# microsoft/UniVL

Hardware: NVIDIA H100
Metric: video-text samples/sec (higher is better)
Workload: dtype bf16

## Files before the change

### include/univl_b200.h

```cpp
#ifndef UNIVL_B200_H_
#define UNIVL_B200_H_

#ifdef __cplusplus
extern "C" {
#endif

const char* univl_last_error_string(void);
int univl_abi_version(void);
int univl_set_reserved_sms(int n);
int univl_partials_reduce(const float* part, int nparts, long long rows, long long cols, float* dst, long long ld,
                          void* stream);

int univl_gemm_bf16(const void* A, long long lda, int a_mn_major, const void* B, long long ldb, int b_mn_major,
                    int M, int N, int Kc, void* out, long long ldo, int epilogue, const float* bias,
                    const void* aux_in, long long ld_aux_in, void* aux_out, long long ld_aux_out, float alpha,
                    int block_n, int split_k, void* stream);
int univl_gemm_plan(int M, int N, int Kc, int epilogue, int block_n, int split_k);

int univl_quantize_e4m3_rows(const void* x, long long ldx, void* q, long long ldq, float* scale, int M, int K,
                             void* stream);
int univl_quantize_e4m3_blocks(const float* w, long long ldw, void* q, long long ldq, float* scale, int N, int K,
                               void* stream);
int univl_gemm_fp8(const void* A, long long lda, const float* a_scale, const void* B, long long ldb,
                   const float* b_scale, int M, int N, int Kc, int epilogue, const float* bias, void* out,
                   long long ldo, float* out_scale, void* stream);

int univl_layernorm_fwd(const void* x, const void* res, const float* gamma, const float* beta, void* y, float* mean,
                        float* rstd, int rows, int cols, float eps, float p_drop, int drop_mode,
                        const unsigned long long* rng_state, unsigned long long stream_id, void* stream);
int univl_layernorm_bwd(const void* dy, const void* dy2, const void* x, const void* res, const float* gamma,
                        const float* mean, const float* rstd, void* dx_res, void* dx_dense, float* dgamma,
                        float* dbeta, float* dbias, int rows, int cols, float p_drop, int drop_mode,
                        const unsigned long long* rng_state, unsigned long long stream_id, void* stream);
int univl_layernorm_f32_fwd(const float* x, const float* gamma, const float* beta, void* y, float* mean, float* rstd,
                            int rows, int cols, float eps, void* stream);
int univl_layernorm_f32_bwd(const void* dy, const float* x, const float* gamma, const float* mean, const float* rstd,
                            float* dgamma, float* dbeta, int rows, int cols, void* stream);

int univl_embed_text_fwd(const long long* ids, const long long* type_ids, const float* word, const float* pos,
                         const float* type, const float* gamma, const float* beta, void* y, float* mean, float* rstd,
                         int n_seq, int S, int H, int vocab, float eps, float p_drop, const unsigned long long* rng_state,
                         unsigned long long stream_id, void* stream);
int univl_embed_text_bwd(const void* dy, const long long* ids, const long long* type_ids, const float* word,
                         const float* pos, const float* type, const float* gamma, const float* mean,
                         const float* rstd, float* dword, float* dpos, float* dtype, float* dgamma, float* dbeta,
                         int n_seq, int S, int H, int vocab, float p_drop, const unsigned long long* rng_state,
                         unsigned long long stream_id, void* stream);
int univl_embed_src_fwd(const void* a, const void* b, const float* pos, const float* type, const float* gamma,
                        const float* beta, void* y, float* mean, float* rstd, int Na, int Wa, int Nb, int Fb,
                        int all_pairs, int H, float eps, float p_drop, const unsigned long long* rng_state,
                        unsigned long long stream_id, void* stream);
int univl_embed_src_bwd(const void* dy, const void* a, const void* b, const float* pos, const float* type,
                        const float* gamma, const float* mean, const float* rstd, void* da, void* db, float* dpos,
                        float* dtype, float* dgamma, float* dbeta, int Na, int Wa, int Nb, int Fb, int all_pairs,
                        int H, float p_drop, const unsigned long long* rng_state, unsigned long long stream_id, void* stream);

int univl_attention_fwd(const void* q, long long ldq, const void* k, long long ldk, const void* v, long long ldv,
                        void* o, long long ldo, float* lse, const long long* mask_a, const long long* mask_b, int Wa,
                        int Fb, int Nb, int all_pairs, int n_seq, int heads, int Sq, int Sk, int causal, float scale,
                        float p_drop, const unsigned long long* rng_state, unsigned long long stream_id, void* stream);
int univl_attention_bwd(const void* q, long long ldq, const void* k, long long ldk, const void* v, long long ldv,
                        const void* o, long long ldo, const float* lse, const void* d_o, long long lddo, void* dq,
                        long long lddq, void* dk, long long lddk, void* dv, long long lddv, const long long* mask_a,
                        const long long* mask_b, int Wa, int Fb, int Nb, int all_pairs, int n_seq, int heads, int Sq,
                        int Sk, int causal, float scale, float p_drop, const unsigned long long* rng_state,
                        unsigned long long stream_id, int rng_layout, float* dbq, float* dbk, float* dbv, void* stream);
int univl_attention_long_fwd(const void* q, long long ldq, const void* k, long long ldk, const void* v, long long ldv,
                             void* o, long long ldo, float* lse, const long long* mask_a, const long long* mask_b,
                             int Wa, int Fb, int Nb, int all_pairs, int n_seq, int heads, int Sq, int Sk, int causal,
                             float scale, float p_drop, const unsigned long long* rng_state,
                             unsigned long long stream_id, void* stream);
int univl_attention_long_bwd(const void* q, long long ldq, const void* k, long long ldk, const void* v, long long ldv,
                             const void* o, long long ldo, const float* lse, const void* d_o, long long lddo, void* dq,
                             long long lddq, void* dk, long long lddk, void* dv, long long lddv,
                             const long long* mask_a, const long long* mask_b, int Wa, int Fb, int Nb, int all_pairs,
                             int n_seq, int heads, int Sq, int Sk, int causal, float scale, float p_drop,
                             const unsigned long long* rng_state, unsigned long long stream_id, int rng_layout,
                             float* dbq, float* dbk, float* dbv, void* stream);
int univl_attention_pair_fwd(const void* qa, long long ldqa, const void* ka, long long ldka, const void* va,
                             long long ldva, const void* qb, long long ldqb, const void* kb, long long ldkb,
                             const void* vb, long long ldvb, void* o, long long ldo, float* lse,
                             const long long* mask_a, const long long* mask_b, int Na, int Wa, int Nb, int Fb,
                             int heads, int Sq, float scale, void* stream);
int univl_attention_varlen_fwd(const void* qa, long long ldqa, const void* ka, long long ldka, const void* va,
                               long long ldva, const void* qb, long long ldqb, const void* kb, long long ldkb,
                               const void* vb, long long ldvb, const int* idx_a, const int* idx_b, const int* start_a,
                               const int* start_b, const int* len_a, const int* cu_seqlens, int n_seq, int max_sk,
                               int heads, int q_first, void* o, long long ldo, float* lse, float scale, void* stream);
int univl_gather_rows_varlen(const void* a, long long lda, const void* b, long long ldb, const int* idx_a,
                             const int* idx_b, const int* start_a, const int* start_b, const int* len_a,
                             const int* cu_seqlens, int n_seq, int q_first, int cols, void* out, long long ldo,
                             void* stream);
int univl_fused_qkv_attention_supported(int n_seq, int heads, int S, int H);
int univl_fused_qkv_attention_fwd(const void* x, long long ldx, const void* wqkv, long long ldw, const float* bias,
                                  void* qkv_out, long long ld_qkv, void* o, long long ldo, float* lse,
                                  const long long* mask_a, const long long* mask_b, int Wa, int Fb, int Nb,
                                  int all_pairs, int n_seq, int heads, int S, int causal, float scale, float p_drop,
                                  const unsigned long long* rng_state, unsigned long long stream_id, void* stream);
int univl_fused_attention_bwd(const void* qkv, long long ld_qkv, const void* o, long long ldo, const float* lse,
                              const void* d_o, long long lddo, void* dqkv, long long ld_dqkv, float* dbias,
                              const long long* mask_a, const long long* mask_b, int Wa, int Fb, int Nb, int all_pairs,
                              int n_seq, int heads, int S, int causal, float scale, float p_drop,
                              const unsigned long long* rng_state, unsigned long long stream_id, void* stream);

int univl_colsum_bf16(const void* x, long long ld, float* out, int rows, int cols, void* stream);
int univl_cast_f32_to_bf16(const float* src, void* dst, long long n, void* stream);
int univl_cast_bf16_to_f32(const void* src, float* dst, long long n, void* stream);
int univl_multi_cast_f32_to_bf16(const unsigned long long* device_table, int n_tensors, int blocks_per_tensor,
                                 void* stream);
int univl_fill_f32(float* p, float value, long long n, void* stream);
int univl_rng_advance(unsigned long long* rng_state, void* stream);
int univl_gelu_fwd_bf16(const void* x, void* out, long long n, void* stream);
int univl_gelu_bwd_bf16(const void* dy, const void* pre, void* out, long long n, void* stream);
int univl_tanh_fwd_bf16(const void* x, void* out, long long n, void* stream);
int univl_tanh_bwd_bf16(const void* dy, const void* y, void* out, long long n, void* stream);
int univl_scale_f32(float* dst, const float* src, long long n, const float* gscale, void* stream);

int univl_meanpool_fwd(const void* x, const long long* mask, float* out, float* norm_out, int N, int S, int H,
                       int skip_first, int guard_zero, int l2norm, void* stream);
int univl_meanpool_bwd(const float* dy, const float* y, const float* norm, const long long* mask, void* dx, int N,
                       int S, int H, int skip_first, int guard_zero, int l2norm, void* stream);
int univl_sim_matmul_fwd(const float* t, const float* v, float* sim, int Bt, int Bv, int H, int groups, void* stream);
int univl_sim_matmul_bwd(const float* dsim, const float* t, const float* v, float* dt, float* dv, int Bt, int Bv,
                         int H, int groups, void* stream);
int univl_maxmargin_loss(const float* sim, float* loss, float* dsim, int B, float margin, int n_pair, float w_same,
                         float w_diff, int groups, void* stream);
int univl_crossen_loss(const float* sim, float* loss, float* dsim, int B, int groups, void* stream);
int univl_milnce_loss(const float* sim, float* loss, float* dsim, int batch_size, int n_pair, int groups,
                      void* stream);
int univl_softmax_xent_fwd(const float* logits, long long ld, const long long* labels, const long long* pair_mask,
                           float* lse, float* sum_count, float* loss, int T, int V, int target_mode,
                           long long ignore_index, int groups, void* stream);
int univl_softmax_xent_bwd(const float* logits, long long ld, const long long* labels, const long long* pair_mask,
                           const float* lse, const float* sum_count, const float* gscale, void* dlogits,
                           long long ld_d, int T, int V, int target_mode, long long ignore_index, int groups,
                           void* stream);
int univl_vocab_xent_workspace(int T, int V);
int univl_vocab_xent_fwd(const void* x, long long ldx, const void* w, long long ldw, const float* bias,
                         const long long* labels, float* lse, float* sum_count, float* loss, void* workspace,
                         long long workspace_bytes, int T, int V, int Kc, int groups, void* stream);
int univl_vocab_xent_bwd(const void* x, long long ldx, const void* w, long long ldw, const float* bias,
                         const long long* labels, const float* lse, const float* sum_count, const float* gscale,
                         void* dlogits, long long ld_d, int T, int V, int Kc, int groups, void* stream);
int univl_pooler_sim_fwd(const void* u, const float* w, const float* b, float* out, int N, int H, void* stream);
int univl_pooler_sim_bwd(const void* u, const float* w, const float* dout, void* du, float* dw, float* db, int N,
                         int H, void* stream);

int univl_bert_adam_step(float* p, const float* g, float* m, float* v, void* p_bf16, const void* segs, int n_chunks,
                         int n_tensors, float* scratch, long long* step, float b1, float b2, float eps,
                         float max_grad_norm, float global_clip_norm, float warmup, long long t_total,
                         float grad_scale, void* stream);
int univl_bert_adam_step_bf16grad(float* p, const void* g_bf16, float* m, float* v, void* p_bf16, const void* segs,
                                  int n_chunks, int n_tensors, float* scratch, long long* step, float b1, float b2,
                                  float eps, float max_grad_norm, float global_clip_norm, float warmup,
                                  long long t_total, float grad_scale, void* stream);

#ifdef __cplusplus
}
#endif
#endif
```

### univl_b200/csrc/gemm_wgmma.cu

```cuda
#include "common.cuh"
#include "fp8.cuh"
#include "pipeline.cuh"
#include "tmap.cuh"

#include <stdio.h>
#include <type_traits>

namespace univl {

enum GemmEpilogue : int {
  EPI_BIAS_BF16 = 0,
  EPI_BIAS_GELU_BF16 = 1,
  EPI_GELU_BWD_BF16 = 2,
  EPI_ADD_BF16 = 3,
  EPI_BIAS_F32 = 4,
  EPI_ATOMIC_F32 = 5,
};

struct GemmParams {
  int M, N, Kc;
  int k_blocks_per_split;
  int epilogue;
  float alpha;
  void* out;
// ... 102 lines not shown
  if (epi == EPI_BIAS_GELU_BF16) {
    bf16* ao = p.aux_out + (long long)row * p.ld_aux_out + col;
    if (vec) *reinterpret_cast<uint32_t*>(ao) = pack_bf16x2(v0, v1);
    else {
      ao[0] = __float2bfloat16(v0);
      if (two) ao[1] = __float2bfloat16(v1);
    }
    v0 = gelu_erf(v0);
    v1 = gelu_erf(v1);
  }
  bf16* o = reinterpret_cast<bf16*>(p.out) + (long long)row * p.ldo + col;
  if (vec) *reinterpret_cast<uint32_t*>(o) = pack_bf16x2(v0, v1);
  else {
    o[0] = __float2bfloat16(v0);
    if (two) o[1] = __float2bfloat16(v1);
  }
}

constexpr int EPI_CHUNK = 8;

__device__ __forceinline__ uint4 quad_transpose(uint32_t w0, uint32_t w1, uint32_t w2, uint32_t w3, int q) {
  const bool odd = q & 1;
  uint32_t r0 = __shfl_xor_sync(0xffffffffu, odd ? w0 : w1, 1);
  uint32_t r1 = __shfl_xor_sync(0xffffffffu, odd ? w2 : w3, 1);
  if (odd) {
    w0 = r0;
    w2 = r1;
  } else {
    w1 = r0;
    w3 = r1;
  }
  const bool hi = q & 2;
  r0 = __shfl_xor_sync(0xffffffffu, hi ? w0 : w2, 2);
  r1 = __shfl_xor_sync(0xffffffffu, hi ? w1 : w3, 2);
  if (hi) {
    w0 = r0;
    w1 = r1;
  } else {
    w2 = r0;
    w3 = r1;
  }
  return make_uint4(w0, w1, w2, w3);
}

template <int EPI, bool BIAS, int BLOCK_N, bool WIDE = false>
__device__ __forceinline__ void epi_tile(const GemmParams& p, float alpha, int row, int col0,
                                         const float (&acc)[BLOCK_N / 2]) {
  constexpr int GROUPS = BLOCK_N / 8;
  constexpr int CHUNK = WIDE ? 4 : (GROUPS < EPI_CHUNK ? GROUPS : EPI_CHUNK);
  static_assert(CHUNK % 4 == 0, "a chunk holds whole quads of 8-column groups");
  constexpr bool AUX = EPI == EPI_GELU_BWD_BF16 || EPI == EPI_ADD_BF16;
  constexpr bool OUT_F32 = EPI == EPI_BIAS_F32 || EPI == EPI_ATOMIC_F32;
  static_assert(!(WIDE && OUT_F32), "16-byte stores are for the bf16 outputs");
  constexpr bool ACCUM = EPI == EPI_ATOMIC_F32;
  const int q = threadIdx.x & 3;
  const float* bias = p.bias + col0;
  const bf16* ax = p.aux_in + (long long)row * p.ld_aux_in + col0;
  const long long ax8 = 8 * p.ld_aux_in;
  bf16* ao = p.aux_out + (long long)row * p.ld_aux_out + col0;
  const long long ao8 = 8 * p.ld_aux_out;
  const long long o8 = 8 * p.ldo;
  float* of = reinterpret_cast<float*>(p.out) + (long long)row * p.ldo + col0;
  bf16* ob = reinterpret_cast<bf16*>(p.out) + (long long)row * p.ldo + col0;
  float b[2][CHUNK][2];
  uint32_t x[2][CHUNK][2];
  float2 a[2][CHUNK][2];
  auto load = [&](int j0, int s) {
#pragma unroll
    for (int j = 0; j < CHUNK; ++j) {
      const int c = (j0 + j) * 8;
      if constexpr (BIAS) {
        b[s][j][0] = __ldg(bias + c);
        b[s][j][1] = __ldg(bias + c + 1);
      }
#pragma unroll
      for (int h = 0; h < 2; ++h) {
        if constexpr (AUX) x[s][j][h] = *reinterpret_cast<const uint32_t*>(ax + h * ax8 + c);
        if constexpr (ACCUM) a[s][j][h] = *reinterpret_cast<const float2*>(of + h * o8 + c);
      }
    }
  };
  load(0, 0);
#pragma unroll
  for (int j0 = 0; j0 < GROUPS; j0 += CHUNK) {
    const int s = (j0 / CHUNK) & 1;
    if (j0 + CHUNK < GROUPS) load(j0 + CHUNK, s ^ 1);
#pragma unroll
    for (int jq = 0; jq < CHUNK; jq += 4) {
#pragma unroll
      for (int h = 0; h < 2; ++h) {
        uint32_t wo[4], wa[4];
#pragma unroll
        for (int jj = 0; jj < 4; ++jj) {
          const int j = jq + jj;
          const int c = (j0 + j) * 8;
          float v0 = __fmul_rn(acc[4 * (j0 + j) + 2 * h], alpha);
          float v1 = __fmul_rn(acc[4 * (j0 + j) + 2 * h + 1], alpha);
          if constexpr (BIAS) {
            v0 = __fadd_rn(v0, b[s][j][0]);
            v1 = __fadd_rn(v1, b[s][j][1]);
          }
          if constexpr (AUX) {
            const float2 f = unpack_bf16x2(x[s][j][h]);
            if constexpr (EPI == EPI_GELU_BWD_BF16) {
              v0 = __fmul_rn(v0, gelu_erf_grad(f.x));
              v1 = __fmul_rn(v1, gelu_erf_grad(f.y));
            } else {
              v0 = __fadd_rn(v0, f.x);
              v1 = __fadd_rn(v1, f.y);
            }
          }
          if constexpr (OUT_F32) {
            if constexpr (ACCUM) {
              v0 = __fadd_rn(a[s][j][h].x, v0);
              v1 = __fadd_rn(a[s][j][h].y, v1);
            }
            *reinterpret_cast<float2*>(of + h * o8 + c) = make_float2(v0, v1);
          } else {
            if constexpr (EPI == EPI_BIAS_GELU_BF16) {
              const uint32_t w = pack_bf16x2(v0, v1);
              if constexpr (WIDE) wa[jj] = w;
              else *reinterpret_cast<uint32_t*>(ao + h * ao8 + c) = w;
              v0 = gelu_erf(v0);
              v1 = gelu_erf(v1);
            }
            const uint32_t w = pack_bf16x2(v0, v1);
            if constexpr (WIDE) wo[jj] = w;
            else *reinterpret_cast<uint32_t*>(ob + h * o8 + c) = w;
          }
        }
        if constexpr (WIDE) {
          const int c = (j0 + jq) * 8 + 6 * q;
          if constexpr (EPI == EPI_BIAS_GELU_BF16)
            *reinterpret_cast<uint4*>(ao + h * ao8 + c) = quad_transpose(wa[0], wa[1], wa[2], wa[3], q);
          *reinterpret_cast<uint4*>(ob + h * o8 + c) = quad_transpose(wo[0], wo[1], wo[2], wo[3], q);
        }
      }
    }
  }
}

template <int BLOCK_N>
__device__ __forceinline__ void epilogue_block(const GemmParams& p, bool inside, float alpha, int n0, int row,
                                               int col0, const float (&acc)[BLOCK_N / 2]) {
  if (inside) {
    const bool bias = p.bias != nullptr;
    const bool wide = p.vec8;
    switch (p.epilogue) {
      case EPI_BIAS_BF16:
        if (wide) {
          if (bias) epi_tile<EPI_BIAS_BF16, true, BLOCK_N, true>(p, alpha, row, col0, acc);
          else epi_tile<EPI_BIAS_BF16, false, BLOCK_N, true>(p, alpha, row, col0, acc);
        } else {
          if (bias) epi_tile<EPI_BIAS_BF16, true, BLOCK_N>(p, alpha, row, col0, acc);
          else epi_tile<EPI_BIAS_BF16, false, BLOCK_N>(p, alpha, row, col0, acc);
        }
        break;
      case EPI_BIAS_GELU_BF16:
        if (wide) {
          if (bias) epi_tile<EPI_BIAS_GELU_BF16, true, BLOCK_N, true>(p, alpha, row, col0, acc);
          else epi_tile<EPI_BIAS_GELU_BF16, false, BLOCK_N, true>(p, alpha, row, col0, acc);
        } else {
          if (bias) epi_tile<EPI_BIAS_GELU_BF16, true, BLOCK_N>(p, alpha, row, col0, acc);
          else epi_tile<EPI_BIAS_GELU_BF16, false, BLOCK_N>(p, alpha, row, col0, acc);
        }
        break;
      case EPI_GELU_BWD_BF16:
        if (wide) epi_tile<EPI_GELU_BWD_BF16, false, BLOCK_N, true>(p, alpha, row, col0, acc);
        else epi_tile<EPI_GELU_BWD_BF16, false, BLOCK_N>(p, alpha, row, col0, acc);
        break;
      case EPI_ADD_BF16:
        if (wide) epi_tile<EPI_ADD_BF16, false, BLOCK_N, true>(p, alpha, row, col0, acc);
        else epi_tile<EPI_ADD_BF16, false, BLOCK_N>(p, alpha, row, col0, acc);
        break;
      case EPI_BIAS_F32:
        if (bias) epi_tile<EPI_BIAS_F32, true, BLOCK_N>(p, alpha, row, col0, acc);
        else epi_tile<EPI_BIAS_F32, false, BLOCK_N>(p, alpha, row, col0, acc);
        break;
      default:
        epi_tile<EPI_ATOMIC_F32, false, BLOCK_N>(p, alpha, row, col0, acc);
    }
  } else {
#pragma unroll
    for (int j = 0; j < BLOCK_N / 8; ++j) {
      if (n0 + j * 8 >= p.N) break;
      epi_pair(p, alpha, row, col0 + j * 8, acc[4 * j], acc[4 * j + 1]);
      epi_pair(p, alpha, row + 8, col0 + j * 8, acc[4 * j + 2], acc[4 * j + 3]);
    }
  }
}

__device__ __forceinline__ bool tile_inside(const GemmParams& p, const WorkItem& wi, int bn) {
  return p.vec2 && wi.m0 + BLOCK_M <= p.M && wi.n0 + bn <= p.N;
}

template <int BLOCK_N>
__device__ __forceinline__ bool splitk_fixup(const GemmParams& p, int tile, int half, int split, float alpha,
                                             float (&acc)[BLOCK_N / 2]) {
  constexpr int V = BLOCK_N / 8;
  constexpr int CHUNK = BLOCK_N == 256 ? 4 : 8;
  const int t = threadIdx.x & 127;
  const int lane = t & 31;
  const long long slot = 64LL * BLOCK_N;
  float4* base = reinterpret_cast<float4*>(p.slots + ((long long)tile * p.splits * 2 + half) * slot) + t;
  float4* mine = base + split * (2 * slot / 4);
#pragma unroll
  for (int j = 0; j < V; ++j) {
#pragma unroll
    for (int e = 0; e < 4; ++e) acc[4 * j + e] = __fmul_rn(acc[4 * j + e], alpha);
    __stcg(mine + j * 128, make_float4(acc[4 * j], acc[4 * j + 1], acc[4 * j + 2], acc[4 * j + 3]));
  }
  fence_acq_rel_gpu();
  __syncwarp();
  unsigned before = 0;
  if (lane == 0) before = atom_add_acq_rel_gpu(p.arrived + (tile * 2 + half) * 4 + (t >> 5), 1u);
  before = __shfl_sync(0xffffffffu, before, 0);
  if (before != (unsigned)p.splits - 1) return false;
  fence_acq_rel_gpu();
#pragma unroll
  for (int j0 = 0; j0 < V; j0 += CHUNK) {
    float4 s4[CHUNK];
#pragma unroll
    for (int j = 0; j < CHUNK; ++j) s4[j] = make_float4(0.f, 0.f, 0.f, 0.f);
    for (int s = 0; s < p.splits; ++s) {
      float4 v[CHUNK];
      if (s == split) {
#pragma unroll
        for (int j = 0; j < CHUNK; ++j) {
          const int a = 4 * (j0 + j);
          v[j] = make_float4(acc[a], acc[a + 1], acc[a + 2], acc[a + 3]);
        }
      } else {
        const float4* src = base + s * (2 * slot / 4);
#pragma unroll
        for (int j = 0; j < CHUNK; ++j) v[j] = __ldcg(src + (j0 + j) * 128);
      }
#pragma unroll
      for (int j = 0; j < CHUNK; ++j) {
        s4[j].x = __fadd_rn(s4[j].x, v[j].x);
        s4[j].y = __fadd_rn(s4[j].y, v[j].y);
        s4[j].z = __fadd_rn(s4[j].z, v[j].z);
        s4[j].w = __fadd_rn(s4[j].w, v[j].w);
      }
    }
#pragma unroll
    for (int j = 0; j < CHUNK; ++j) {
      const int a = 4 * (j0 + j);
      acc[a] = s4[j].x;
      acc[a + 1] = s4[j].y;
      acc[a + 2] = s4[j].z;
      acc[a + 3] = s4[j].w;
    }
  }
  return true;
}

template <int BLOCK_N>
__device__ __forceinline__ void finish_block(const GemmParams& p, const WorkItem& wi, int n_tiles, int kb_per,
                                             bool inside, float alpha, int half, int row, int col0,
                                             float (&acc)[BLOCK_N / 2]) {
  if (p.slots != nullptr) {
    const int tile = (wi.m0 / BLOCK_M) * n_tiles + wi.n0 / BLOCK_N;
    if (!splitk_fixup<BLOCK_N>(p, tile, half, wi.kb_begin / kb_per, alpha, acc)) return;
    alpha = 1.f;
  }
  epilogue_block<BLOCK_N>(p, inside, alpha, wi.n0, row, col0, acc);
}

constexpr int TURN_BAR = 1;

template <int BLOCK_N, int STAGES, bool A_MN, bool B_MN, int ELEM = 2>
__device__ __forceinline__ void produce_ring(const CUtensorMap* tmap_a, const CUtensorMap* tmap_b, uint8_t* smem,
                                             const Ring<STAGES>& ring, int num_work, int m_tiles, int n_tiles,
                                             int total_kb, int kb_per) {
  using L = GemmSmem<BLOCK_N, STAGES>;
  uint32_t it = 0;
  for (int w = blockIdx.x; w < num_work; w += gridDim.x) {
    const WorkItem wi = decode_work(w, m_tiles, n_tiles, total_kb, kb_per, BLOCK_N);
    for (int i = 0; i < wi.num_kb; ++i, ++it) {
      const int s = ring.acquire(it, L::STAGE_BYTES);
      uint64_t* bar = &ring.full[s];
      uint8_t* sa = smem + s * L::STAGE_BYTES;
      uint8_t* sb = sa + L::A_BYTES;
      const int k_elem = (wi.kb_begin + i) * (128 / ELEM);
      if (!A_MN) {
        tma_load_2d(sa, tmap_a, bar, k_elem, wi.m0);
      } else {
#pragma unroll
        for (int c = 0; c < BLOCK_M / 64; ++c)
          tma_load_2d(sa + c * (BLOCK_K * 128), tmap_a, bar, wi.m0 + c * 64, k_elem);
      }
      if (!B_MN) {
        tma_load_2d(sb, tmap_b, bar, k_elem, wi.n0);
      } else {
#pragma unroll
        for (int c = 0; c < BLOCK_N / 64; ++c)
          tma_load_2d(sb + c * (BLOCK_K * 128), tmap_b, bar, wi.n0 + c * 64, k_elem);
      }
    }
  }
}

template <int BLOCK_N, int STAGES, bool A_MN, bool B_MN>
__global__ void __launch_bounds__(PIPELINE_THREADS, 1)
gemm_wgmma_kernel(const __grid_constant__ CUtensorMap tmap_a, const __grid_constant__ CUtensorMap tmap_b,
                  const GemmParams p, const int num_work) {
  using L = GemmSmem<BLOCK_N, STAGES>;
  constexpr bool PING = BLOCK_N <= 128;
  constexpr bool FOLD = BLOCK_N == 64;
  Ring<STAGES> ring;
  uint8_t* smem = kernel_prologue(ring, L::BAR_OFFSET, PING ? 1 : 2, &tmap_a, &tmap_b);

  const int wg = threadIdx.x >> 7;
  const int m_tiles = (p.M + BLOCK_M - 1) / BLOCK_M;
  const int n_tiles = (p.N + BLOCK_N - 1) / BLOCK_N;
  const int total_kb = (p.Kc + BLOCK_K - 1) / BLOCK_K;
  const int kb_per = p.k_blocks_per_split;

  if (wg == 0) {
    if (producer_regs())
      produce_ring<BLOCK_N, STAGES, A_MN, B_MN>(&tmap_a, &tmap_b, smem, ring, num_work, m_tiles, n_tiles, total_kb,
                                                kb_per);
  } else if constexpr (!PING) {
    consumer_regs();
    const int c = wg - 1;
    const int t = threadIdx.x & 127;
    const int warp = t >> 5, lane = t & 31;
    uint32_t it = 0;
    for (int w = blockIdx.x; w < num_work; w += gridDim.x) {
      const WorkItem wi = decode_work(w, m_tiles, n_tiles, total_kb, kb_per, BLOCK_N);
      float acc[BLOCK_N / 2];
#pragma unroll
      for (int e = 0; e < BLOCK_N / 2; ++e) acc[e] = 0.f;
      const int last = mma_kblocks<BLOCK_N, A_MN, B_MN, L::STAGE_BYTES, L::A_BYTES>(ring, smem, c * (64 * 128), acc,
                                                                                     0, wi.num_kb, it, t == 0);
      mma_drain(ring, last, acc, t == 0);
      const int row = wi.m0 + c * 64 + warp * 16 + (lane >> 2);
      const int col0 = wi.n0 + 2 * (lane & 3);
      finish_block<BLOCK_N>(p, wi, n_tiles, kb_per, tile_inside(p, wi, BLOCK_N), p.alpha, c, row, col0, acc);
    }
  } else {
    consumer_regs();
    const int c = wg - 1;
    const int t = threadIdx.x & 127;
    const int warp = t >> 5, lane = t & 31;
    uint32_t it = 0;
    int j = 0;
    for (int w = blockIdx.x; w < num_work; w += gridDim.x, ++j) {
      const WorkItem wi = decode_work(w, m_tiles, n_tiles, total_kb, kb_per, BLOCK_N);
      if ((j & 1) != c) {
        it += wi.num_kb;
        continue;
      }
      float acc[2][BLOCK_N / 2];
#pragma unroll
      for (int e = 0; e < BLOCK_N / 2; ++e) acc[0][e] = acc[1][e] = 0.f;
      const bool fold = FOLD && p.kb_seg < wi.num_kb;
      const int seg = fold ? p.kb_seg : wi.num_kb;
      float sum[2][FOLD ? BLOCK_N / 2 : 1];
      if constexpr (FOLD) {
#pragma unroll
        for (int e = 0; e < BLOCK_N / 2; ++e) sum[0][e] = sum[1][e] = 0.f;
      }
      if (j > 0) named_bar(TURN_BAR + c, 256);
      for (int i0 = 0; i0 < wi.num_kb; i0 += seg) {
        const int i1 = min(wi.num_kb, i0 + seg);
        const int last =
            mma_kblocks<BLOCK_N, 2, A_MN, B_MN, L::STAGE_BYTES, L::A_BYTES>(ring, smem, 0, acc, i0, i1, it, t == 0);
        if (i1 == wi.num_kb && w + (int)gridDim.x < num_work)
          named_bar_arrive(TURN_BAR + (c ^ 1), 256);
        mma_drain(ring, last, acc, t == 0);
        if constexpr (FOLD) {
          if (fold) {
#pragma unroll
            for (int e = 0; e < BLOCK_N / 2; ++e) {
              sum[0][e] = __fadd_rn(sum[0][e], __fmul_rn(acc[0][e], p.alpha));
              sum[1][e] = __fadd_rn(sum[1][e], __fmul_rn(acc[1][e], p.alpha));
            }
          }
        }
      }
      float alpha = p.alpha;
      if constexpr (FOLD) {
        if (fold) {
#pragma unroll
          for (int e = 0; e < BLOCK_N / 2; ++e) {
            acc[0][e] = sum[0][e];
            acc[1][e] = sum[1][e];
          }
          alpha = 1.f;
        }
      }
      const bool inside = tile_inside(p, wi, BLOCK_N);
      const int row = wi.m0 + warp * 16 + (lane >> 2);
      const int col0 = wi.n0 + 2 * (lane & 3);
      finish_block<BLOCK_N>(p, wi, n_tiles, kb_per, inside, alpha, 0, row, col0, acc[0]);
      finish_block<BLOCK_N>(p, wi, n_tiles, kb_per, inside, alpha, 1, row + 64, col0, acc[1]);
    }
  }
}

template <int BLOCK_N, int STAGES, bool A_MN, bool B_MN>
static int launch_gemm(const CUtensorMap& ta, const CUtensorMap& tb, const GemmParams& p, int splits,
                       cudaStream_t stream) {
  using L = GemmSmem<BLOCK_N, STAGES>;
  auto kern = gemm_wgmma_kernel<BLOCK_N, STAGES, A_MN, B_MN>;
  const char* name = "univl_gemm_bf16";
  if (int rc = persistent_prepare(kern, L::DYN_BYTES, name)) return rc;
  const long long work =
      (long long)((p.M + BLOCK_M - 1) / BLOCK_M) * ((p.N + BLOCK_N - 1) / BLOCK_N) * (long long)splits;
  return persistent_launch(kern, name, work, L::DYN_BYTES, stream, ta, tb, p, (int)work);
}

template <int BLOCK_N, int STAGES>
static int dispatch_major(bool a_mn, bool b_mn, const CUtensorMap& ta, const CUtensorMap& tb, const GemmParams& p,
                          int splits, cudaStream_t stream) {
  if (!a_mn && !b_mn) return launch_gemm<BLOCK_N, STAGES, false, false>(ta, tb, p, splits, stream);
  if (!a_mn && b_mn) return launch_gemm<BLOCK_N, STAGES, false, true>(ta, tb, p, splits, stream);
  if (a_mn && b_mn) return launch_gemm<BLOCK_N, STAGES, true, true>(ta, tb, p, splits, stream);
  return launch_gemm<BLOCK_N, STAGES, true, false>(ta, tb, p, splits, stream);
}

enum Fp8Epilogue : int { FP8_EPI_BIAS_BF16 = 0, FP8_EPI_GELU_E4M3 = 1 };

struct Fp8Params {
  const float* a_scale;
  const float* b_scale;
  uint8_t* out_q;
  float* out_scale;
};

constexpr int FP8_BLOCK_N = 128;
constexpr int FP8_STAGES = 6;

template <int EPI, bool PAIRS>
__global__ void __launch_bounds__(PIPELINE_THREADS, 1)
gemm_fp8_kernel(const __grid_constant__ CUtensorMap tmap_a, const __grid_constant__ CUtensorMap tmap_b,
                const GemmParams p, const Fp8Params f, const int num_work) {
  using L = GemmSmem<FP8_BLOCK_N, FP8_STAGES>;
  Ring<FP8_STAGES> ring;
  uint8_t* smem = kernel_prologue(ring, L::BAR_OFFSET, 2, &tmap_a, &tmap_b);

  const int wg = threadIdx.x >> 7;
  const int m_tiles = (p.M + BLOCK_M - 1) / BLOCK_M;
  const int n_tiles = p.N / FP8_BLOCK_N;
  const int total_kb = p.Kc / 128;

  if (wg == 0) {
    if (producer_regs())
      produce_ring<FP8_BLOCK_N, FP8_STAGES, false, false, 1>(&tmap_a, &tmap_b, smem, ring, num_work, m_tiles, n_tiles,
                                                              total_kb, total_kb);
    return;
  }
  consumer_regs();
  const int c = wg - 1;
  const int t = threadIdx.x & 127;
  const int warp = t >> 5, lane = t & 31;
  const int M = p.M;
  uint32_t it = 0;
  for (int w = blockIdx.x; w < num_work; w += gridDim.x) {
    const WorkItem wi = decode_work(w, m_tiles, n_tiles, total_kb, total_kb, FP8_BLOCK_N);
    const int row = wi.m0 + c * 64 + warp * 16 + (lane >> 2);
    const bool in0 = row < M, in1 = row + 8 < M;
    const float* sa = f.a_scale + row;
    const float* sb = f.b_scale + (long long)(wi.n0 / FP8_BLOCK_N) * total_kb;
    float acc[FP8_BLOCK_N / 2];
#pragma unroll
    for (int e = 0; e < FP8_BLOCK_N / 2; ++e) acc[e] = 0.f;
    auto issue = [&](float (&tmp)[FP8_BLOCK_N / 2], int kb) {
      const int s = ring.wait(it + kb);
      const uint32_t a_s = smem_u32(smem + s * L::STAGE_BYTES) + c * (64 * 128);
      const uint32_t b_s = smem_u32(smem + s * L::STAGE_BYTES) + L::A_BYTES;
      wgmma_fence();
      fence_regs(tmp);
#pragma unroll
      for (int k = 0; k < 4; ++k)
        WgmmaSSE4M3N128::mma(tmp, make_smem_desc_sw128(a_s + k * 32, 16, 1024),
                             make_smem_desc_sw128(b_s + k * 32, 16, 1024), k > 0 ? 1 : 0);
      wgmma_commit();
      fence_regs(tmp);
    };
    auto promote = [&](auto newer, float (&tmp)[FP8_BLOCK_N / 2], int kb) {
      const float bs = __ldg(sb + kb);
      const float s0 = in0 ? __ldg(sa + (long long)kb * M) : 0.f;
      const float s1 = in1 ? __ldg(sa + (long long)kb * M + 8) : 0.f;
      wgmma_wait<decltype(newer)::value>();
      fence_regs(tmp);
      if (t == 0) ring.release(ring.stage(it + kb));
      const float f0 = s0 * bs, f1 = s1 * bs;
#pragma unroll
      for (int j = 0; j < FP8_BLOCK_N / 8; ++j) {
        acc[4 * j] = __fmaf_rn(tmp[4 * j], f0, acc[4 * j]);
        acc[4 * j + 1] = __fmaf_rn(tmp[4 * j + 1], f0, acc[4 * j + 1]);
        acc[4 * j + 2] = __fmaf_rn(tmp[4 * j + 2], f1, acc[4 * j + 2]);
        acc[4 * j + 3] = __fmaf_rn(tmp[4 * j + 3], f1, acc[4 * j + 3]);
      }
    };
    using One = std::integral_constant<int, 1>;
    using None = std::integral_constant<int, 0>;
    float ta[FP8_BLOCK_N / 2];
    if constexpr (PAIRS) {
      float tb[FP8_BLOCK_N / 2];
      issue(ta, 0);
      issue(tb, 1);
      int kb = 0;
      for (; kb + 2 < total_kb; kb += 2) {
        promote(One(), ta, kb);
        issue(ta, kb + 2);
        promote(One(), tb, kb + 1);
        issue(tb, kb + 3);
      }
      promote(One(), ta, kb);
      promote(None(), tb, kb + 1);
    } else {
      for (int kb = 0; kb < total_kb; ++kb) {
        issue(ta, kb);
        promote(None(), ta, kb);
      }
    }
    it += total_kb;
    const int col0 = wi.n0 + 2 * (lane & 3);
    if constexpr (EPI == FP8_EPI_BIAS_BF16) {
      if (tile_inside(p, wi, FP8_BLOCK_N)) {
        if (p.vec8) epi_tile<EPI_BIAS_BF16, true, FP8_BLOCK_N, true>(p, p.alpha, row, col0, acc);
        else epi_tile<EPI_BIAS_BF16, true, FP8_BLOCK_N>(p, p.alpha, row, col0, acc);
      } else {
#pragma unroll
        for (int j = 0; j < FP8_BLOCK_N / 8; ++j) {
          epi_pair(p, p.alpha, row, col0 + j * 8, acc[4 * j], acc[4 * j + 1]);
          epi_pair(p, p.alpha, row + 8, col0 + j * 8, acc[4 * j + 2], acc[4 * j + 3]);
        }
      }
    } else {
      const float* bias = p.bias + col0;
#pragma unroll
      for (int h = 0; h < 2; ++h) {
        float amax = 0.f;
#pragma unroll
        for (int j = 0; j < FP8_BLOCK_N / 8; ++j) {
          const float v0 = gelu_erf(__fadd_rn(acc[4 * j + 2 * h], __ldg(bias + 8 * j)));
          const float v1 = gelu_erf(__fadd_rn(acc[4 * j + 2 * h + 1], __ldg(bias + 8 * j + 1)));
          acc[4 * j + 2 * h] = v0;
          acc[4 * j + 2 * h + 1] = v1;
          amax = fmaxf(amax, fmaxf(fabsf(v0), fabsf(v1)));
        }
        amax = fmaxf(amax, __shfl_xor_sync(0xffffffffu, amax, 1));
        amax = fmaxf(amax, __shfl_xor_sync(0xffffffffu, amax, 2));
        const float sc = e4m3_scale(amax);
        const float inv = e4m3_inv_scale(sc);
        const int r = row + 8 * h;
        if (r < M) {
          uint8_t* q = f.out_q + (long long)r * p.ldo + col0;
#pragma unroll
          for (int j = 0; j < FP8_BLOCK_N / 8; ++j)
            *reinterpret_cast<uint16_t*>(q + 8 * j) =
                e4m3x2(__fmul_rn(acc[4 * j + 2 * h], inv), __fmul_rn(acc[4 * j + 2 * h + 1], inv));
          if ((lane & 3) == 0) f.out_scale[(long long)(wi.n0 / FP8_BLOCK_N) * M + r] = sc;
        }
      }
    }
  }
}

template <int EPI, bool PAIRS>
static int launch_gemm_fp8(const CUtensorMap& ta, const CUtensorMap& tb, const GemmParams& p, const Fp8Params& f,
                           cudaStream_t stream) {
  using L = GemmSmem<FP8_BLOCK_N, FP8_STAGES>;
  auto kern = gemm_fp8_kernel<EPI, PAIRS>;
  const char* name = "univl_gemm_fp8";
  if (int rc = persistent_prepare(kern, L::DYN_BYTES, name)) return rc;
  const long long work = (long long)((p.M + BLOCK_M - 1) / BLOCK_M) * (p.N / FP8_BLOCK_N);
  return persistent_launch(kern, name, work, L::DYN_BYTES, stream, ta, tb, p, f, (int)work);
}

constexpr int VX_BLOCK_N = 128;
constexpr int VX_STAGES = 6;

struct VocabXentParams {
  int T, V, Kc;
  int m_tiles, n_tiles, chunks, chunk_tiles;
  const float* bias;
  const long long* labels;
  float4* part;
  const float* lse;
  const float* count;
  const float* gscale;
  int rows_per_group, groups;
  bf16* dl;
  long long ld_d;
};

template <bool BWD>
__global__ void __launch_bounds__(PIPELINE_THREADS, 1)
vocab_xent_kernel(const __grid_constant__ CUtensorMap tmap_a, const __grid_constant__ CUtensorMap tmap_b,
                  const VocabXentParams p, const int num_work) {
  using L = GemmSmem<VX_BLOCK_N, VX_STAGES>;
  Ring<VX_STAGES> ring;
  uint8_t* smem = kernel_prologue(ring, L::BAR_OFFSET, 2, &tmap_a, &tmap_b);
  const int wg = threadIdx.x >> 7;
  const int total_kb = (p.Kc + BLOCK_K - 1) / BLOCK_K;

  if (wg == 0) {
    if (!producer_regs()) return;
    uint32_t it = 0;
    for (int w = blockIdx.x; w < num_work; w += gridDim.x) {
      const int chunk = w / p.m_tiles;
      const int m0 = (w - chunk * p.m_tiles) * BLOCK_M;
      const int nt1 = min(p.n_tiles, (chunk + 1) * p.chunk_tiles);
      for (int nt = chunk * p.chunk_tiles; nt < nt1; ++nt) {
        for (int kb = 0; kb < total_kb; ++kb, ++it) {
          const int s = ring.acquire(it, L::STAGE_BYTES);
          uint8_t* sa = smem + s * L::STAGE_BYTES;
          tma_load_2d(sa, &tmap_a, &ring.full[s], kb * BLOCK_K, m0);
          tma_load_2d(sa + L::A_BYTES, &tmap_b, &ring.full[s], kb * BLOCK_K, nt * VX_BLOCK_N);
        }
      }
    }
    return;
  }
  consumer_regs();
  const int c = wg - 1;
  const int t = threadIdx.x & 127;
  const int warp = t >> 5, lane = t & 31, q = lane & 3;
  uint32_t it = 0;
  for (int w = blockIdx.x; w < num_work; w += gridDim.x) {
    const int chunk = w / p.m_tiles;
    const int row = (w - chunk * p.m_tiles) * BLOCK_M + c * 64 + warp * 16 + (lane >> 2);
    long long lab[2];
    float m[2], s[2], xt[2], lse[2], g[2];
#pragma unroll
    for (int h = 0; h < 2; ++h) {
      const int r = row + 8 * h;
      lab[h] = r < p.T ? __ldg(p.labels + r) : -1;
      m[h] = -INFINITY;
      s[h] = 0.f;
      xt[h] = 0.f;
      if constexpr (BWD) {
        lse[h] = 0.f;
        g[h] = 0.f;
        if (lab[h] != -1) {
          lse[h] = __ldg(p.lse + r);
          g[h] = ((p.gscale ? __ldg(p.gscale) : 1.f) / (float)p.groups) / __ldg(p.count + r / p.rows_per_group);
        }
      }
    }
    const int nt1 = min(p.n_tiles, (chunk + 1) * p.chunk_tiles);
    for (int nt = chunk * p.chunk_tiles; nt < nt1; ++nt) {
      float acc[VX_BLOCK_N / 2];
#pragma unroll
      for (int e = 0; e < VX_BLOCK_N / 2; ++e) acc[e] = 0.f;
      const int last = mma_kblocks<VX_BLOCK_N, false, false, L::STAGE_BYTES, L::A_BYTES>(ring, smem, c * (64 * 128),
                                                                                          acc, 0, total_kb, it, t == 0);
      mma_drain(ring, last, acc, t == 0);

      const int col0 = nt * VX_BLOCK_N + 2 * q;
#pragma unroll
      for (int j = 0; j < VX_BLOCK_N / 8; ++j) {
#pragma unroll
        for (int e = 0; e < 2; ++e) {
          const int col = col0 + 8 * j + e;
          const float b = (p.bias != nullptr && col < p.V) ? __ldg(p.bias + col) : 0.f;
          acc[4 * j + e] = __fadd_rn(acc[4 * j + e], b);
          acc[4 * j + 2 + e] = __fadd_rn(acc[4 * j + 2 + e], b);
        }
      }
      if constexpr (!BWD) {
#pragma unroll
        for (int h = 0; h < 2; ++h) {
          float tm = -INFINITY;
#pragma unroll
          for (int j = 0; j < VX_BLOCK_N / 8; ++j)
#pragma unroll
            for (int e = 0; e < 2; ++e)
              if (col0 + 8 * j + e < p.V) tm = fmaxf(tm, acc[4 * j + 2 * h + e]);
          if (tm > m[h]) {
            s[h] = s[h] * __expf(m[h] - tm);
            m[h] = tm;
          }
#pragma unroll
          for (int j = 0; j < VX_BLOCK_N / 8; ++j)
#pragma unroll
            for (int e = 0; e < 2; ++e) {
              const int col = col0 + 8 * j + e;
              const float v = acc[4 * j + 2 * h + e];
              if (col < p.V) s[h] += __expf(v - m[h]);
              if (col == lab[h]) xt[h] = v;
            }
        }
      } else {
        const int ncol = min(p.ld_d - (long long)nt * VX_BLOCK_N, (long long)VX_BLOCK_N);
#pragma unroll
        for (int h = 0; h < 2; ++h) {
          const int r = row + 8 * h;
          if (r >= p.T) continue;
          bf16* drow = p.dl + (long long)r * p.ld_d + col0;
          const bool scored = lab[h] != -1;
#pragma unroll
          for (int j = 0; j < VX_BLOCK_N / 8; ++j) {
            if (8 * j + 2 * q >= ncol) break;
            float d[2];
#pragma unroll
            for (int e = 0; e < 2; ++e) {
              const int col = col0 + 8 * j + e;
              d[e] = 0.f;
              if (scored && col < p.V)
                d[e] = (__expf(acc[4 * j + 2 * h + e] - lse[h]) - (col == lab[h] ? 1.f : 0.f)) * g[h];
            }
            *reinterpret_cast<uint32_t*>(drow + 8 * j) = pack_bf16x2(d[0], d[1]);
          }
        }
      }
    }
    if constexpr (!BWD) {
#pragma unroll
      for (int h = 0; h < 2; ++h) {
#pragma unroll
        for (int o = 1; o <= 2; o <<= 1) {
          const float mo = __shfl_xor_sync(0xffffffffu, m[h], o);
          const float so = __shfl_xor_sync(0xffffffffu, s[h], o);
          const float xo = __shfl_xor_sync(0xffffffffu, xt[h], o);
          const float mx = fmaxf(m[h], mo);
          const float a = m[h] == -INFINITY ? 0.f : s[h] * __expf(m[h] - mx);
          const float b = mo == -INFINITY ? 0.f : so * __expf(mo - mx);
          m[h] = mx;
          s[h] = a + b;
          xt[h] += xo;
        }
        const int r = row + 8 * h;
        if (q == 0 && r < p.T) p.part[(long long)r * p.chunks + chunk] = make_float4(m[h], s[h], xt[h], 0.f);
      }
    }
  }
}

__global__ void __launch_bounds__(256)
vocab_xent_rows_kernel(const float4* __restrict__ part, const long long* __restrict__ labels, int T, int V, int chunks,
                       int chunk_cols, float* __restrict__ lse_out, float* __restrict__ nll) {
  const int r = blockIdx.x * blockDim.x + threadIdx.x;
  if (r >= T) return;
  const long long lab = labels[r];
  if (lab == -1) {
    lse_out[r] = 0.f;
    return;
  }
  const float4* pr = part + (long long)r * chunks;
  float4 f = pr[0];
  float m = f.x, s = f.y;
  for (int k = 1; k < chunks; ++k) {
    f = pr[k];
    const float mx = fmaxf(m, f.x);
    s = s * __expf(m - mx) + f.y * __expf(f.x - mx);
    m = mx;
  }
  const float lse = m + __logf(s);
  lse_out[r] = lse;
  nll[r] = (lab >= 0 && lab < V) ? lse - pr[lab / chunk_cols].z : __int_as_float(0x7fc00000);
}

constexpr int VX_GROUP_THREADS = 512;
__global__ void __launch_bounds__(VX_GROUP_THREADS)
vocab_xent_group_kernel(const float* __restrict__ nll, const long long* __restrict__ labels, int rows_per_group,
                        float* __restrict__ sum_count, int groups) {
  __shared__ float red[2][VX_GROUP_THREADS];
  const int grp = blockIdx.x;
  float sum = 0.f, cnt = 0.f;
  for (int i = threadIdx.x; i < rows_per_group; i += VX_GROUP_THREADS) {
    const long long r = (long long)grp * rows_per_group + i;
    if (labels[r] == -1) continue;
    sum += nll[r];
    cnt += 1.f;
  }
  red[0][threadIdx.x] = sum;
  red[1][threadIdx.x] = cnt;
  __syncthreads();
  for (int o = VX_GROUP_THREADS / 2; o > 0; o >>= 1) {
    if (threadIdx.x < o) {
      red[0][threadIdx.x] += red[0][threadIdx.x + o];
      red[1][threadIdx.x] += red[1][threadIdx.x + o];
    }
    __syncthreads();
  }
  if (threadIdx.x == 0) {
    sum_count[grp] = red[0][0];
    sum_count[groups + grp] = red[1][0];
  }
}

__global__ void vocab_xent_mean_kernel(const float* __restrict__ sum_count, int groups, float* __restrict__ out) {
  float acc = sum_count[0] / sum_count[groups];
  for (int g = 1; g < groups; ++g) acc += sum_count[g] / sum_count[groups + g];
  *out = groups > 1 ? acc / (float)groups : acc;
}

template <bool BWD>
static int launch_vocab_xent(const CUtensorMap& ta, const CUtensorMap& tb, const VocabXentParams& p,
                             cudaStream_t stream) {
  const long long work = (long long)p.m_tiles * p.chunks;
  return persistent_launch(vocab_xent_kernel<BWD>, BWD ? "univl_vocab_xent_bwd" : "univl_vocab_xent_fwd", work,
                           GemmSmem<VX_BLOCK_N, VX_STAGES>::DYN_BYTES, stream, ta, tb, p, (int)work);
}

}

using namespace univl;

namespace {
struct GemmPlan {
  int bn, splits, kb_per, kb_seg;
};
int plan_gemm(int M, int N, int Kc, int epilogue, int block_n, int split_k, GemmPlan* plan) {
  const int total_kb = (Kc + BLOCK_K - 1) / BLOCK_K;
  const int m_tiles = (M + BLOCK_M - 1) / BLOCK_M;
  int bn = block_n;
  if (bn == 0) {
    bn = 256;
    if (epilogue != EPI_ATOMIC_F32) {
      const auto tiles = [&](int w) { return (long long)m_tiles * ((N + w - 1) / w); };
      if (tiles(256) < 2 * PLAN_SMS) bn = 128;
      if (tiles(128) < PLAN_SMS) bn = 64;
    }
    if (N <= 64) bn = 64;
    else if (N <= 128 && bn > 128) bn = 128;
  }
  UNIVL_CHECK_ARG(bn == 64 || bn == 128 || bn == 256, "gemm: block_n must be 64/128/256");
  const int n_tiles = (N + bn - 1) / bn;
  int splits = 1;
  if (epilogue == EPI_ATOMIC_F32) {
    splits = split_k;
    if (splits == 0) {
      const long long tiles = (long long)m_tiles * n_tiles;
      splits = (int)((2 * PLAN_SMS + tiles - 1) / tiles);
      if (splits > total_kb / 2) splits = total_kb / 2;
      if (splits < 1) splits = 1;
    }
    if (splits > total_kb) splits = total_kb;
  }
  int kb_per = (total_kb + splits - 1) / splits;
  splits = (total_kb + kb_per - 1) / kb_per;
  int kb_seg = kb_per;
  if (epilogue == EPI_ATOMIC_F32 && block_n == 0 && split_k == 0 && Kc < SPLIT_MIN_K && splits > 1) {
    bn = 64;
    splits = 1;
    kb_per = total_kb;
  }
  plan->bn = bn; plan->splits = splits; plan->kb_per = kb_per; plan->kb_seg = kb_seg;
  return UNIVL_OK;
}

GemmParams gemm_params(int M, int N, int Kc, int kb_per, int epilogue, float alpha, void* out, long long ldo,
                       const float* bias, const void* aux_in, long long ld_aux_in, void* aux_out,
                       long long ld_aux_out) {
  GemmParams p;
  p.M = M; p.N = N; p.Kc = Kc;
  p.k_blocks_per_split = kb_per;
  p.epilogue = epilogue;
  p.alpha = alpha;
  p.out = out; p.ldo = ldo;
  p.bias = bias;
  p.aux_in = reinterpret_cast<const bf16*>(aux_in); p.ld_aux_in = ld_aux_in;
  p.aux_out = reinterpret_cast<bf16*>(aux_out); p.ld_aux_out = ld_aux_out;
  const bool out_f32 = epilogue == EPI_BIAS_F32 || epilogue == EPI_ATOMIC_F32;
  bool vec2 = ((uintptr_t)out % (out_f32 ? 8 : 4)) == 0 && (ldo % 2) == 0;
  if (aux_in != nullptr) vec2 = vec2 && ((uintptr_t)aux_in % 4) == 0 && (ld_aux_in % 2) == 0;
  if (aux_out != nullptr) vec2 = vec2 && ((uintptr_t)aux_out % 4) == 0 && (ld_aux_out % 2) == 0;
  p.vec2 = vec2 ? 1 : 0;
  bool vec8 = !out_f32 && ((uintptr_t)out % 16) == 0 && (ldo % 8) == 0;
  if (aux_out != nullptr) vec8 = vec8 && ((uintptr_t)aux_out % 16) == 0 && (ld_aux_out % 8) == 0;
  p.vec8 = vec8 ? 1 : 0;
  p.slots = nullptr;
  p.arrived = nullptr;
  p.splits = 1;
  p.kb_seg = kb_per;
  return p;
}
}

extern "C" int univl_gemm_plan(int M, int N, int Kc, int epilogue, int block_n, int split_k) {
  GemmPlan plan;
  if (int rc = plan_gemm(M, N, Kc, epilogue, block_n, split_k, &plan)) return rc;
  return 1;
}

extern "C" int univl_gemm_bf16(const void* A, long long lda, int a_mn_major, const void* B, long long ldb,
                               int b_mn_major, int M, int N, int Kc, void* out, long long ldo, int epilogue,
                               const float* bias, const void* aux_in, long long ld_aux_in, void* aux_out,
                               long long ld_aux_out, float alpha, int block_n, int split_k, void* stream_) {
  cudaStream_t stream = reinterpret_cast<cudaStream_t>(stream_);
  UNIVL_CHECK_ARG(M > 0 && N > 0 && Kc > 0, "gemm: empty problem M=%d N=%d K=%d", M, N, Kc);
  UNIVL_CHECK_ARG(A && B && out, "gemm: null operand");
  UNIVL_CHECK_ARG((lda % 8) == 0 && (ldb % 8) == 0, "gemm: lda/ldb must be multiples of 8 elements (got %lld, %lld)",
                  lda, ldb);
  UNIVL_CHECK_ARG(((uintptr_t)A & 15) == 0 && ((uintptr_t)B & 15) == 0, "gemm: operands must be 16-byte aligned");
  UNIVL_CHECK_ARG(epilogue >= 0 && epilogue <= 5, "gemm: unknown epilogue %d", epilogue);
  if (epilogue == EPI_GELU_BWD_BF16 || epilogue == EPI_ADD_BF16)
    UNIVL_CHECK_ARG(aux_in != nullptr, "gemm: epilogue %d needs aux_in", epilogue);
  if (epilogue == EPI_BIAS_GELU_BF16) UNIVL_CHECK_ARG(aux_out != nullptr, "gemm: gelu epilogue needs aux_out");
  UNIVL_CHECK_ARG(split_k >= 0, "gemm: bad split_k");
  if (epilogue != EPI_ATOMIC_F32) UNIVL_CHECK_ARG(split_k <= 1, "gemm: split_k>1 needs the atomic epilogue");

  GemmPlan plan;
  if (int prc = plan_gemm(M, N, Kc, epilogue, block_n, split_k, &plan)) return prc;
  const int bn = plan.bn;

  CUtensorMap ta, tb;
  int rc;
  if (!a_mn_major) rc = make_tmap(&ta, A, M, Kc, lda, BLOCK_M);
  else             rc = make_tmap(&ta, A, Kc, M, lda, BLOCK_K);
  if (rc) return rc;
  if (!b_mn_major) rc = make_tmap(&tb, B, N, Kc, ldb, bn);
  else             rc = make_tmap(&tb, B, Kc, N, ldb, BLOCK_K);
  if (rc) return rc;

  GemmParams p = gemm_params(M, N, Kc, plan.kb_per, epilogue, alpha, out, ldo, bias, aux_in, ld_aux_in, aux_out,
                             ld_aux_out);
  p.splits = plan.splits;
  p.kb_seg = plan.kb_seg;
  if (plan.splits > 1) {
    const long long tiles = (long long)((M + BLOCK_M - 1) / BLOCK_M) * ((N + bn - 1) / bn);
    const size_t slot_bytes = (size_t)tiles * plan.splits * BLOCK_M * bn * sizeof(float);
    const size_t counter_bytes = (size_t)tiles * 8 * sizeof(unsigned);
    if ((rc = scratch_alloc((void**)&p.slots, slot_bytes + counter_bytes, stream))) return rc;
    p.arrived = reinterpret_cast<unsigned*>(p.slots + slot_bytes / sizeof(float));
    const cudaError_t e = cudaMemsetAsync(p.arrived, 0, counter_bytes, stream);
    if (e != cudaSuccess) {
      cudaFreeAsync(p.slots, stream);
      return set_error(UNIVL_ERR_CUDA, "gemm split-K counters: %s", cudaGetErrorString(e));
    }
  }

  const bool amn = a_mn_major != 0, bmn = b_mn_major != 0;
  if (bn == 256) rc = dispatch_major<256, 4>(amn, bmn, ta, tb, p, plan.splits, stream);
  else if (bn == 128) rc = dispatch_major<128, 6>(amn, bmn, ta, tb, p, plan.splits, stream);
  else rc = dispatch_major<64, 8>(amn, bmn, ta, tb, p, plan.splits, stream);
  if (p.slots != nullptr) cudaFreeAsync(p.slots, stream);
  return rc;
}

extern "C" int univl_gemm_fp8(const void* A, long long lda, const float* a_scale, const void* B, long long ldb,
                              const float* b_scale, int M, int N, int Kc, int epilogue, const float* bias, void* out,
                              long long ldo, float* out_scale, void* stream_) {
  cudaStream_t stream = reinterpret_cast<cudaStream_t>(stream_);
  UNIVL_CHECK_ARG(M > 0 && N > 0 && Kc > 0, "univl_gemm_fp8: empty problem M=%d N=%d K=%d", M, N, Kc);
  UNIVL_CHECK_ARG(Kc % 128 == 0, "univl_gemm_fp8: K=%d must be a multiple of 128 (one scale per 128 columns)", Kc);
  UNIVL_CHECK_ARG(N % 128 == 0, "univl_gemm_fp8: N=%d must be a multiple of 128 (one scale per 128 x 128 block)", N);
  UNIVL_CHECK_ARG(epilogue == FP8_EPI_BIAS_BF16 || epilogue == FP8_EPI_GELU_E4M3,
                  "univl_gemm_fp8: unknown epilogue %d", epilogue);
  UNIVL_CHECK_ARG(A && B && a_scale && b_scale && bias && out, "univl_gemm_fp8: null operand, scale, bias or output");
  UNIVL_CHECK_ARG(lda >= Kc && ldb >= Kc && (lda % 16) == 0 && (ldb % 16) == 0,
                  "univl_gemm_fp8: lda/ldb must be >= K and multiples of 16 (got %lld, %lld, K=%d)", lda, ldb, Kc);
  UNIVL_CHECK_ARG(((uintptr_t)A & 15) == 0 && ((uintptr_t)B & 15) == 0,
                  "univl_gemm_fp8: A and B must be 16-byte aligned");
  UNIVL_CHECK_ARG(ldo >= N, "univl_gemm_fp8: ldo=%lld must be >= N=%d", ldo, N);
  if (epilogue == FP8_EPI_GELU_E4M3) {
    UNIVL_CHECK_ARG(out_scale != nullptr, "univl_gemm_fp8: the GELU epilogue needs out_scale");
    UNIVL_CHECK_ARG(((uintptr_t)out & 15) == 0 && (ldo % 16) == 0,
                    "univl_gemm_fp8: the e4m3 output must be 16-byte aligned with ldo a multiple of 16 (got %lld)",
                    ldo);
  }

  CUtensorMap ta, tb;
  int rc;
  if ((rc = make_tmap(&ta, A, M, Kc, lda, BLOCK_M, true))) return rc;
  if ((rc = make_tmap(&tb, B, N, Kc, ldb, FP8_BLOCK_N, true))) return rc;

  const GemmParams p = gemm_params(M, N, Kc, Kc / 128, EPI_BIAS_BF16, 1.f, out, ldo, bias, nullptr, 0, nullptr, 0);
  Fp8Params f;
  f.a_scale = a_scale;
  f.b_scale = b_scale;
  f.out_q = reinterpret_cast<uint8_t*>(out);
  f.out_scale = out_scale;
  const bool pairs = (Kc / 128) % 2 == 0;
  if (epilogue == FP8_EPI_BIAS_BF16)
    return pairs ? launch_gemm_fp8<FP8_EPI_BIAS_BF16, true>(ta, tb, p, f, stream)
                 : launch_gemm_fp8<FP8_EPI_BIAS_BF16, false>(ta, tb, p, f, stream);
  return pairs ? launch_gemm_fp8<FP8_EPI_GELU_E4M3, true>(ta, tb, p, f, stream)
               : launch_gemm_fp8<FP8_EPI_GELU_E4M3, false>(ta, tb, p, f, stream);
}

namespace {
constexpr int VX_MIN_CHUNK_TILES = 8;
struct VxPlan {
  int m_tiles, n_tiles, chunks, chunk_tiles;
};
VxPlan vx_plan(int T, int V) {
  VxPlan pl;
  pl.m_tiles = (T + BLOCK_M - 1) / BLOCK_M;
  pl.n_tiles = (V + VX_BLOCK_N - 1) / VX_BLOCK_N;
  long long best = -1;
  for (int c = 1; c <= pl.n_tiles; ++c) {
    const int ct = (pl.n_tiles + c - 1) / c;
    if (ct < VX_MIN_CHUNK_TILES && c > 1) break;
    if (c > 1 && ct == (pl.n_tiles + c - 2) / (c - 1)) continue;
    const int chunks = (pl.n_tiles + ct - 1) / ct;
    const long long rounds = ((long long)pl.m_tiles * chunks + PLAN_SMS - 1) / PLAN_SMS;
    if (best < 0 || rounds * ct < best) {
      best = rounds * ct;
      pl.chunks = chunks;
      pl.chunk_tiles = ct;
    }
  }
  return pl;
}

int vx_check(const char* name, const void* x, long long ldx, const void* w, long long ldw, const long long* labels,
             int T, int V, int Kc, int groups) {
  UNIVL_CHECK_ARG(T > 0 && V > 0 && Kc > 0, "%s: empty problem T=%d V=%d K=%d", name, T, V, Kc);
  UNIVL_CHECK_ARG(x && w && labels, "%s: null x, W or labels", name);
  UNIVL_CHECK_ARG(ldx >= Kc && ldw >= Kc && (ldx % 8) == 0 && (ldw % 8) == 0,
                  "%s: ldx/ldw must be >= K and multiples of 8 (got %lld, %lld, K=%d)", name, ldx, ldw, Kc);
  UNIVL_CHECK_ARG(((uintptr_t)x & 15) == 0 && ((uintptr_t)w & 15) == 0, "%s: x and W must be 16-byte aligned", name);
  UNIVL_CHECK_ARG(groups > 0 && T % groups == 0, "%s: %d groups must divide T=%d", name, groups, T);
  return UNIVL_OK;
}

template <bool BWD>
int vx_params(const void* x, long long ldx, const void* w, long long ldw, int T, int V, int Kc, CUtensorMap* ta,
              CUtensorMap* tb, VocabXentParams* p) {
  if (int rc = persistent_prepare(vocab_xent_kernel<BWD>, GemmSmem<VX_BLOCK_N, VX_STAGES>::DYN_BYTES,
                                  BWD ? "univl_vocab_xent_bwd" : "univl_vocab_xent_fwd"))
    return rc;
  const VxPlan pl = vx_plan(T, V);
  int rc;
  if ((rc = make_tmap(ta, x, T, Kc, ldx, BLOCK_M))) return rc;
  if ((rc = make_tmap(tb, w, V, Kc, ldw, VX_BLOCK_N))) return rc;
  *p = VocabXentParams{};
  p->T = T; p->V = V; p->Kc = Kc;
  p->m_tiles = pl.m_tiles; p->n_tiles = pl.n_tiles; p->chunks = pl.chunks; p->chunk_tiles = pl.chunk_tiles;
  return UNIVL_OK;
}


long long vx_workspace_bytes(int T, int V) {
  return (long long)T * vx_plan(T, V).chunks * (long long)sizeof(float4) + ((long long)T * 4 + 15) / 16 * 16;
}
}

extern "C" int univl_vocab_xent_workspace(int T, int V) {
  UNIVL_CHECK_ARG(T > 0 && V > 0, "univl_vocab_xent_workspace: empty problem T=%d V=%d", T, V);
  const long long bytes = vx_workspace_bytes(T, V);
  UNIVL_CHECK_ARG(bytes <= 0x7fffffffLL, "univl_vocab_xent_workspace: T=%d V=%d needs over 2 GiB", T, V);
  return (int)bytes;
}

extern "C" int univl_vocab_xent_fwd(const void* x, long long ldx, const void* w, long long ldw, const float* bias,
                                    const long long* labels, float* lse, float* sum_count, float* loss,
                                    void* workspace, long long workspace_bytes, int T, int V, int Kc, int groups,
                                    void* stream_) {
  const char* name = "univl_vocab_xent_fwd";
  if (int rc = vx_check(name, x, ldx, w, ldw, labels, T, V, Kc, groups)) return rc;
  UNIVL_CHECK_ARG(lse && sum_count && loss && workspace, "%s: null lse, sum_count, loss or workspace", name);
  UNIVL_CHECK_ARG(((uintptr_t)workspace & 15) == 0, "%s: the workspace must be 16-byte aligned", name);
  const long long need = vx_workspace_bytes(T, V);
  UNIVL_CHECK_ARG(workspace_bytes >= need, "%s: workspace of %lld bytes, needs %lld (univl_vocab_xent_workspace)",
                  name, workspace_bytes, need);
  cudaStream_t stream = reinterpret_cast<cudaStream_t>(stream_);
  CUtensorMap ta, tb;
  VocabXentParams p;
  if (int rc = vx_params<false>(x, ldx, w, ldw, T, V, Kc, &ta, &tb, &p)) return rc;
  p.bias = bias;
  p.labels = labels;
  p.part = reinterpret_cast<float4*>(workspace);
  if (int rc = launch_vocab_xent<false>(ta, tb, p, stream)) return rc;
  float* nll = reinterpret_cast<float*>(p.part + (long long)T * p.chunks);
  vocab_xent_rows_kernel<<<(T + 255) / 256, 256, 0, stream>>>(p.part, labels, T, V, p.chunks,
                                                               p.chunk_tiles * VX_BLOCK_N, lse, nll);
  vocab_xent_group_kernel<<<groups, VX_GROUP_THREADS, 0, stream>>>(nll, labels, T / groups, sum_count, groups);
  vocab_xent_mean_kernel<<<1, 1, 0, stream>>>(sum_count, groups, loss);
  UNIVL_CHECK_LAUNCH(name);
  return UNIVL_OK;
}

extern "C" int univl_vocab_xent_bwd(const void* x, long long ldx, const void* w, long long ldw, const float* bias,
                                    const long long* labels, const float* lse, const float* sum_count,
                                    const float* gscale, void* dlogits, long long ld_d, int T, int V, int Kc,
                                    int groups, void* stream_) {
  const char* name = "univl_vocab_xent_bwd";
  if (int rc = vx_check(name, x, ldx, w, ldw, labels, T, V, Kc, groups)) return rc;
  UNIVL_CHECK_ARG(lse && sum_count && dlogits, "%s: null lse, sum_count or dlogits", name);
  const long long cols = (long long)vx_plan(T, V).n_tiles * VX_BLOCK_N;
  UNIVL_CHECK_ARG(ld_d >= V && ld_d <= cols && (ld_d % 2) == 0 && ((uintptr_t)dlogits & 3) == 0,
                  "%s: ld_d=%lld must be even, >= V=%d and <= V rounded up to 128, with dlogits 4-byte aligned", name,
                  ld_d, V);
  cudaStream_t stream = reinterpret_cast<cudaStream_t>(stream_);
  CUtensorMap ta, tb;
  VocabXentParams p;
  if (int rc = vx_params<true>(x, ldx, w, ldw, T, V, Kc, &ta, &tb, &p)) return rc;
  p.bias = bias;
  p.labels = labels;
  p.lse = lse;
  p.count = sum_count + groups;
  p.gscale = gscale;
  p.rows_per_group = T / groups;
  p.groups = groups;
  p.dl = reinterpret_cast<bf16*>(dlogits);
  p.ld_d = ld_d;
  return launch_vocab_xent<true>(ta, tb, p, stream);
}
```

### univl_b200/csrc/layernorm.cu

```cuda
#include "common.cuh"

namespace univl {

constexpr int LN_WARPS = 8;
constexpr int LN_MAX_VEC = 4;

__device__ __forceinline__ void load8(const bf16* p, float (&v)[8]) {
  const uint4 u = *reinterpret_cast<const uint4*>(p);
  const uint32_t w[4] = {u.x, u.y, u.z, u.w};
#pragma unroll
  for (int j = 0; j < 4; ++j) {
    const float2 f = unpack_bf16x2(w[j]);
    v[2 * j] = f.x;
    v[2 * j + 1] = f.y;
  }
}
__device__ __forceinline__ void load8(const float* p, float (&v)[8]) {
  const float4 a = *reinterpret_cast<const float4*>(p);
  const float4 b = *reinterpret_cast<const float4*>(p + 4);
  v[0] = a.x; v[1] = a.y; v[2] = a.z; v[3] = a.w;
  v[4] = b.x; v[5] = b.y; v[6] = b.z; v[7] = b.w;
}
template <typename T> struct Raw8;
template <> struct Raw8<bf16> { uint4 u; };
template <> struct Raw8<float> { float4 a, b; };
__device__ __forceinline__ void raw_load(const bf16* p, Raw8<bf16>& r) {
  asm volatile("ld.global.nc.L1::no_allocate.v4.u32 {%0, %1, %2, %3}, [%4];"
               : "=r"(r.u.x), "=r"(r.u.y), "=r"(r.u.z), "=r"(r.u.w) : "l"(p));
}
__device__ __forceinline__ void raw_load(const float* p, Raw8<float>& r) {
  r.a = __ldg(reinterpret_cast<const float4*>(p));
  r.b = __ldg(reinterpret_cast<const float4*>(p + 4));
}
__device__ __forceinline__ void raw_unpack(const Raw8<bf16>& r, float (&v)[8]) {
  const uint32_t w[4] = {r.u.x, r.u.y, r.u.z, r.u.w};
#pragma unroll
  for (int j = 0; j < 4; ++j) {
    const float2 f = unpack_bf16x2(w[j]);
    v[2 * j] = f.x;
    v[2 * j + 1] = f.y;
  }
}
__device__ __forceinline__ void raw_unpack(const Raw8<float>& r, float (&v)[8]) {
  v[0] = r.a.x; v[1] = r.a.y; v[2] = r.a.z; v[3] = r.a.w;
  v[4] = r.b.x; v[5] = r.b.y; v[6] = r.b.z; v[7] = r.b.w;
}
__device__ __forceinline__ void store8(bf16* p, const float (&v)[8]) {
  uint4 u;
  u.x = pack_bf16x2(v[0], v[1]);
  u.y = pack_bf16x2(v[2], v[3]);
  u.z = pack_bf16x2(v[4], v[5]);
  u.w = pack_bf16x2(v[6], v[7]);
  *reinterpret_cast<uint4*>(p) = u;
}

struct DropCfg {
  int mode;
  uint32_t threshold;
  float scale;
  uint64_t seed, stream;
  const unsigned long long* rng;
};
__device__ __forceinline__ DropCfg resolve_drop(DropCfg d) {
  if (d.mode != 0 && d.rng != nullptr) {
    d.seed = d.rng[0];
    d.stream += d.rng[1] << 20;
  }
  return d;
}

__device__ __forceinline__ uint32_t keep8_mask(const DropCfg& d, uint64_t idx0) {
  return dropout_keep8(d.seed, d.stream, idx0, d.threshold);
}

template <typename TIn, int NVEC>
__global__ void __launch_bounds__(LN_WARPS * 32, NVEC <= 3 ? 3 : 2)
layernorm_fwd_kernel(const TIn* __restrict__ x, const bf16* __restrict__ res, const float* __restrict__ gamma,
                     const float* __restrict__ beta, bf16* __restrict__ y, float* __restrict__ mean_out,
                     float* __restrict__ rstd_out, int rows, float eps, DropCfg drop_in) {
  pdl_trigger();
  pdl_wait();
  const DropCfg drop = resolve_drop(drop_in);
  constexpr int cols = NVEC * 256;
  const int warp = threadIdx.x >> 5, lane = threadIdx.x & 31;
  const float inv_cols = 1.0f / (float)cols;
  const long long stride = (long long)gridDim.x * LN_WARPS;
  long long row = (long long)blockIdx.x * LN_WARPS + warp;
  Raw8<TIn> nx[NVEC];
  Raw8<bf16> nr[NVEC];
  if (row < rows) {
#pragma unroll
    for (int i = 0; i < NVEC; ++i) {
      const long long off = row * cols + (i * 32 + lane) * 8;
      raw_load(x + off, nx[i]);
      if (res != nullptr) raw_load(res + off, nr[i]);
    }
  }
  for (; row < rows; row += stride) {
    float z[NVEC][8];
    float s = 0.f;
#pragma unroll
    for (int i = 0; i < NVEC; ++i) {
      const int c = (i * 32 + lane) * 8;
      raw_unpack(nx[i], z[i]);
      if (drop.mode == 1) {
        const uint32_t keep = keep8_mask(drop, (uint64_t)row * cols + c);
#pragma unroll
        for (int j = 0; j < 8; ++j) z[i][j] = ((keep >> j) & 1u) ? z[i][j] * drop.scale : 0.f;
      }
      if (res != nullptr) {
        float r[8];
        raw_unpack(nr[i], r);
#pragma unroll
        for (int j = 0; j < 8; ++j) z[i][j] += r[j];
      }
#pragma unroll
      for (int j = 0; j < 8; ++j) s += z[i][j];
    }
    const long long next = row + stride;
    if (next < rows) {
#pragma unroll
      for (int i = 0; i < NVEC; ++i) {
        const long long off = next * cols + (i * 32 + lane) * 8;
        raw_load(x + off, nx[i]);
        if (res != nullptr) raw_load(res + off, nr[i]);
      }
    }
    const float mean = warp_sum(s) * inv_cols;
    float q = 0.f;
#pragma unroll
    for (int i = 0; i < NVEC; ++i)
#pragma unroll
      for (int j = 0; j < 8; ++j) {
        const float d = z[i][j] - mean;
        q += d * d;
      }
    const float var = warp_sum(q) * inv_cols;
    const float rstd = 1.0f / sqrtf(var + eps);
    if (lane == 0) {
      if (mean_out) mean_out[row] = mean;
      if (rstd_out) rstd_out[row] = rstd;
    }
#pragma unroll
    for (int i = 0; i < NVEC; ++i) {
      const int c = (i * 32 + lane) * 8;
      float g[8], b[8], o[8];
      load8(gamma + c, g);
      load8(beta + c, b);
#pragma unroll
      for (int j = 0; j < 8; ++j) o[j] = g[j] * ((z[i][j] - mean) * rstd) + b[j];
      if (drop.mode == 2) {
        const uint32_t keep = keep8_mask(drop, (uint64_t)row * cols + c);
#pragma unroll
        for (int j = 0; j < 8; ++j) o[j] = ((keep >> j) & 1u) ? o[j] * drop.scale : 0.f;
      }
      store8(y + row * cols + c, o);
    }
  }
}

template <typename TIn>
static void launch_ln_fwd(int grid, cudaStream_t st, const TIn* x, const bf16* res, const float* gamma,
                          const float* beta, bf16* y, float* mean, float* rstd, int rows, int cols, float eps,
                          DropCfg drop) {
  const dim3 g(grid), b(LN_WARPS * 32);
  switch (cols >> 8) {
    case 1: launch_kernel(layernorm_fwd_kernel<TIn, 1>, g, b, 0, st, x, res, gamma, beta, y, mean, rstd, rows, eps, drop); break;
    case 2: launch_kernel(layernorm_fwd_kernel<TIn, 2>, g, b, 0, st, x, res, gamma, beta, y, mean, rstd, rows, eps, drop); break;
    case 3: launch_kernel(layernorm_fwd_kernel<TIn, 3>, g, b, 0, st, x, res, gamma, beta, y, mean, rstd, rows, eps, drop); break;
    default: launch_kernel(layernorm_fwd_kernel<TIn, 4>, g, b, 0, st, x, res, gamma, beta, y, mean, rstd, rows, eps, drop); break;
  }
}


template <typename TIn>
__device__ __forceinline__ void ln_bwd_load(const bf16* dy, const bf16* dy2, const TIn* x, const bf16* res,
                                            long long off, const DropCfg& drop, float (&z)[8], float (&d)[8],
                                            uint32_t& keep) {
  load8(x + off, z);
  keep = 0xffu;
  if (drop.mode != 0) keep = keep8_mask(drop, (uint64_t)off);
  if (drop.mode == 1) {
#pragma unroll
    for (int j = 0; j < 8; ++j) z[j] = ((keep >> j) & 1u) ? z[j] * drop.scale : 0.f;
  }
  if (res != nullptr) {
    float r[8];
    load8(res + off, r);
#pragma unroll
    for (int j = 0; j < 8; ++j) z[j] += r[j];
  }
  load8(dy + off, d);
  if (dy2 != nullptr) {
    float d2[8];
    load8(dy2 + off, d2);
#pragma unroll
    for (int j = 0; j < 8; ++j) d[j] += d2[j];
  }
  if (drop.mode == 2) {
#pragma unroll
    for (int j = 0; j < 8; ++j) d[j] = ((keep >> j) & 1u) ? d[j] * drop.scale : 0.f;
  }
}

constexpr int LNB_WARPS = 4;
__device__ __forceinline__ void acc8_add(float* p, const float (&v)[8]) {
  float4 a = *reinterpret_cast<float4*>(p), b = *reinterpret_cast<float4*>(p + 4);
  a.x += v[0]; a.y += v[1]; a.z += v[2]; a.w += v[3];
  b.x += v[4]; b.y += v[5]; b.z += v[6]; b.w += v[7];
  *reinterpret_cast<float4*>(p) = a;
  *reinterpret_cast<float4*>(p + 4) = b;
}
template <typename TIn, int NVEC>
__global__ void __launch_bounds__(LNB_WARPS * 32, NVEC <= 3 ? 5 : 3)
layernorm_bwd_kernel(const bf16* __restrict__ dy, const bf16* __restrict__ dy2, const TIn* __restrict__ x,
                     const bf16* __restrict__ res, const float* __restrict__ gamma, const float* __restrict__ mean_in,
                     const float* __restrict__ rstd_in, bf16* __restrict__ dx_res, bf16* __restrict__ dx_dense,
                     float* __restrict__ dgamma, float* __restrict__ dbeta, float* __restrict__ dbias, int rows,
                     DropCfg drop_in) {
  pdl_trigger();
  pdl_wait();
  const DropCfg drop = resolve_drop(drop_in);
  extern __shared__ __align__(16) float lnb_acc[];
  constexpr int cols = NVEC * 256;
  const int warp = threadIdx.x >> 5, lane = threadIdx.x & 31;
  const float inv_cols = 1.0f / (float)cols;
  const bool emit = dx_res != nullptr || dx_dense != nullptr || dbias != nullptr;
  float* my = lnb_acc + warp * 3 * cols;
  for (int k = lane * 4; k < 3 * cols; k += 128) *reinterpret_cast<float4*>(my + k) = make_float4(0.f, 0.f, 0.f, 0.f);
  __syncwarp();

  for (long long row = (long long)blockIdx.x * LNB_WARPS + warp; row < rows; row += (long long)gridDim.x * LNB_WARPS) {
    const float mean = mean_in[row], rstd = rstd_in[row];
    const float nm = -mean * rstd;
    float xh[NVEC][8], g[NVEC][8];
    uint32_t keep[NVEC];
    float s1 = 0.f, s2 = 0.f;
#pragma unroll
    for (int i = 0; i < NVEC; ++i) {
      const int c = (i * 32 + lane) * 8;
      float d[8], gm[8], dh[8];
      ln_bwd_load(dy, dy2, x, res, row * cols + c, drop, xh[i], d, keep[i]);
      load8(gamma + c, gm);
#pragma unroll
      for (int j = 0; j < 8; ++j) {
        const float h = fmaf(xh[i][j], rstd, nm);
        const float gg = d[j] * gm[j];
        s1 += gg;
        s2 = fmaf(gg, h, s2);
        dh[j] = d[j] * h;
        xh[i][j] = h;
        g[i][j] = gg;
      }
      acc8_add(my + c, dh);
      acc8_add(my + cols + c, d);
    }
    if (!emit) continue;
    s1 = warp_sum(s1);
    s2 = warp_sum(s2);
    const float a = -s1 * inv_cols * rstd, b = -s2 * inv_cols * rstd;
#pragma unroll
    for (int i = 0; i < NVEC; ++i) {
      const int c = (i * 32 + lane) * 8;
      float dz[8], dd[8];
#pragma unroll
      for (int j = 0; j < 8; ++j) {
        dz[j] = fmaf(xh[i][j], b, fmaf(g[i][j], rstd, a));
        dd[j] = (drop.mode == 1) ? (((keep[i] >> j) & 1u) ? dz[j] * drop.scale : 0.f) : dz[j];
      }
      if (dbias != nullptr) acc8_add(my + 2 * cols + c, dd);
      if (dx_res != nullptr) store8(dx_res + row * cols + c, dz);
      if (dx_dense != nullptr && dx_dense != dx_res) store8(dx_dense + row * cols + c, dd);
    }
  }
  __syncthreads();
  for (int which = 0; which < 3; ++which) {
    float* dst = which == 0 ? dgamma : which == 1 ? dbeta : dbias;
    if (dst == nullptr) continue;
    for (int e = threadIdx.x; e < cols; e += LNB_WARPS * 32) {
      float t = 0.f;
#pragma unroll
      for (int w = 0; w < LNB_WARPS; ++w) t += lnb_acc[(w * 3 + which) * cols + e];
      dst[(long long)blockIdx.x * cols + e] = t;
    }
  }
}

template <typename TIn>
static int launch_ln_bwd(int grid, cudaStream_t st, const bf16* dy, const bf16* dy2, const TIn* x, const bf16* res,
                         const float* gamma, const float* mean, const float* rstd, bf16* dx_res, bf16* dx_dense,
                         float* dgamma_out, float* dbeta_out, float* dbias_out, int rows, int cols, DropCfg drop) {
  const size_t smem = (size_t)LNB_WARPS * 3 * cols * sizeof(float);
  float* outs[3] = {dgamma_out, dbeta_out, dbias_out};
  float* parts[3] = {nullptr, nullptr, nullptr};
  for (int w = 0; w < 3; ++w)
    if (outs[w] != nullptr)
      if (int rc = scratch_alloc((void**)&parts[w], (size_t)grid * cols * sizeof(float), st)) return rc;
  float *dgamma = parts[0], *dbeta = parts[1], *dbias = parts[2];
  switch (cols >> 8) {
    case 1: launch_kernel(layernorm_bwd_kernel<TIn, 1>, dim3(grid), dim3(LNB_WARPS * 32), smem, st, dy, dy2, x, res, gamma, mean, rstd, dx_res, dx_dense, dgamma, dbeta, dbias, rows, drop); break;
    case 2: launch_kernel(layernorm_bwd_kernel<TIn, 2>, dim3(grid), dim3(LNB_WARPS * 32), smem, st, dy, dy2, x, res, gamma, mean, rstd, dx_res, dx_dense, dgamma, dbeta, dbias, rows, drop); break;
    case 3: launch_kernel(layernorm_bwd_kernel<TIn, 3>, dim3(grid), dim3(LNB_WARPS * 32), smem, st, dy, dy2, x, res, gamma, mean, rstd, dx_res, dx_dense, dgamma, dbeta, dbias, rows, drop); break;
    default: launch_kernel(layernorm_bwd_kernel<TIn, 4>, dim3(grid), dim3(LNB_WARPS * 32), smem, st, dy, dy2, x, res, gamma, mean, rstd, dx_res, dx_dense, dgamma, dbeta, dbias, rows, drop); break;
  }
  UNIVL_CHECK_LAUNCH("layernorm_bwd");
  for (int w = 0; w < 3; ++w)
    if (parts[w] != nullptr)
      if (int rc = partials_reduce(parts[w], grid, 1, cols, outs[w], cols, st)) return rc;
  return UNIVL_OK;
}

static int check_ln_shape(const char* what, int rows, int cols) {
  UNIVL_CHECK_ARG(rows >= 0 && cols > 0 && (cols % 256) == 0 && cols <= 256 * LN_MAX_VEC,
                  "%s: cols must be a multiple of 256 and <= %d (got rows=%d cols=%d)", what, 256 * LN_MAX_VEC, rows,
                  cols);
  return UNIVL_OK;
}

static DropCfg make_drop(int mode, float p, const unsigned long long* rng, unsigned long long stream) {
  DropCfg d;
  d.mode = (p > 0.f) ? mode : 0;
  d.threshold = dropout_threshold16(p);
  d.scale = (p > 0.f) ? 1.0f / (1.0f - p) : 1.0f;
  d.seed = 0;
  d.stream = stream;
  d.rng = rng;
  return d;
}

static int lnb_grid(int rows) {
  long long blocks = ((long long)rows + LNB_WARPS - 1) / LNB_WARPS;
  const long long cap = (long long)device_sms() * 5;
  return (int)(blocks < 1 ? 1 : (blocks > cap ? cap : blocks));
}
static int ln_grid(int rows) {
  long long blocks = ((long long)rows + LN_WARPS - 1) / LN_WARPS;
  const long long cap = (long long)device_sms() * 8;
  return (int)(blocks < 1 ? 1 : (blocks > cap ? cap : blocks));
}

}

using namespace univl;

extern "C" int univl_layernorm_fwd(const void* x, const void* res, const float* gamma, const float* beta, void* y,
                                   float* mean, float* rstd, int rows, int cols, float eps, float p_drop,
                                   int drop_mode, const unsigned long long* rng_state,
                                   unsigned long long stream_id, void* stream) {
  if (int rc = check_ln_shape("layernorm_fwd", rows, cols)) return rc;
  UNIVL_CHECK_ARG(x && gamma && beta && y, "layernorm_fwd: null pointer");
  UNIVL_CHECK_ARG(p_drop == 0.f || rng_state != nullptr, "layernorm_fwd: dropout needs rng_state");
  UNIVL_CHECK_ARG(p_drop >= 0.f && p_drop < 1.f && drop_mode >= 0 && drop_mode <= 2, "layernorm_fwd: bad dropout");
  if (rows == 0) return UNIVL_OK;
  launch_ln_fwd<bf16>(ln_grid(rows), (cudaStream_t)stream, (const bf16*)x, (const bf16*)res, gamma, beta, (bf16*)y, mean,
                      rstd, rows, cols, eps, make_drop(drop_mode, p_drop, rng_state, stream_id));
  UNIVL_CHECK_LAUNCH("layernorm_fwd");
  return UNIVL_OK;
}

extern "C" int univl_layernorm_bwd(const void* dy, const void* dy2, const void* x, const void* res,
                                   const float* gamma, const float* mean, const float* rstd, void* dx_res,
                                   void* dx_dense, float* dgamma, float* dbeta, float* dbias, int rows, int cols,
                                   float p_drop, int drop_mode, const unsigned long long* rng_state,
                                   unsigned long long stream_id, void* stream) {
  if (int rc = check_ln_shape("layernorm_bwd", rows, cols)) return rc;
  UNIVL_CHECK_ARG(dy && x && gamma && mean && rstd, "layernorm_bwd: null pointer");
  UNIVL_CHECK_ARG(p_drop == 0.f || rng_state != nullptr, "layernorm_bwd: dropout needs rng_state");
  UNIVL_CHECK_ARG(p_drop >= 0.f && p_drop < 1.f && drop_mode >= 0 && drop_mode <= 2, "layernorm_bwd: bad dropout");
  if (rows == 0) return UNIVL_OK;
  return launch_ln_bwd<bf16>(lnb_grid(rows), (cudaStream_t)stream, (const bf16*)dy, (const bf16*)dy2, (const bf16*)x,
                             (const bf16*)res, gamma, mean, rstd, (bf16*)dx_res, (bf16*)dx_dense, dgamma, dbeta, dbias,
                             rows, cols, make_drop(drop_mode, p_drop, rng_state, stream_id));
}

extern "C" int univl_layernorm_f32_fwd(const float* x, const float* gamma, const float* beta, void* y, float* mean,
                                       float* rstd, int rows, int cols, float eps, void* stream) {
  if (int rc = check_ln_shape("layernorm_f32_fwd", rows, cols)) return rc;
  UNIVL_CHECK_ARG(x && gamma && beta && y, "layernorm_f32_fwd: null pointer");
  if (rows == 0) return UNIVL_OK;
  launch_ln_fwd<float>(ln_grid(rows), (cudaStream_t)stream, x, (const bf16*)nullptr, gamma, beta, (bf16*)y, mean, rstd,
                       rows, cols, eps, make_drop(0, 0.f, nullptr, 0));
  UNIVL_CHECK_LAUNCH("layernorm_f32_fwd");
  return UNIVL_OK;
}

extern "C" int univl_layernorm_f32_bwd(const void* dy, const float* x, const float* gamma, const float* mean,
                                       const float* rstd, float* dgamma, float* dbeta, int rows, int cols,
                                       void* stream) {
  if (int rc = check_ln_shape("layernorm_f32_bwd", rows, cols)) return rc;
  UNIVL_CHECK_ARG(dy && x && gamma && mean && rstd && dgamma && dbeta, "layernorm_f32_bwd: null pointer");
  if (rows == 0) return UNIVL_OK;
  return launch_ln_bwd<float>(lnb_grid(rows), (cudaStream_t)stream, (const bf16*)dy, nullptr, x, nullptr, gamma, mean,
                              rstd, nullptr, nullptr, dgamma, dbeta, nullptr, rows, cols, make_drop(0, 0.f, nullptr, 0));
}
```

### univl_b200/csrc/misc.cu

```cuda
#include "common.cuh"

namespace univl {

__device__ __forceinline__ uint4 ld_nc_v4(const bf16* p) {
  uint4 u;
  asm volatile("ld.global.nc.L1::no_allocate.v4.u32 {%0, %1, %2, %3}, [%4];"
               : "=r"(u.x), "=r"(u.y), "=r"(u.z), "=r"(u.w) : "l"(p));
  return u;
}

__global__ void __launch_bounds__(256)
colsum_bf16_kernel(const bf16* __restrict__ x, long long ld, float* __restrict__ out, int rows, int cols,
                   int rows_per_block) {
  pdl_trigger();
  pdl_wait();
  __shared__ float red[8][257];
  const int cv = threadIdx.x & 31, rl = threadIdx.x >> 5;
  const int c0 = blockIdx.x * 256 + cv * 8;
  const int r_begin = blockIdx.y * rows_per_block;
  const int r_end = min(rows, r_begin + rows_per_block);
  float acc[8];
#pragma unroll
  for (int j = 0; j < 8; ++j) acc[j] = 0.f;
  auto add8 = [&](const uint4& u) {
    const uint32_t w[4] = {u.x, u.y, u.z, u.w};
#pragma unroll
    for (int j = 0; j < 4; ++j) {
      const float2 f = unpack_bf16x2(w[j]);
      acc[2 * j] += f.x;
      acc[2 * j + 1] += f.y;
    }
  };
  if (c0 < cols) {
    const bf16* base = x + c0;
    if (c0 + 8 <= cols && (ld & 7) == 0 && (reinterpret_cast<uintptr_t>(base) & 15) == 0) {
      int r = r_begin + rl;
      for (; r + 24 < r_end; r += 32) {
        uint4 u[4];
#pragma unroll
        for (int k = 0; k < 4; ++k) u[k] = ld_nc_v4(base + (long long)(r + 8 * k) * ld);
#pragma unroll
        for (int k = 0; k < 4; ++k) add8(u[k]);
      }
      for (; r < r_end; r += 8) add8(ld_nc_v4(base + (long long)r * ld));
    } else {
      for (int r = r_begin + rl; r < r_end; r += 8) {
        const bf16* p = base + (long long)r * ld;
#pragma unroll
        for (int j = 0; j < 8; ++j)
          if (c0 + j < cols) acc[j] += __bfloat162float(p[j]);
      }
    }
  }
#pragma unroll
  for (int j = 0; j < 8; ++j) red[rl][cv * 8 + j] = acc[j];
  __syncthreads();
  const int e = threadIdx.x;
  const int c = blockIdx.x * 256 + e;
  if (c < cols) {
    float t = 0.f;
#pragma unroll
    for (int w = 0; w < 8; ++w) t += red[w][e];
    out[(long long)blockIdx.y * cols + c] = t;
  }
}

__global__ void __launch_bounds__(256)
cast_f32_bf16_kernel(const float* __restrict__ src, bf16* __restrict__ dst, long long n) {
  const long long stride = (long long)gridDim.x * blockDim.x * 8;
  for (long long i = ((long long)blockIdx.x * blockDim.x + threadIdx.x) * 8; i < n; i += stride) {
    if (i + 8 <= n && (reinterpret_cast<uintptr_t>(src + i) & 15) == 0 && (reinterpret_cast<uintptr_t>(dst + i) & 15) == 0) {
      const float4 a = *reinterpret_cast<const float4*>(src + i);
      const float4 b = *reinterpret_cast<const float4*>(src + i + 4);
      uint4 u;
      u.x = pack_bf16x2(a.x, a.y); u.y = pack_bf16x2(a.z, a.w);
      u.z = pack_bf16x2(b.x, b.y); u.w = pack_bf16x2(b.z, b.w);
      *reinterpret_cast<uint4*>(dst + i) = u;
    } else {
      for (long long j = i; j < n && j < i + 8; ++j) dst[j] = __float2bfloat16(src[j]);
    }
  }
}

__global__ void __launch_bounds__(256)
multi_cast_kernel(const unsigned long long* __restrict__ table) {
  const float* src = reinterpret_cast<const float*>(table[3 * blockIdx.y]);
  bf16* dst = reinterpret_cast<bf16*>(table[3 * blockIdx.y + 1]);
  const long long n = (long long)table[3 * blockIdx.y + 2];
  const long long stride = (long long)gridDim.x * blockDim.x * 8;
  for (long long i = ((long long)blockIdx.x * blockDim.x + threadIdx.x) * 8; i < n; i += stride) {
    if (i + 8 <= n && (reinterpret_cast<uintptr_t>(src + i) & 15) == 0 && (reinterpret_cast<uintptr_t>(dst + i) & 15) == 0) {
      const float4 a = *reinterpret_cast<const float4*>(src + i);
      const float4 b = *reinterpret_cast<const float4*>(src + i + 4);
      uint4 u;
      u.x = pack_bf16x2(a.x, a.y); u.y = pack_bf16x2(a.z, a.w);
      u.z = pack_bf16x2(b.x, b.y); u.w = pack_bf16x2(b.z, b.w);
      *reinterpret_cast<uint4*>(dst + i) = u;
    } else {
      for (long long j = i; j < n && j < i + 8; ++j) dst[j] = __float2bfloat16(src[j]);
    }
  }
}

__global__ void __launch_bounds__(256)
eltwise_bf16_kernel(const bf16* __restrict__ dy, const bf16* __restrict__ x, bf16* __restrict__ out, long long n,
                    int mode) {
  const long long stride = (long long)gridDim.x * blockDim.x * 2;
  for (long long i = ((long long)blockIdx.x * blockDim.x + threadIdx.x) * 2; i < n; i += stride) {
    const bool pair = i + 1 < n;
    const float x0 = __bfloat162float(x[i]), x1 = pair ? __bfloat162float(x[i + 1]) : 0.f;
    const float d0 = dy ? __bfloat162float(dy[i]) : 0.f, d1 = (dy && pair) ? __bfloat162float(dy[i + 1]) : 0.f;
    float o0, o1;
    if (mode == 0) { o0 = d0 * gelu_erf_grad(x0); o1 = d1 * gelu_erf_grad(x1); }
    else if (mode == 1) { o0 = tanhf(x0); o1 = tanhf(x1); }
    else if (mode == 3) { o0 = gelu_erf(x0); o1 = gelu_erf(x1); }
    else { o0 = d0 * (1.f - x0 * x0); o1 = d1 * (1.f - x1 * x1); }
    out[i] = __float2bfloat16(o0);
    if (pair) out[i + 1] = __float2bfloat16(o1);
  }
}

__global__ void __launch_bounds__(256) fill_f32_kernel(float* __restrict__ p, float v, long long n) {
  const long long stride = (long long)gridDim.x * blockDim.x;
  for (long long i = (long long)blockIdx.x * blockDim.x + threadIdx.x; i < n; i += stride) p[i] = v;
}

__global__ void rng_advance_kernel(unsigned long long* state) { state[1] += 1; }

}

using namespace univl;

extern "C" int univl_rng_advance(unsigned long long* rng_state, void* stream) {
  UNIVL_CHECK_ARG(rng_state != nullptr, "rng_advance: null state");
  rng_advance_kernel<<<1, 1, 0, (cudaStream_t)stream>>>(rng_state);
  UNIVL_CHECK_LAUNCH("rng_advance");
  return UNIVL_OK;
}

extern "C" int univl_colsum_bf16(const void* x, long long ld, float* out, int rows, int cols, void* stream) {
  UNIVL_CHECK_ARG(x && out && rows >= 0 && cols > 0, "colsum: bad arguments");
  if (rows == 0) return UNIVL_OK;
  const int col_blocks = (cols + 255) / 256;
  int row_blocks = (device_sms() * 4 + col_blocks - 1) / col_blocks;
  if (row_blocks > (rows + 63) / 64) row_blocks = (rows + 63) / 64;
  if (row_blocks < 1) row_blocks = 1;
  const int rpb = (rows + row_blocks - 1) / row_blocks;
  row_blocks = (rows + rpb - 1) / rpb;
  float* part;
  if (int rc = scratch_alloc((void**)&part, (size_t)row_blocks * cols * sizeof(float), (cudaStream_t)stream)) return rc;
  launch_kernel(colsum_bf16_kernel, dim3(col_blocks, row_blocks), dim3(256), 0, (cudaStream_t)stream, (const bf16*)x, ld,
                part, rows, cols, rpb);
  UNIVL_CHECK_LAUNCH("colsum_bf16");
  return partials_reduce(part, row_blocks, 1, cols, out, cols, (cudaStream_t)stream);
}

extern "C" int univl_cast_f32_to_bf16(const float* src, void* dst, long long n, void* stream) {
  UNIVL_CHECK_ARG(src && dst && n >= 0, "cast: bad arguments");
  if (n == 0) return UNIVL_OK;
  long long blocks = (n + 2047) / 2048;
  if (blocks > device_sms() * 8) blocks = device_sms() * 8;
  cast_f32_bf16_kernel<<<(int)blocks, 256, 0, (cudaStream_t)stream>>>(src, (bf16*)dst, n);
  UNIVL_CHECK_LAUNCH("cast_f32_to_bf16");
  return UNIVL_OK;
}

namespace univl {
__global__ void __launch_bounds__(256) cast_bf16_f32_kernel(const bf16* __restrict__ src, float* __restrict__ dst, long long n) {
  const long long n8 = n >> 3;
  for (long long i = (long long)blockIdx.x * blockDim.x + threadIdx.x; i < n8; i += (long long)gridDim.x * blockDim.x) {
    const uint4 u = *reinterpret_cast<const uint4*>(src + i * 8);
    const float2 a = unpack_bf16x2(u.x), b = unpack_bf16x2(u.y), c = unpack_bf16x2(u.z), d = unpack_bf16x2(u.w);
    *reinterpret_cast<float4*>(dst + i * 8) = make_float4(a.x, a.y, b.x, b.y);
    *reinterpret_cast<float4*>(dst + i * 8 + 4) = make_float4(c.x, c.y, d.x, d.y);
  }
  if (blockIdx.x == 0)
    for (long long i = n8 * 8 + threadIdx.x; i < n; i += blockDim.x) dst[i] = __bfloat162float(src[i]);
}
}

extern "C" int univl_cast_bf16_to_f32(const void* src, float* dst, long long n, void* stream) {
  UNIVL_CHECK_ARG(src && dst && n >= 0, "cast: bad arguments");
  UNIVL_CHECK_ARG(((uintptr_t)src & 15) == 0 && ((uintptr_t)dst & 15) == 0, "cast_bf16_to_f32: 16-byte alignment");
  if (n == 0) return UNIVL_OK;
  long long blocks = (n + 2047) / 2048;
  if (blocks > device_sms() * 8) blocks = device_sms() * 8;
  cast_bf16_f32_kernel<<<(int)blocks, 256, 0, (cudaStream_t)stream>>>((const bf16*)src, dst, n);
  UNIVL_CHECK_LAUNCH("cast_bf16_to_f32");
  return UNIVL_OK;
}

extern "C" int univl_multi_cast_f32_to_bf16(const unsigned long long* device_table, int n_tensors, int blocks_per_tensor,
                                            void* stream) {
  UNIVL_CHECK_ARG(device_table && n_tensors >= 0 && blocks_per_tensor > 0, "multi_cast: bad arguments");
  if (n_tensors == 0) return UNIVL_OK;
  UNIVL_CHECK_ARG(n_tensors <= 65535, "multi_cast: too many tensors");
  multi_cast_kernel<<<dim3(blocks_per_tensor, n_tensors), 256, 0, (cudaStream_t)stream>>>(device_table);
  UNIVL_CHECK_LAUNCH("multi_cast_f32_to_bf16");
  return UNIVL_OK;
}

static int launch_eltwise(const void* dy, const void* x, void* out, long long n, int mode, void* stream) {
  if (n == 0) return UNIVL_OK;
  long long blocks = (n + 511) / 512;
  if (blocks > device_sms() * 8) blocks = device_sms() * 8;
  eltwise_bf16_kernel<<<(int)blocks, 256, 0, (cudaStream_t)stream>>>((const bf16*)dy, (const bf16*)x, (bf16*)out, n,
                                                                     mode);
  UNIVL_CHECK_LAUNCH("eltwise_bf16");
  return UNIVL_OK;
}
extern "C" int univl_gelu_bwd_bf16(const void* dy, const void* pre, void* out, long long n, void* stream) {
  UNIVL_CHECK_ARG(dy && pre && out && n >= 0, "gelu_bwd: bad arguments");
  return launch_eltwise(dy, pre, out, n, 0, stream);
}
extern "C" int univl_gelu_fwd_bf16(const void* x, void* out, long long n, void* stream) {
  UNIVL_CHECK_ARG(x && out && n >= 0, "gelu_fwd: bad arguments");
  return launch_eltwise(nullptr, x, out, n, 3, stream);
}
extern "C" int univl_tanh_fwd_bf16(const void* x, void* out, long long n, void* stream) {
  UNIVL_CHECK_ARG(x && out && n >= 0, "tanh_fwd: bad arguments");
  return launch_eltwise(nullptr, x, out, n, 1, stream);
}
extern "C" int univl_tanh_bwd_bf16(const void* dy, const void* y, void* out, long long n, void* stream) {
  UNIVL_CHECK_ARG(dy && y && out && n >= 0, "tanh_bwd: bad arguments");
  return launch_eltwise(dy, y, out, n, 2, stream);
}

extern "C" int univl_fill_f32(float* p, float value, long long n, void* stream) {
  UNIVL_CHECK_ARG(p && n >= 0, "fill: bad arguments");
  if (n == 0) return UNIVL_OK;
  if (value == 0.0f) {
    cudaError_t e = cudaMemsetAsync(p, 0, (size_t)n * sizeof(float), (cudaStream_t)stream);
    if (e != cudaSuccess) return set_error(UNIVL_ERR_CUDA, "fill memset: %s", cudaGetErrorString(e));
    return UNIVL_OK;
  }
  long long blocks = (n + 255) / 256;
  if (blocks > device_sms() * 16) blocks = device_sms() * 16;
  fill_f32_kernel<<<(int)blocks, 256, 0, (cudaStream_t)stream>>>(p, value, n);
  UNIVL_CHECK_LAUNCH("fill_f32");
  return UNIVL_OK;
}
```

### univl_b200/modules/module_cross.py

```python
import logging

import torch
from torch import nn

from .. import ops
from .. import runtime as rt
from .transformer import EncoderStack, Pooler, _layer_params, check_config, hidden_list
from .until_config import PretrainedConfig
from .until_module import LayerNorm, PreTrainedModel

logger = logging.getLogger(__name__)

PRETRAINED_MODEL_ARCHIVE_MAP = {}
CONFIG_NAME = "cross_config.json"
WEIGHTS_NAME = "cross_pytorch_model.bin"


class CrossConfig(PretrainedConfig):
    pretrained_model_archive_map = PRETRAINED_MODEL_ARCHIVE_MAP
    config_name = CONFIG_NAME
    weights_name = WEIGHTS_NAME

    def __init__(self, vocab_size_or_config_json_file, hidden_size=768, num_hidden_layers=12,
                 num_attention_heads=12, intermediate_size=3072, hidden_act="gelu", hidden_dropout_prob=0.1,
                 attention_probs_dropout_prob=0.1, max_position_embeddings=512, type_vocab_size=2,
                 initializer_range=0.02):
        self._init_from(vocab_size_or_config_json_file, dict(
            hidden_size=hidden_size, num_hidden_layers=num_hidden_layers, num_attention_heads=num_attention_heads,
            hidden_act=hidden_act, intermediate_size=intermediate_size, hidden_dropout_prob=hidden_dropout_prob,
            attention_probs_dropout_prob=attention_probs_dropout_prob,
            max_position_embeddings=max_position_embeddings, type_vocab_size=type_vocab_size,
            initializer_range=initializer_range))


class CrossEmbeddings(nn.Module):

    def __init__(self, config):
        super(CrossEmbeddings, self).__init__()
        self.position_embeddings = nn.Embedding(config.max_position_embeddings, config.hidden_size)
        self.token_type_embeddings = nn.Embedding(config.type_vocab_size, config.hidden_size)
        self.LayerNorm = LayerNorm(config.hidden_size, eps=1e-12)
        self.dropout = nn.Dropout(config.hidden_dropout_prob)

    def run(self, text2d, video2d, Nt, W, Nv, F, all_pairs):
        return ops.EmbedSrcFn.apply(text2d, video2d, Nt, W, Nv, F, all_pairs, self.position_embeddings.weight,
                                    self.token_type_embeddings.weight, self.LayerNorm.weight, self.LayerNorm.bias,
                                    self.dropout.p, self.training)


def _n_seq(Nt, Nv, groups):
    groups = int(groups)
    if groups and (Nt % groups or Nv % groups):
        raise ValueError("cross pairing: %d groups must divide %d text and %d video rows" % (groups, Nt, Nv))
    return Nt * Nv // groups if groups else Nt


class CrossModel(PreTrainedModel):

    def __init__(self, config):
        super(CrossModel, self).__init__(config)
        check_config(config)
        self.embeddings = CrossEmbeddings(config)
        self.encoder = EncoderStack(config)
        self.pooler = Pooler(config)
        self.apply(self.init_weights)

    def encode_pairs(self, text2d, video2d, text_mask, video_mask, all_pairs, keep_all=False):
        Nt, W = text_mask.shape
        Nv, F = video_mask.shape
        n_seq = _n_seq(Nt, Nv, all_pairs)
        x = self.embeddings.run(text2d, video2d, Nt, W, Nv, F, all_pairs)
        mask = ops.MaskSpec(text_mask, video_mask, all_pairs=all_pairs)
        return self.encoder.run(x, n_seq, W + F, mask, keep_all=keep_all), n_seq, W + F

    def encode_pairs_first_token(self, text2d, video2d, text_mask, video_mask, all_pairs):
        Nt, W = text_mask.shape
        Nv, F = video_mask.shape
        n_seq = _n_seq(Nt, Nv, all_pairs)
        x = self.embeddings.run(text2d, video2d, Nt, W, Nv, F, all_pairs)
        mask = ops.MaskSpec(text_mask, video_mask, all_pairs=all_pairs)
        return self.encoder.run_first_token(x, n_seq, W + F, mask), n_seq

    def first_layer_source_qkv(self, text2d, video2d, Nt, W, Nv, F):
        return self.first_layer_source_rows(text2d, video2d, Nt, W, Nv, F)[1]

    def first_layer_source_rows(self, text2d, video2d, Nt, W, Nv, F):
        emb = self.embeddings
        pos, typ = emb.position_embeddings.weight, emb.token_type_embeddings.weight
        gamma, beta = emb.LayerNorm.weight, emb.LayerNorm.bias
        rows_t = Nt * W
        x = torch.empty((rows_t + Nv * F, text2d.shape[1]), dtype=torch.bfloat16, device=text2d.device)
        ops.embed_src_rows_eval(text2d, Nt, W, pos, typ, gamma, beta, x[:rows_t])
        ops.embed_src_rows_eval(video2d, Nv, F, pos[W:], typ[1:], gamma, beta, x[rows_t:])
        a = self.encoder.layer[0].attention.self
        wqkv = rt.current().bf16_qkv(a.query.weight, a.key.weight, a.value.weight)
        return x, ops.linear_fwd(x, wqkv, rt.packed_bias(a.query.bias, a.key.bias, a.value.bias))

    def encode_pairs_first_token_eval(self, text2d, video2d, text_mask, video_mask, qkv_t, qkv_v):
        Nt, W = text_mask.shape
        Nv, F = video_mask.shape
        S = W + F
        x = self.embeddings.run(text2d, video2d, Nt, W, Nv, F, 1)
        mask = ops.MaskSpec(text_mask, video_mask, all_pairs=1)
        layers = self.encoder.layer
        x = ops.pair_layer_eval(x, qkv_t, qkv_v, Nt, Nv, S, mask, _layer_params(layers[0]), len(layers) == 1)
        if len(layers) == 1:
            return x
        return self.encoder.run_first_token(x, Nt * Nv, S, mask, start=1)

    def fp8_eval_weights(self):
        layers = self.encoder.layer
        out = []
        for i, layer in enumerate(layers):
            names = ("kv",) if i == len(layers) - 1 else ("o", "w1", "w2") if i == 0 else ("qkv", "o", "w1", "w2")
            out.append(ops.fp8_layer_weights(_layer_params(layer), names))
        return out

    def encode_pairs_first_token_eval_fp8(self, text2d, video2d, text_mask, video_mask, qkv_t, qkv_v, qw):
        Nt, W = text_mask.shape
        Nv, F = video_mask.shape
        S = W + F
        n_seq = Nt * Nv
        x = self.embeddings.run(text2d, video2d, Nt, W, Nv, F, 1)
        mask = ops.MaskSpec(text_mask, video_mask, all_pairs=1)
        layers = self.encoder.layer
        x = ops.pair_layer_eval_fp8(x, qkv_t, qkv_v, Nt, Nv, S, mask, _layer_params(layers[0]), qw[0])
        for i in range(1, len(layers) - 1):
            x = ops.encoder_layer_eval_fp8(x, n_seq, S, mask, _layer_params(layers[i]), qw[i])
        return ops.cls_layer_eval_fp8(x, n_seq, S, mask, _layer_params(layers[-1]), qw[-1])

    def encode_pairs_first_token_eval_packed(self, x, qkv, rows_t, seqs, qw=None):
        layers = self.encoder.layer
        h = ops.pair_layer_eval_packed(x[:rows_t], x[rows_t:], qkv[:rows_t], qkv[rows_t:], seqs,
                                       _layer_params(layers[0]), len(layers) == 1, qw[0] if qw else None)
        if len(layers) == 1:
            return h
        for i in range(1, len(layers) - 1):
            h = ops.encoder_layer_eval_packed(h, seqs, _layer_params(layers[i]), qw[i] if qw else None)
        return ops.cls_layer_eval_packed(h, seqs, _layer_params(layers[-1]), qw[-1] if qw else None)

    def forward(self, concat_input, concat_type=None, attention_mask=None, output_all_encoded_layers=True):
        N, S, _ = concat_input.shape
        if attention_mask is None:
            attention_mask = torch.ones(N, S, dtype=torch.long, device=concat_input.device)
        if concat_type is None:
            concat_type = torch.zeros_like(attention_mask)
        W = int((concat_type[0] == 0).sum().item())
        if not bool((concat_type[:, :W] == 0).all()) or not bool((concat_type[:, W:] == 1).all()):
            raise ValueError("CrossModel.forward: concat_type must be [0]*W + [1]*F for every row")
        with rt.use_model(self, concat_input.device):
            x = concat_input.to(torch.bfloat16)
            text = x[:, :W].contiguous().view(N * W, -1)
            video = x[:, W:].contiguous().view(N * (S - W), -1) if S > W else None
            am = attention_mask.long()
            outs, n_seq, S2 = self.encode_pairs(text, video, am[:, :W].contiguous(),
                                                am[:, W:].contiguous() if S > W else am[:, :0], False, keep_all=True)
            pooled = self.pooler.run(outs[-1], n_seq, S2)
            layers = hidden_list(outs, n_seq, S2)
            return (layers if output_all_encoded_layers else layers[-1]), pooled
```

### univl_b200/ops.py

```python
import math
import os

import torch

from . import lib
from . import runtime as rt
from .runtime import call, ptr

BF16 = torch.bfloat16
F32 = torch.float32
LN_EPS = 1e-12
HEADS = 12
LD_VOCAB_ALIGN = 64

EPI_BIAS, EPI_GELU, EPI_GELU_BWD, EPI_ADD, EPI_F32, EPI_ATOMIC = 0, 1, 2, 3, 4, 5


def _empty(shape, dtype, like):
    return torch.empty(shape, dtype=dtype, device=like.device)


def _zeros(shape, dtype, like):
    return torch.zeros(shape, dtype=dtype, device=like.device)


def _check2d(t, name):
    if t.dim() != 2 or t.stride(1) != 1:
        raise RuntimeError("univl_b200: %s must be a row-major 2-D tensor (got shape %s strides %s)"
                           % (name, tuple(t.shape), t.stride()))


class GradSink:

    def __init__(self):
        self.flat = rt.current_sink()

    def one(self, param):
        if param is None:
            return None, None
        if self.flat is not None and self.flat.has(param):
            return self.flat.grad_view(param), None
        t = torch.zeros(param.shape, dtype=F32, device=param.device)
        return t, t

    def packed(self, params):
        if self.flat is not None and all(self.flat.has(p) for p in params):
            v = self.flat.grad_view_packed(params)
            if v is not None:
                return v, [None] * len(params)
        rows = sum(p.shape[0] for p in params)
        t = torch.zeros((rows,) + tuple(params[0].shape[1:]), dtype=F32, device=params[0].device)
        outs, r = [], 0
        for p in params:
            outs.append(t[r:r + p.shape[0]])
            r += p.shape[0]
        return t, outs


def gemm(a, b, M, N, K, out, epi=EPI_BIAS, bias=None, aux_in=None, aux_out=None, a_mn=False, b_mn=False, alpha=1.0,
         block_n=0, split_k=0):
    _check2d(a, "gemm A"); _check2d(b, "gemm B"); _check2d(out, "gemm out")
    call("univl_gemm_bf16", a.data_ptr(), a.stride(0), int(a_mn), b.data_ptr(), b.stride(0), int(b_mn), M, N, K,
         out.data_ptr(), out.stride(0), epi, ptr(bias), ptr(aux_in), aux_in.stride(0) if aux_in is not None else 0,
         ptr(aux_out), aux_out.stride(0) if aux_out is not None else 0, float(alpha), block_n, split_k)
    return out


def linear_fwd(x, w16, bias, epi=EPI_BIAS, aux_out=None, out_dtype=BF16, ld_out=None):
    T, K = x.shape
    N = w16.shape[0]
    if ld_out is None:
        out = _empty((T, N), out_dtype, x)
    else:
        out = _empty((T, ld_out), out_dtype, x)[:, :N]
    return gemm(x, w16, T, N, K, out, epi=epi, bias=bias, aux_out=aux_out)


def linear_dgrad(dy, w16, epi=EPI_BIAS, aux_in=None):
    T, N = dy.shape
    K = w16.shape[1]
    out = _empty((T, K), BF16, dy)
    return gemm(dy, w16, T, K, N, out, epi=epi, aux_in=aux_in, b_mn=True)


def linear_wgrad(dy, x, dw=None):
    T, N = dy.shape
    K = x.shape[1]
    if dw is None:
        dw = _zeros((N, K), F32, dy)
    return gemm(dy, x, N, K, T, dw, epi=EPI_ATOMIC, a_mn=True, b_mn=True)


def colsum(x, out=None):
    rows, cols = x.shape
    if out is None:
        out = _zeros((cols,), F32, x)
    call("univl_colsum_bf16", x.data_ptr(), x.stride(0), out.data_ptr(), rows, cols)
    return out


def layernorm_fwd(x, res, gamma, beta, p=0.0, mode=0, seed=0, stream=0):
    rows, cols = x.shape
    y = _empty((rows, cols), BF16, x)
    mean = _empty((rows,), F32, x)
    rstd = _empty((rows,), F32, x)
    call("univl_layernorm_fwd", x.data_ptr(), ptr(res), gamma.data_ptr(), beta.data_ptr(), y.data_ptr(),
         mean.data_ptr(), rstd.data_ptr(), rows, cols, LN_EPS, float(p), mode, seed, stream)
    return y, mean, rstd


def layernorm_bwd(dy, dy2, x, res, gamma, mean, rstd, p=0.0, mode=0, seed=0, stream=0, want_dbias=True,
                  want_dx=True, dgamma=None, dbeta=None, dbias=None):
    rows, cols = x.shape
    dx_res = _empty((rows, cols), BF16, x) if want_dx else None
    dx_dense = _empty((rows, cols), BF16, x) if (want_dx and p > 0.0 and mode == 1) else dx_res
    dgamma = _zeros((cols,), F32, x) if dgamma is None else dgamma
    dbeta = _zeros((cols,), F32, x) if dbeta is None else dbeta
    if dbias is None and want_dbias:
        dbias = _zeros((cols,), F32, x)
    call("univl_layernorm_bwd", dy.data_ptr(), ptr(dy2), x.data_ptr(), ptr(res), gamma.data_ptr(), mean.data_ptr(),
         rstd.data_ptr(), ptr(dx_res), ptr(dx_dense), dgamma.data_ptr(), dbeta.data_ptr(), ptr(dbias), rows, cols,
         float(p), mode, seed, stream)
    return dx_res, dx_dense, dgamma, dbeta, dbias


class MaskSpec:

    def __init__(self, mask_a=None, mask_b=None, all_pairs=False, causal=False):
        self.a = mask_a.contiguous() if mask_a is not None else None
        self.b = mask_b.contiguous() if mask_b is not None else None
        self.all_pairs = int(all_pairs)
        self.causal = bool(causal)
        for m in (self.a, self.b):
            if m is not None and m.dtype != torch.int64:
                raise RuntimeError("univl_b200: masks must be int64 (as the reference dataloaders emit them)")

    @property
    def Wa(self):
        return self.a.shape[1] if self.a is not None else 0

    @property
    def Fb(self):
        return self.b.shape[1] if self.b is not None else 0

    @property
    def Nb(self):
        return self.b.shape[0] if self.b is not None else 0


SHORT_ATTN_MAX_S = 256


def _attention_entry(kind, Sq, Sk):
    if Sq > SHORT_ATTN_MAX_S or Sk > SHORT_ATTN_MAX_S:
        return "univl_attention_long_" + kind
    return "univl_attention_" + kind


def attention_fwd(q, k, v, n_seq, Sq, Sk, mask, p=0.0, seed=0, stream=0):
    o = _empty((n_seq * Sq, HEADS * 64), BF16, q)
    lse = _empty((n_seq * HEADS * Sq,), F32, q)
    call(_attention_entry("fwd", Sq, Sk), q.data_ptr(), q.stride(0), k.data_ptr(), k.stride(0), v.data_ptr(),
         v.stride(0), o.data_ptr(), o.stride(0), lse.data_ptr(), ptr(mask.a), ptr(mask.b), mask.Wa, mask.Fb, mask.Nb,
         int(mask.all_pairs), n_seq, HEADS, Sq, Sk, int(mask.causal), 1.0 / math.sqrt(64.0), float(p), seed, stream)
    return o, lse


def fused_attention_supported(n_seq, S, H):
    if os.environ.get("UNIVL_FUSED_ATTN", "1") == "0":
        return False
    from . import lib
    return bool(lib.load().univl_fused_qkv_attention_supported(int(n_seq), HEADS, int(S), int(H)))


def fused_qkv_attention_fwd(x, wqkv, bqkv, n_seq, S, mask, p=0.0, seed=0, stream=0, save_qkv=True):
    T, H = x.shape
    _check2d(x, "fused attention x"); _check2d(wqkv, "fused attention wqkv")
    o = _empty((T, H), BF16, x)
    lse = _empty((n_seq * HEADS * S,), F32, x)
    qkv = _empty((T, 3 * H), BF16, x) if save_qkv else None
    call("univl_fused_qkv_attention_fwd", x.data_ptr(), x.stride(0), wqkv.data_ptr(), wqkv.stride(0), bqkv.data_ptr(),
         ptr(qkv), 3 * H, o.data_ptr(), o.stride(0), lse.data_ptr(), ptr(mask.a), ptr(mask.b), mask.Wa, mask.Fb,
         mask.Nb, int(mask.all_pairs), n_seq, HEADS, S, int(mask.causal), 1.0 / math.sqrt(64.0), float(p), seed, stream)
    return o, lse, qkv


def fused_attention_bwd(qkv, o, lse, d_o, dqkv, n_seq, S, mask, p=0.0, seed=0, stream=0, dbias=None):
    call("univl_fused_attention_bwd", qkv.data_ptr(), qkv.stride(0), o.data_ptr(), o.stride(0), lse.data_ptr(),
         d_o.data_ptr(), d_o.stride(0), dqkv.data_ptr(), dqkv.stride(0), ptr(dbias), ptr(mask.a), ptr(mask.b), mask.Wa,
         mask.Fb, mask.Nb, int(mask.all_pairs), n_seq, HEADS, S, int(mask.causal), 1.0 / math.sqrt(64.0), float(p), seed,
         stream)


def attention_bwd(q, k, v, o, lse, d_o, dq, dk, dv, n_seq, Sq, Sk, mask, p=0.0, seed=0, stream=0, dbias=None,
                  rng_layout=0):
    dbq, dbk, dbv = dbias if dbias is not None else (None, None, None)
    entry = _attention_entry("bwd", Sq, Sk)
    assert rng_layout == 0 or entry == "univl_attention_bwd", (rng_layout, Sq, Sk)
    call(entry, q.data_ptr(), q.stride(0), k.data_ptr(), k.stride(0), v.data_ptr(), v.stride(0),
         o.data_ptr(), o.stride(0), lse.data_ptr(), d_o.data_ptr(), d_o.stride(0), dq.data_ptr(), dq.stride(0),
         dk.data_ptr(), dk.stride(0), dv.data_ptr(), dv.stride(0), ptr(mask.a), ptr(mask.b), mask.Wa, mask.Fb,
         mask.Nb, int(mask.all_pairs), n_seq, HEADS, Sq, Sk, int(mask.causal), 1.0 / math.sqrt(64.0), float(p), seed,
         stream, int(rng_layout), ptr(dbq), ptr(dbk), ptr(dbv))


def attention_pair_fwd(qkv_a, qkv_b, Na, Nb, Sq, mask):
    H = HEADS * 64
    o = _empty((Na * Nb * Sq, H), BF16, qkv_a)
    call("univl_attention_pair_fwd", qkv_a.data_ptr(), qkv_a.stride(0), qkv_a[:, H:].data_ptr(), qkv_a.stride(0),
         qkv_a[:, 2 * H:].data_ptr(), qkv_a.stride(0), qkv_b.data_ptr(), qkv_b.stride(0), qkv_b[:, H:].data_ptr(),
         qkv_b.stride(0), qkv_b[:, 2 * H:].data_ptr(), qkv_b.stride(0), o.data_ptr(), o.stride(0), None, ptr(mask.a),
         ptr(mask.b), Na, mask.Wa, Nb, mask.Fb, HEADS, Sq, 1.0 / math.sqrt(64.0))
    return o


def embed_src_rows_eval(a, N, W, pos, type_w, gamma, beta, out):
    mean = _empty((N * W,), F32, a)
    rstd = _empty((N * W,), F32, a)
    call("univl_embed_src_fwd", a.data_ptr(), None, pos.data_ptr(), type_w.data_ptr(), gamma.data_ptr(),
         beta.data_ptr(), out.data_ptr(), mean.data_ptr(), rstd.data_ptr(), N, W, 0, 0, 0, a.shape[1], LN_EPS, 0.0,
         None, 0)
    return out


def pair_layer_eval(x, qkv_a, qkv_b, Na, Nb, S, mask, params, first_token):
    arena = rt.current()
    wa = dict(zip(ATT_KEYS, params[:10]))
    wf = dict(zip(FFN_KEYS, params[10:16]))
    drop = _Drop(0.0, 0.0, False)
    n_seq = Na * Nb
    ctx = attention_pair_fwd(qkv_a, qkv_b, Na, Nb, 1 if first_token else S, mask)
    xq = x.view(n_seq, S, -1)[:, 0].contiguous() if first_token else x
    ao = linear_fwd(ctx, arena.bf16(wa["o"]), wa["bo"])
    y, _, _ = layernorm_fwd(ao, xq, wa["gamma"], wa["beta"], 0.0, 1, drop.seed, drop.stream())
    return ffn_block_fwd(y, wf, drop)[0]


E4M3 = torch.float8_e4m3fn
FP8_EPI_BIAS, FP8_EPI_GELU = 0, 1


def quantize_e4m3_rows(x):
    _check2d(x, "quantize_e4m3_rows x")
    M, K = x.shape
    q = _empty((M, K), E4M3, x)
    s = _empty((K // 128, M), F32, x)
    call("univl_quantize_e4m3_rows", x.data_ptr(), x.stride(0), q.data_ptr(), q.stride(0), s.data_ptr(), M, K)
    return q, s


def quantize_e4m3_blocks(w, q=None, s=None):
    _check2d(w, "quantize_e4m3_blocks w")
    N, K = w.shape
    q = _empty((N, K), E4M3, w) if q is None else q
    s = _empty((N // 128, K // 128), F32, w) if s is None else s
    call("univl_quantize_e4m3_blocks", w.data_ptr(), w.stride(0), q.data_ptr(), q.stride(0), s.data_ptr(), N, K)
    return q, s


def gemm_fp8(a, a_scale, b, b_scale, bias, gelu=False):
    _check2d(a, "gemm_fp8 A"); _check2d(b, "gemm_fp8 B")
    M, K = a.shape
    N = b.shape[0]
    if gelu:
        out = _empty((M, N), E4M3, a)
        out_s = _empty((N // 128, M), F32, a)
    else:
        out = _empty((M, N), BF16, a)
        out_s = None
    call("univl_gemm_fp8", a.data_ptr(), a.stride(0), a_scale.data_ptr(), b.data_ptr(), b.stride(0),
         b_scale.data_ptr(), M, N, K, FP8_EPI_GELU if gelu else FP8_EPI_BIAS, bias.data_ptr(), out.data_ptr(),
         out.stride(0), ptr(out_s))
    return (out, out_s) if gelu else out


def fp8_layer_weights(params, names):
    wa = dict(zip(ATT_KEYS, params[:10]))
    wf = dict(zip(FFN_KEYS, params[10:16]))
    H = wa["q"].shape[1]

    def stacked(ws):
        q = _empty((len(ws) * H, H), E4M3, ws[0])
        s = _empty((len(ws) * H // 128, H // 128), F32, ws[0])
        for i, w in enumerate(ws):
            quantize_e4m3_blocks(w, q[i * H:(i + 1) * H], s[i * H // 128:(i + 1) * H // 128])
        return q, s

    make = {"qkv": lambda: stacked((wa["q"], wa["k"], wa["v"])), "kv": lambda: stacked((wa["k"], wa["v"])),
            "o": lambda: quantize_e4m3_blocks(wa["o"]), "w1": lambda: quantize_e4m3_blocks(wf["w1"]),
            "w2": lambda: quantize_e4m3_blocks(wf["w2"])}
    return {n: make[n]() for n in names}


def _fp8_layer_tail(ctx, x, params, qw):
    wa = dict(zip(ATT_KEYS, params[:10]))
    wf = dict(zip(FFN_KEYS, params[10:16]))
    drop = _Drop(0.0, 0.0, False)
    ao = gemm_fp8(*quantize_e4m3_rows(ctx), *qw["o"], wa["bo"])
    y, _, _ = layernorm_fwd(ao, x, wa["gamma"], wa["beta"], 0.0, 1, drop.seed, drop.stream())
    h, hs = gemm_fp8(*quantize_e4m3_rows(y), *qw["w1"], wf["b1"], gelu=True)
    fo = gemm_fp8(h, hs, *qw["w2"], wf["b2"])
    out, _, _ = layernorm_fwd(fo, y, wf["gamma"], wf["beta"], 0.0, 1, drop.seed, drop.stream())
    return out


def pair_layer_eval_fp8(x, qkv_a, qkv_b, Na, Nb, S, mask, params, qw):
    ctx = attention_pair_fwd(qkv_a, qkv_b, Na, Nb, S, mask)
    return _fp8_layer_tail(ctx, x, params, qw)


def encoder_layer_eval_fp8(x, n_seq, S, mask, params, qw):
    wa = dict(zip(ATT_KEYS, params[:10]))
    H = x.shape[1]
    qkv = gemm_fp8(*quantize_e4m3_rows(x), *qw["qkv"], rt.packed_bias(wa["bq"], wa["bk"], wa["bv"]))
    drop = _Drop(0.0, 0.0, False)
    ctx, _ = attention_fwd(qkv[:, :H], qkv[:, H:2 * H], qkv[:, 2 * H:], n_seq, S, S, mask, 0.0, drop.seed,
                           drop.stream())
    return _fp8_layer_tail(ctx, x, params, qw)


def cls_layer_eval_fp8(x, n_seq, S, mask, params, qw):
    arena = rt.current()
    wa = dict(zip(ATT_KEYS, params[:10]))
    wf = dict(zip(FFN_KEYS, params[10:16]))
    drop = _Drop(0.0, 0.0, False)
    H = x.shape[1]
    x0 = x.view(n_seq, S, H)[:, 0].contiguous()
    kv = gemm_fp8(*quantize_e4m3_rows(x), *qw["kv"], rt.packed_bias(wa["bk"], wa["bv"]))
    q = linear_fwd(x0, arena.bf16_qkv(wa["q"], wa["k"], wa["v"])[:H], wa["bq"])
    ctx, _ = attention_fwd(q, kv[:, :H], kv[:, H:], n_seq, 1, S, mask, 0.0, drop.seed, drop.stream())
    ao = linear_fwd(ctx, arena.bf16(wa["o"]), wa["bo"])
    y, _, _ = layernorm_fwd(ao, x0, wa["gamma"], wa["beta"], 0.0, 1, drop.seed, drop.stream())
    return ffn_block_fwd(y, wf, drop)[0]


I32 = torch.int32


def _exclusive_cumsum(n):
    out = torch.zeros(n.numel() + 1, dtype=torch.int64, device=n.device)
    torch.cumsum(n, 0, out=out[1:])
    return out


class VarlenSeqs:

    def __init__(self, cu, total, max_sk, idx_a=None, idx_b=None, start_a=None, start_b=None, len_a=None):
        self.cu, self.total, self.max_sk = cu, int(total), int(max_sk)
        self.idx_a, self.idx_b, self.start_a, self.start_b, self.len_a = idx_a, idx_b, start_a, start_b, len_a
        self.n_seq = cu.numel() - 1

    def packed(self):
        return VarlenSeqs(self.cu, self.total, self.max_sk)

    def index_args(self):
        return (ptr(self.idx_a), ptr(self.idx_b), ptr(self.start_a), ptr(self.start_b), ptr(self.len_a),
                self.cu.data_ptr())


def _valid_rows(m, n):
    flat = m.reshape(-1)
    slot = torch.where(flat, torch.cumsum(flat, 0) - 1, n)
    out = torch.empty(n + 1, dtype=I32, device=m.device)
    out.scatter_(0, slot, torch.arange(flat.numel(), dtype=I32, device=m.device))
    return out[:n]


class PairPacking:

    def __init__(self, text_mask, video_mask):
        tm, vm = text_mask != 0, video_mask != 0
        self.text_shape, self.video_shape = tuple(tm.shape), tuple(vm.shape)
        nt, nv = tm.sum(1), vm.sum(1)
        token0 = tm[:, 0].all().view(1) if tm.shape[1] else torch.zeros(1, dtype=torch.bool, device=tm.device)
        host = torch.cat([nt, nv, token0.long()]).cpu().tolist()
        Nt = tm.shape[0]
        self.len_t, self.len_v = host[:Nt], host[Nt:-1]
        self.token0_valid = bool(host[-1])
        self.idx_t = _valid_rows(tm, sum(self.len_t))
        self.idx_v = _valid_rows(vm, sum(self.len_v))
        self.start_t = _exclusive_cumsum(nt)[:-1].to(I32)
        self.start_v = _exclusive_cumsum(nv)[:-1].to(I32)
        self.n_t, self.n_v = nt.to(I32), nv.to(I32)
        self.max_sk = max(self.len_t, default=0) + max(self.len_v, default=0)

    def tokens(self, t0, t1, v0, v1):
        return (v1 - v0) * sum(self.len_t[t0:t1]) + (t1 - t0) * sum(self.len_v[v0:v1])

    def tile(self, t0, t1, v0, v1):
        nt, nv = t1 - t0, v1 - v0
        len_a = self.n_t[t0:t1].repeat_interleave(nv)
        len_b = self.n_v[v0:v1].repeat(nt)
        cu = _exclusive_cumsum(len_a.long() + len_b.long()).to(I32)
        return VarlenSeqs(cu, self.tokens(t0, t1, v0, v1), self.max_sk, self.idx_t, self.idx_v,
                          self.start_t[t0:t1].repeat_interleave(nv), self.start_v[v0:v1].repeat(nt), len_a)


def attention_varlen_fwd(q, k, v, seqs, q_first, qb=None, kb=None, vb=None):
    o = _empty((seqs.n_seq if q_first else seqs.total, HEADS * 64), BF16, q)
    if o.shape[0] == 0:
        return o
    b = (qb, kb, vb) if seqs.idx_a is not None else (None, None, None)
    call("univl_attention_varlen_fwd", q.data_ptr(), q.stride(0), k.data_ptr(), k.stride(0), v.data_ptr(),
         v.stride(0), ptr(b[0]), b[0].stride(0) if b[0] is not None else 0, ptr(b[1]),
         b[1].stride(0) if b[1] is not None else 0, ptr(b[2]), b[2].stride(0) if b[2] is not None else 0,
         *seqs.index_args(), seqs.n_seq, seqs.max_sk, HEADS, int(q_first), o.data_ptr(), o.stride(0), None,
         1.0 / math.sqrt(64.0))
    return o


def gather_rows_varlen(a, b, seqs, q_first):
    _check2d(a, "gather_rows_varlen a")
    out = _empty((seqs.n_seq if q_first else seqs.total, a.shape[1]), BF16, a)
    if out.shape[0] == 0:
        return out
    call("univl_gather_rows_varlen", a.data_ptr(), a.stride(0), ptr(b), b.stride(0) if b is not None else 0,
         *seqs.index_args(), seqs.n_seq, int(q_first), a.shape[1], out.data_ptr(), out.stride(0))
    return out


def _split_qkv(qkv):
    H = qkv.shape[1] // 3
    return qkv[:, :H], qkv[:, H:2 * H], qkv[:, 2 * H:]


def _attn_out(ctx, x, params):
    wa = dict(zip(ATT_KEYS, params[:10]))
    drop = _Drop(0.0, 0.0, False)
    ao = linear_fwd(ctx, rt.current().bf16(wa["o"]), wa["bo"])
    return layernorm_fwd(ao, x, wa["gamma"], wa["beta"], 0.0, 1, drop.seed, drop.stream())[0]


def _ffn(y, params):
    return ffn_block_fwd(y, dict(zip(FFN_KEYS, params[10:16])), _Drop(0.0, 0.0, False))[0]


def pair_layer_eval_packed(x_a, x_b, qkv_a, qkv_b, seqs, params, first_token, qw=None):
    xq = gather_rows_varlen(x_a, x_b, seqs, first_token)
    ctx = attention_varlen_fwd(*_split_qkv(qkv_a), seqs, first_token, *_split_qkv(qkv_b))
    if qw is not None:
        return _fp8_layer_tail(ctx, xq, params, qw)
    y = _attn_out(ctx, xq, params)
    del ctx, xq
    return _ffn(y, params)


def encoder_layer_eval_packed(x, seqs, params, qw=None):
    wa = dict(zip(ATT_KEYS, params[:10]))
    bias = rt.packed_bias(wa["bq"], wa["bk"], wa["bv"])
    if qw is None:
        qkv = linear_fwd(x, rt.current().bf16_qkv(wa["q"], wa["k"], wa["v"]), bias)
    else:
        qkv = gemm_fp8(*quantize_e4m3_rows(x), *qw["qkv"], bias)
    ctx = attention_varlen_fwd(*_split_qkv(qkv), seqs.packed(), False)
    del qkv
    if qw is not None:
        return _fp8_layer_tail(ctx, x, params, qw)
    y = _attn_out(ctx, x, params)
    del ctx
    return _ffn(y, params)


def cls_layer_eval_packed(x, seqs, params, qw=None):
    arena = rt.current()
    wa = dict(zip(ATT_KEYS, params[:10]))
    H = x.shape[1]
    wqkv = arena.bf16_qkv(wa["q"], wa["k"], wa["v"])
    bias = rt.packed_bias(wa["bk"], wa["bv"])
    if qw is None:
        kv = linear_fwd(x, wqkv[H:], bias)
    else:
        kv = gemm_fp8(*quantize_e4m3_rows(x), *qw["kv"], bias)
    packed = seqs.packed()
    x0 = gather_rows_varlen(x, None, packed, True)
    q = linear_fwd(x0, wqkv[:H], wa["bq"])
    ctx = attention_varlen_fwd(q, kv[:, :H], kv[:, H:], packed, True)
    del kv
    return _ffn(_attn_out(ctx, x0, params), params)


class _Drop:

    def __init__(self, p_hidden, p_attn, training):
        arena = rt.current()
        self.ph = float(p_hidden) if training else 0.0
        self.pa = float(p_attn) if training else 0.0
        self.seed = arena.seed
        self.arena = arena
        self.epoch = arena.epoch_host

    def stream(self):
        return self.arena.next_stream()


def attn_block_fwd(xq, xkv, n_seq, Sq, Sk, mask, w, drop, need_bwd=True):
    arena = rt.current()
    H = xq.shape[1]
    self_attn = xkv is xq
    sv = {"self": self_attn, "fused": False}
    wqkv = arena.bf16_qkv(w["q"], w["k"], w["v"])
    ctx = None
    if self_attn and fused_attention_supported(n_seq, Sq, H):
        sa, sd = drop.stream(), drop.stream()
        ctx, lse, qkv = fused_qkv_attention_fwd(xq, wqkv, rt.packed_bias(w["bq"], w["bk"], w["bv"]), n_seq, Sq, mask,
                                                drop.pa, drop.seed, sa, save_qkv=need_bwd)
        sv["qkv"] = qkv
        sv["fused"] = True
    elif self_attn:
        qkv = linear_fwd(xq, wqkv, rt.packed_bias(w["bq"], w["bk"], w["bv"]))
        q, k, v = qkv[:, :H], qkv[:, H:2 * H], qkv[:, 2 * H:]
        sv["qkv"] = qkv
    else:
        q = linear_fwd(xq, wqkv[:H], w["bq"])
        kv = linear_fwd(xkv, wqkv[H:], rt.packed_bias(w["bk"], w["bv"]))
        k, v = kv[:, :H], kv[:, H:]
        sv["q"], sv["kv"] = q, kv
    if ctx is None:
        sa, sd = drop.stream(), drop.stream()
        ctx, lse = attention_fwd(q, k, v, n_seq, Sq, Sk, mask, drop.pa, drop.seed, sa)
    ao = linear_fwd(ctx, arena.bf16(w["o"]), w["bo"])
    y, mean, rstd = layernorm_fwd(ao, xq, w["gamma"], w["beta"], drop.ph, 1, drop.seed, sd)
    sv.update(xq=xq, xkv=xkv, ctx=ctx, lse=lse, ao=ao, mean=mean, rstd=rstd, sa=sa, sd=sd, n_seq=n_seq, Sq=Sq, Sk=Sk,
              mask=mask, pa=drop.pa, ph=drop.ph, seed=drop.seed, wqkv=wqkv, wo=arena.bf16(w["o"]),
              gamma=w["gamma"], w=w, sink=GradSink(), arena=arena, epoch=drop.epoch)
    return y, sv


def attn_block_bwd(dy, dy2, sv, need_dxkv=True):
    H = sv["xq"].shape[1]
    sv["arena"].check_epoch(sv["epoch"], max(sv["pa"], sv["ph"]))
    w, sink = sv["w"], sv["sink"]
    dgamma, r_gamma = sink.one(w["gamma"])
    dbeta, r_beta = sink.one(w["beta"])
    dbo, r_bo = sink.one(w["bo"])
    g, gd, _, _, _ = layernorm_bwd(dy, dy2, sv["ao"], sv["xq"], sv["gamma"], sv["mean"], sv["rstd"], sv["ph"], 1,
                                   sv["seed"], sv["sd"], dgamma=dgamma, dbeta=dbeta, dbias=dbo)
    dwo, r_o = sink.one(w["o"])
    linear_wgrad(gd, sv["ctx"], dwo)
    dctx = linear_dgrad(gd, sv["wo"])
    T, Tk = sv["xq"].shape[0], sv["xkv"].shape[0]
    dwqkv, r_w = sink.packed((w["q"], w["k"], w["v"]))
    dbqkv, r_b = sink.packed((w["bq"], w["bk"], w["bv"]))
    if sv["self"]:
        qkv = sv["qkv"]
        dqkv = _empty((T, 3 * H), BF16, dy)
        if sv["fused"] and os.environ.get("UNIVL_FUSED_ATTN_BWD", "1") != "0":
            fused_attention_bwd(qkv, sv["ctx"], sv["lse"], dctx, dqkv, sv["n_seq"], sv["Sq"], sv["mask"], sv["pa"],
                                sv["seed"], sv["sa"], dbias=dbqkv)
        else:
            attention_bwd(qkv[:, :H], qkv[:, H:2 * H], qkv[:, 2 * H:], sv["ctx"], sv["lse"], dctx, dqkv[:, :H],
                          dqkv[:, H:2 * H], dqkv[:, 2 * H:], sv["n_seq"], sv["Sq"], sv["Sk"], sv["mask"], sv["pa"],
                          sv["seed"], sv["sa"], dbias=(dbqkv[:H], dbqkv[H:2 * H], dbqkv[2 * H:]),
                          rng_layout=1 if sv["fused"] else 0)
        linear_wgrad(dqkv, sv["xq"], dwqkv)
        dxq = linear_dgrad(dqkv, sv["wqkv"], epi=EPI_ADD, aux_in=g)
        dxkv = None
    else:
        q, kv = sv["q"], sv["kv"]
        dq = _empty((T, H), BF16, dy)
        dkv = _empty((Tk, 2 * H), BF16, dy)
        attention_bwd(q, kv[:, :H], kv[:, H:], sv["ctx"], sv["lse"], dctx, dq, dkv[:, :H], dkv[:, H:], sv["n_seq"],
                      sv["Sq"], sv["Sk"], sv["mask"], sv["pa"], sv["seed"], sv["sa"],
                      dbias=(dbqkv[:H], dbqkv[H:2 * H], dbqkv[2 * H:]))
        linear_wgrad(dq, sv["xq"], dwqkv[:H])
        linear_wgrad(dkv, sv["xkv"], dwqkv[H:])
        dxq = linear_dgrad(dq, sv["wqkv"][:H], epi=EPI_ADD, aux_in=g)
        dxkv = linear_dgrad(dkv, sv["wqkv"][H:]) if need_dxkv else None
    rets = {"q": r_w[0], "k": r_w[1], "v": r_w[2], "bq": r_b[0], "bk": r_b[1], "bv": r_b[2], "o": r_o, "bo": r_bo,
            "gamma": r_gamma, "beta": r_beta}
    return dxq, dxkv, rets


def ffn_block_fwd(x, w, drop):
    arena = rt.current()
    w1, w2 = arena.bf16(w["w1"]), arena.bf16(w["w2"])
    T = x.shape[0]
    pre = _empty((T, w1.shape[0]), BF16, x)
    h = linear_fwd(x, w1, w["b1"], epi=EPI_GELU, aux_out=pre)
    fo = linear_fwd(h, w2, w["b2"])
    sd = drop.stream()
    y, mean, rstd = layernorm_fwd(fo, x, w["gamma"], w["beta"], drop.ph, 1, drop.seed, sd)
    sv = dict(x=x, pre=pre, h=h, fo=fo, mean=mean, rstd=rstd, sd=sd, ph=drop.ph, seed=drop.seed, w1=w1, w2=w2,
              gamma=w["gamma"], w=w, sink=GradSink(), arena=arena, epoch=drop.epoch)
    return y, sv


def ffn_block_bwd(dy, sv):
    w, sink = sv["w"], sv["sink"]
    sv["arena"].check_epoch(sv["epoch"], sv["ph"])
    dgamma, r_gamma = sink.one(w["gamma"])
    dbeta, r_beta = sink.one(w["beta"])
    db2, r_b2 = sink.one(w["b2"])
    g, gd, _, _, _ = layernorm_bwd(dy, None, sv["fo"], sv["x"], sv["gamma"], sv["mean"], sv["rstd"], sv["ph"], 1,
                                   sv["seed"], sv["sd"], dgamma=dgamma, dbeta=dbeta, dbias=db2)
    dw2, r_w2 = sink.one(w["w2"])
    linear_wgrad(gd, sv["h"], dw2)
    dpre = linear_dgrad(gd, sv["w2"], epi=EPI_GELU_BWD, aux_in=sv["pre"])
    db1, r_b1 = sink.one(w["b1"])
    colsum(dpre, db1)
    dw1, r_w1 = sink.one(w["w1"])
    linear_wgrad(dpre, sv["x"], dw1)
    dx = linear_dgrad(dpre, sv["w1"])
    return g, dx, {"w1": r_w1, "b1": r_b1, "w2": r_w2, "b2": r_b2, "gamma": r_gamma, "beta": r_beta}


ATT_KEYS = ("q", "bq", "k", "bk", "v", "bv", "o", "bo", "gamma", "beta")
FFN_KEYS = ("w1", "b1", "w2", "b2", "gamma", "beta")


class EncoderLayerFn(torch.autograd.Function):

    @staticmethod
    def forward(ctx, x, n_seq, S, mask, p_hidden, p_attn, training, *params):
        wa = dict(zip(ATT_KEYS, params[:10]))
        wf = dict(zip(FFN_KEYS, params[10:16]))
        drop = _Drop(p_hidden, p_attn, training)
        y1, sva = attn_block_fwd(x, x, n_seq, S, S, mask, wa, drop, need_bwd=any(ctx.needs_input_grad))
        y2, svf = ffn_block_fwd(y1, wf, drop)
        ctx.sva, ctx.svf = sva, svf
        return y2

    @staticmethod
    def backward(ctx, dy):
        dy = dy.contiguous()
        g2, dy1, gf = ffn_block_bwd(dy, ctx.svf)
        dx, _, ga = attn_block_bwd(dy1, g2, ctx.sva)
        ctx.sva = ctx.svf = None
        return (dx, None, None, None, None, None, None) + tuple(ga[k] for k in ATT_KEYS) + \
            tuple(gf[k] for k in FFN_KEYS)


class EncoderLayerClsFn(torch.autograd.Function):

    @staticmethod
    def forward(ctx, x, n_seq, S, mask, p_hidden, p_attn, training, *params):
        wa = dict(zip(ATT_KEYS, params[:10]))
        wf = dict(zip(FFN_KEYS, params[10:16]))
        drop = _Drop(p_hidden, p_attn, training)
        H = x.shape[1]
        xq = x.view(n_seq, S, H)[:, 0].contiguous()
        y1, sva = attn_block_fwd(xq, x, n_seq, 1, S, mask, wa, drop)
        y2, svf = ffn_block_fwd(y1, wf, drop)
        ctx.sva, ctx.svf = sva, svf
        ctx.shape = (n_seq, S, H)
        return y2

    @staticmethod
    def backward(ctx, dy):
        dy = dy.contiguous()
        n_seq, S, H = ctx.shape
        g2, dy1, gf = ffn_block_bwd(dy, ctx.svf)
        dxq, dxkv, ga = attn_block_bwd(dy1, g2, ctx.sva)
        dxkv.view(n_seq, S, H)[:, 0].add_(dxq)
        ctx.sva = ctx.svf = None
        return (dxkv, None, None, None, None, None, None) + tuple(ga[k] for k in ATT_KEYS) + \
            tuple(gf[k] for k in FFN_KEYS)


class DecoderLayerFn(torch.autograd.Function):

    @staticmethod
    def forward(ctx, x, enc, n_seq, L, Se, slf_mask, enc_mask, p_hidden, p_attn, training, *params):
        ws = dict(zip(ATT_KEYS, params[:10]))
        we = dict(zip(ATT_KEYS, params[10:20]))
        wf = dict(zip(FFN_KEYS, params[20:26]))
        drop = _Drop(p_hidden, p_attn, training)
        s, svs = attn_block_fwd(x, x, n_seq, L, L, slf_mask, ws, drop, need_bwd=any(ctx.needs_input_grad))
        d, sve = attn_block_fwd(s, enc, n_seq, L, Se, enc_mask, we, drop)
        y, svf = ffn_block_fwd(d, wf, drop)
        ctx.svs, ctx.sve, ctx.svf = svs, sve, svf
        ctx.need_enc = enc.requires_grad
        return y

    @staticmethod
    def backward(ctx, dy):
        dy = dy.contiguous()
        g3, dd, gf = ffn_block_bwd(dy, ctx.svf)
        ds, denc, ge = attn_block_bwd(dd, g3, ctx.sve, need_dxkv=ctx.need_enc)
        dx, _, gs = attn_block_bwd(ds, None, ctx.svs)
        ctx.svs = ctx.sve = ctx.svf = None
        return (dx, denc) + (None,) * 8 + tuple(gs[k] for k in ATT_KEYS) + tuple(ge[k] for k in ATT_KEYS) + \
            tuple(gf[k] for k in FFN_KEYS)


class VideoNormFn(torch.autograd.Function):

    @staticmethod
    def forward(ctx, video, gamma, beta):
        x = video.reshape(-1, video.shape[-1])
        rows, cols = x.shape
        y = _empty((rows, cols), BF16, x)
        mean = _empty((rows,), F32, x)
        rstd = _empty((rows,), F32, x)
        call("univl_layernorm_f32_fwd", x.data_ptr(), gamma.data_ptr(), beta.data_ptr(), y.data_ptr(),
             mean.data_ptr(), rstd.data_ptr(), rows, cols, LN_EPS)
        ctx.save_for_backward(x, gamma, beta, mean, rstd)
        ctx.sink = GradSink()
        return y.view(video.shape)

    @staticmethod
    def backward(ctx, dy):
        x, gamma, beta, mean, rstd = ctx.saved_tensors
        dy = dy.contiguous().view(x.shape)
        dgamma, r_g = ctx.sink.one(gamma)
        dbeta, r_b = ctx.sink.one(beta)
        call("univl_layernorm_f32_bwd", dy.data_ptr(), x.data_ptr(), gamma.data_ptr(), mean.data_ptr(),
             rstd.data_ptr(), dgamma.data_ptr(), dbeta.data_ptr(), x.shape[0], x.shape[1])
        return None, r_g, r_b


class EmbedTextFn(torch.autograd.Function):

    @staticmethod
    def forward(ctx, ids, type_ids, word, pos, type_w, gamma, beta, p, training):
        n_seq, S = ids.shape
        H = word.shape[1]
        arena = rt.current()
        p = float(p) if training else 0.0
        stream = arena.next_stream()
        ids = ids.contiguous()
        type_ids = type_ids.contiguous() if type_ids is not None else None
        y = _empty((n_seq * S, H), BF16, word)
        mean = _empty((n_seq * S,), F32, word)
        rstd = _empty((n_seq * S,), F32, word)
        call("univl_embed_text_fwd", ids.data_ptr(), ptr(type_ids), word.data_ptr(), pos.data_ptr(), ptr(type_w),
             gamma.data_ptr(), beta.data_ptr(), y.data_ptr(), mean.data_ptr(), rstd.data_ptr(), n_seq, S, H,
             word.shape[0], LN_EPS, p, arena.seed, stream)
        ctx.save_for_backward(ids, type_ids, word, pos, type_w, gamma, beta, mean, rstd)
        ctx.cfg = (n_seq, S, H, p, arena.seed, stream)
        ctx.sink = GradSink()
        return y

    @staticmethod
    def backward(ctx, dy):
        ids, type_ids, word, pos, type_w, gamma, beta, mean, rstd = ctx.saved_tensors
        n_seq, S, H, p, seed, stream = ctx.cfg
        dy = dy.contiguous()
        dword, r_word = ctx.sink.one(word)
        dpos, r_pos = ctx.sink.one(pos)
        dtype, r_type = ctx.sink.one(type_w)
        dgamma, r_g = ctx.sink.one(gamma)
        dbeta, r_b = ctx.sink.one(beta)
        call("univl_embed_text_bwd", dy.data_ptr(), ids.data_ptr(), ptr(type_ids), word.data_ptr(), pos.data_ptr(),
             ptr(type_w), gamma.data_ptr(), mean.data_ptr(), rstd.data_ptr(), dword.data_ptr(), dpos.data_ptr(),
             ptr(dtype), dgamma.data_ptr(), dbeta.data_ptr(), n_seq, S, H, word.shape[0], p, seed, stream)
        return None, None, r_word, r_pos, r_type, r_g, r_b, None, None


class EmbedSrcFn(torch.autograd.Function):

    @staticmethod
    def forward(ctx, a, b, Na, Wa, Nb, Fb, all_pairs, pos, type_w, gamma, beta, p, training):
        arena = rt.current()
        H = a.shape[1]
        p = float(p) if training else 0.0
        stream = arena.next_stream()
        all_pairs = int(all_pairs)
        n_seq = Na * Nb // all_pairs if (all_pairs and Fb > 0) else Na
        rows = n_seq * (Wa + Fb)
        y = _empty((rows, H), BF16, a)
        mean = _empty((rows,), F32, a)
        rstd = _empty((rows,), F32, a)
        call("univl_embed_src_fwd", a.data_ptr(), ptr(b), pos.data_ptr(), ptr(type_w), gamma.data_ptr(),
             beta.data_ptr(), y.data_ptr(), mean.data_ptr(), rstd.data_ptr(), Na, Wa, Nb, Fb, all_pairs, H,
             LN_EPS, p, arena.seed, stream)
        ctx.save_for_backward(a, b, pos, type_w, gamma, beta, mean, rstd)
        ctx.cfg = (Na, Wa, Nb, Fb, all_pairs, H, p, arena.seed, stream)
        ctx.sink = GradSink()
        return y

    @staticmethod
    def backward(ctx, dy):
        a, b, pos, type_w, gamma, beta, mean, rstd = ctx.saved_tensors
        Na, Wa, Nb, Fb, all_pairs, H, p, seed, stream = ctx.cfg
        dy = dy.contiguous()
        da = _empty(a.shape, BF16, a)
        db = _empty(b.shape, BF16, a) if b is not None else None
        dpos, r_pos = ctx.sink.one(pos)
        dtype, r_type = ctx.sink.one(type_w)
        dgamma, r_g = ctx.sink.one(gamma)
        dbeta, r_b = ctx.sink.one(beta)
        call("univl_embed_src_bwd", dy.data_ptr(), a.data_ptr(), ptr(b), pos.data_ptr(), ptr(type_w),
             gamma.data_ptr(), mean.data_ptr(), rstd.data_ptr(), da.data_ptr(), ptr(db), dpos.data_ptr(),
             ptr(dtype), dgamma.data_ptr(), dbeta.data_ptr(), Na, Wa, Nb, Fb, all_pairs, H, p, seed, stream)
        return da, db, None, None, None, None, None, r_pos, r_type, r_g, r_b, None, None


class LinearFn(torch.autograd.Function):

    @staticmethod
    def forward(ctx, x, weight, bias, gelu, needs_dx):
        arena = rt.current()
        w16 = arena.bf16(weight)
        T = x.shape[0]
        pre = None
        if gelu:
            pre = _empty((T, w16.shape[0]), BF16, x)
            y = linear_fwd(x, w16, bias, epi=EPI_GELU, aux_out=pre)
        else:
            y = linear_fwd(x, w16, bias)
        ctx.save_for_backward(x, w16, pre, weight, bias)
        ctx.needs_dx = needs_dx
        ctx.sink = GradSink()
        return y

    @staticmethod
    def backward(ctx, dy):
        x, w16, pre, weight, bias = ctx.saved_tensors
        dy = dy.contiguous()
        if pre is not None:
            dy = gelu_bwd(dy, pre)
        db, r_b = ctx.sink.one(bias)
        if db is not None:
            colsum(dy, db)
        dw, r_w = ctx.sink.one(weight)
        linear_wgrad(dy, x, dw)
        dx = linear_dgrad(dy, w16) if ctx.needs_dx else None
        return dx, r_w, r_b, None, None


class LinearTFn(torch.autograd.Function):

    @staticmethod
    def forward(ctx, x, weight, bias):
        w16 = rt.current().bf16(weight)
        T, K = x.shape
        N = w16.shape[1]
        y = _empty((T, N), BF16, x)
        gemm(x, w16, T, N, K, y, bias=bias, b_mn=True)
        ctx.save_for_backward(x, w16, weight, bias)
        ctx.sink = GradSink()
        return y

    @staticmethod
    def backward(ctx, dy):
        x, w16, weight, bias = ctx.saved_tensors
        dy = dy.contiguous()
        T, K = x.shape
        N = w16.shape[1]
        dx = _empty((T, K), BF16, x)
        gemm(dy, w16, T, K, N, dx)
        dw, r_w = ctx.sink.one(weight)
        gemm(x, dy, K, N, T, dw, epi=EPI_ATOMIC, a_mn=True, b_mn=True)
        db, r_b = ctx.sink.one(bias)
        colsum(dy, db)
        return dx, r_w, r_b


def gelu_bwd(dy, pre):
    out = _empty(dy.shape, BF16, dy)
    call("univl_gelu_bwd_bf16", dy.data_ptr(), pre.data_ptr(), out.data_ptr(), dy.numel())
    return out


class TanhFn(torch.autograd.Function):

    @staticmethod
    def forward(ctx, x):
        x = x.contiguous()
        y = _empty(x.shape, BF16, x)
        call("univl_tanh_fwd_bf16", x.data_ptr(), y.data_ptr(), x.numel())
        ctx.save_for_backward(y)
        return y

    @staticmethod
    def backward(ctx, dy):
        (y,) = ctx.saved_tensors
        out = _empty(y.shape, BF16, y)
        dy = dy.contiguous()
        call("univl_tanh_bwd_bf16", dy.data_ptr(), y.data_ptr(), out.data_ptr(), y.numel())
        return out


class LayerNormFn(torch.autograd.Function):

    @staticmethod
    def forward(ctx, x, gamma, beta):
        y, mean, rstd = layernorm_fwd(x, None, gamma, beta)
        ctx.save_for_backward(x, gamma, beta, mean, rstd)
        ctx.sink = GradSink()
        return y

    @staticmethod
    def backward(ctx, dy):
        x, gamma, beta, mean, rstd = ctx.saved_tensors
        dgamma, r_g = ctx.sink.one(gamma)
        dbeta, r_b = ctx.sink.one(beta)
        dx, _, _, _, _ = layernorm_bwd(dy.contiguous(), None, x, None, gamma, mean, rstd, want_dbias=False,
                                       dgamma=dgamma, dbeta=dbeta)
        return dx, r_g, r_b


def _ld_pad(n):
    return (n + LD_VOCAB_ALIGN - 1) // LD_VOCAB_ALIGN * LD_VOCAB_ALIGN


VOCAB_LOSS_MODES = ("logits", "fused")


def vocab_loss_mode():
    value = os.environ.get("UNIVL_VOCAB_LOSS", "logits")
    if value not in VOCAB_LOSS_MODES:
        raise ValueError("UNIVL_VOCAB_LOSS must be one of %s, got %r" % ("/".join(VOCAB_LOSS_MODES), value))
    return value


def vocab_xent_fwd(x, w16, bias, labels, groups):
    _check2d(x, "vocab_xent x"); _check2d(w16, "vocab_xent W")
    T, K = x.shape
    V = w16.shape[0]
    nbytes = lib.load().univl_vocab_xent_workspace(T, V)
    if nbytes < 0:
        raise RuntimeError("univl_vocab_xent_workspace failed: %s" % lib.load().univl_last_error_string().decode())
    ws = _empty((nbytes,), torch.uint8, x)
    lse = _empty((T,), F32, x)
    sc = _empty((2 * groups,), F32, x)
    loss = _empty((), F32, x)
    call("univl_vocab_xent_fwd", x.data_ptr(), x.stride(0), w16.data_ptr(), w16.stride(0), ptr(bias),
         labels.data_ptr(), lse.data_ptr(), sc.data_ptr(), loss.data_ptr(), ws.data_ptr(), ws.numel(), T, V, K, groups)
    return loss, lse, sc


def vocab_xent_bwd(x, w16, bias, labels, lse, sc, g, groups):
    T, K = x.shape
    V = w16.shape[0]
    ld = _ld_pad(V)
    dl = _empty((T, ld), BF16, x)
    call("univl_vocab_xent_bwd", x.data_ptr(), x.stride(0), w16.data_ptr(), w16.stride(0), ptr(bias),
         labels.data_ptr(), lse.data_ptr(), sc.data_ptr(), ptr(g), dl.data_ptr(), ld, T, V, K, groups)
    return dl


class ProjXentFn(torch.autograd.Function):

    @staticmethod
    def forward(ctx, x, W, bias, labels, pair_mask, target_mode, w_is_param, return_logits, groups):
        arena = rt.current()
        w16 = arena.bf16(W) if w_is_param else W
        T, K = x.shape
        fused = vocab_loss_mode() == "fused" and target_mode == 0 and pair_mask is None and not return_logits
        if fused:
            labels = labels.contiguous()
            loss, lse, sc = vocab_xent_fwd(x, w16, bias, labels, groups)
            ctx.save_for_backward(x, w16, None, labels, None, lse, sc, W if w_is_param else None, bias)
            ctx.cfg = (target_mode, w_is_param, bias is not None, groups, False)
            ctx.sink = GradSink()
            return loss
        windowed = target_mode == 1 and groups > 1
        if windowed and (w_is_param or w16.shape[0] != T or T % groups):
            raise ValueError("grouped NCE needs one frame row per scored row and T divisible by the %d groups" % groups)
        V = T // groups if windowed else w16.shape[0]
        ld = _ld_pad(V)
        logits = _empty((T, ld), F32, x)[:, :V]
        if windowed:
            for g in range(groups):
                rows = slice(g * V, (g + 1) * V)
                gemm(x[rows], w16[rows], V, V, K, logits[rows], epi=EPI_F32, bias=bias)
        else:
# ... 165 lines not shown
```

Measured before the change: 1445.

## Pack padded sequences and bound GEMM/layernorm work by device-side live row count

Adds a packed-row path for encoder layers in which only live (unpadded) tokens are processed. GEMM kernels read a device-side live row count and shrink M and the work count, and layernorm forward/backward and colsum take row maps so dropout indices stay consistent with the padded layout. Weight gradients expand the packed rows back to the padded layout and keep the full-size GEMMs. This cuts the FLOPs and bandwidth spent on padding tokens. In exchange it adds gather/expand kernels, extra template instantiations, and layernorm launch bounds that give fewer blocks per SM on the live variants.

```diff
diff --git a/include/univl_b200.h b/include/univl_b200.h
--- a/include/univl_b200.h
+++ b/include/univl_b200.h
@@ -16,6 +16,10 @@
                     const void* aux_in, long long ld_aux_in, void* aux_out, long long ld_aux_out, float alpha,
                     int block_n, int split_k, void* stream);
 int univl_gemm_plan(int M, int N, int Kc, int epilogue, int block_n, int split_k);
+int univl_gemm_bf16_live(const void* A, long long lda, int a_mn_major, const void* B, long long ldb, int b_mn_major,
+                         int M, int N, int Kc, void* out, long long ldo, int epilogue, const float* bias,
+                         const void* aux_in, long long ld_aux_in, void* aux_out, long long ld_aux_out, float alpha,
+                         int block_n, int split_k, const int* live, void* stream);
 
 int univl_quantize_e4m3_rows(const void* x, long long ldx, void* q, long long ldq, float* scale, int M, int K,
                              void* stream);
@@ -32,6 +36,15 @@
                         const float* mean, const float* rstd, void* dx_res, void* dx_dense, float* dgamma,
                         float* dbeta, float* dbias, int rows, int cols, float p_drop, int drop_mode,
                         const unsigned long long* rng_state, unsigned long long stream_id, void* stream);
+int univl_layernorm_fwd_rows(const void* x, const void* res, const float* gamma, const float* beta, void* y,
+                             float* mean, float* rstd, int rows, int cols, float eps, float p_drop, int drop_mode,
+                             const unsigned long long* rng_state, unsigned long long stream_id, const int* live,
+                             const int* row_map, void* stream);
+int univl_layernorm_bwd_rows(const void* dy, const void* dy2, const void* x, const void* res, const float* gamma,
+                             const float* mean, const float* rstd, void* dx_res, void* dx_dense, float* dgamma,
+                             float* dbeta, float* dbias, int rows, int cols, float p_drop, int drop_mode,
+                             const unsigned long long* rng_state, unsigned long long stream_id, const int* pos,
+                             void* stream);
 int univl_layernorm_f32_fwd(const float* x, const float* gamma, const float* beta, void* y, float* mean, float* rstd,
                             int rows, int cols, float eps, void* stream);
 int univl_layernorm_f32_bwd(const void* dy, const float* x, const float* gamma, const float* mean, const float* rstd,
@@ -104,6 +117,11 @@
                               const unsigned long long* rng_state, unsigned long long stream_id, void* stream);
 
 int univl_colsum_bf16(const void* x, long long ld, float* out, int rows, int cols, void* stream);
+int univl_colsum_bf16_rows(const void* x, long long ld, float* out, int rows, int cols, const int* pos, void* stream);
+int univl_rows_gather(const void* src, long long lds, const int* idx, const int* live, int rows, int cols, void* out,
+                      long long ldo, void* stream);
+int univl_rows_expand(const void* src, long long lds, const int* pos, int rows, int cols, void* out, long long ldo,
+                      void* stream);
 int univl_cast_f32_to_bf16(const float* src, void* dst, long long n, void* stream);
 int univl_cast_bf16_to_f32(const void* src, float* dst, long long n, void* stream);
 int univl_multi_cast_f32_to_bf16(const unsigned long long* device_table, int n_tensors, int blocks_per_tensor,
diff --git a/univl_b200/csrc/gemm_wgmma.cu b/univl_b200/csrc/gemm_wgmma.cu
--- a/univl_b200/csrc/gemm_wgmma.cu
+++ b/univl_b200/csrc/gemm_wgmma.cu
@@ -428,9 +428,8 @@
 }
 
 template <int BLOCK_N, int STAGES, bool A_MN, bool B_MN>
-__global__ void __launch_bounds__(PIPELINE_THREADS, 1)
-gemm_wgmma_kernel(const __grid_constant__ CUtensorMap tmap_a, const __grid_constant__ CUtensorMap tmap_b,
-                  const GemmParams p, const int num_work) {
+__device__ __forceinline__ void gemm_body(const CUtensorMap& tmap_a, const CUtensorMap& tmap_b, const GemmParams& p,
+                                          const int num_work) {
   using L = GemmSmem<BLOCK_N, STAGES>;
   constexpr bool PING = BLOCK_N <= 128;
   constexpr bool FOLD = BLOCK_N == 64;
@@ -526,25 +525,52 @@
   }
 }
 
-template <int BLOCK_N, int STAGES, bool A_MN, bool B_MN>
-static int launch_gemm(const CUtensorMap& ta, const CUtensorMap& tb, const GemmParams& p, int splits,
+enum GemmLive : int { LIVE_NONE = 0, LIVE_M = 1 };
+
+template <int BLOCK_N, int STAGES, bool A_MN, bool B_MN, int LIVE>
+__global__ void __launch_bounds__(PIPELINE_THREADS, 1)
+gemm_wgmma_kernel(const __grid_constant__ CUtensorMap tmap_a, const __grid_constant__ CUtensorMap tmap_b,
+                  const GemmParams p_in, const int num_work_in, const int* __restrict__ live) {
+  if constexpr (LIVE == LIVE_NONE) {
+    gemm_body<BLOCK_N, STAGES, A_MN, B_MN>(tmap_a, tmap_b, p_in, num_work_in);
+  } else {
+    GemmParams p = p_in;
+    p.M = min(max(0, *live), p_in.M);
+    const int num_work = ((p.M + BLOCK_M - 1) / BLOCK_M) * ((p.N + BLOCK_N - 1) / BLOCK_N);
+    gemm_body<BLOCK_N, STAGES, A_MN, B_MN>(tmap_a, tmap_b, p, num_work);
+  }
+}
+
+template <int BLOCK_N, int STAGES, bool A_MN, bool B_MN, int LIVE>
+static int launch_gemm(const CUtensorMap& ta, const CUtensorMap& tb, const GemmParams& p, int splits, const int* live,
                        cudaStream_t stream) {
   using L = GemmSmem<BLOCK_N, STAGES>;
-  auto kern = gemm_wgmma_kernel<BLOCK_N, STAGES, A_MN, B_MN>;
+  auto kern = gemm_wgmma_kernel<BLOCK_N, STAGES, A_MN, B_MN, LIVE>;
   const char* name = "univl_gemm_bf16";
   if (int rc = persistent_prepare(kern, L::DYN_BYTES, name)) return rc;
   const long long work =
       (long long)((p.M + BLOCK_M - 1) / BLOCK_M) * ((p.N + BLOCK_N - 1) / BLOCK_N) * (long long)splits;
-  return persistent_launch(kern, name, work, L::DYN_BYTES, stream, ta, tb, p, (int)work);
+  return persistent_launch(kern, name, work, L::DYN_BYTES, stream, ta, tb, p, (int)work, live);
+}
+
+template <int BLOCK_N, int STAGES, int LIVE>
+static int dispatch_major(bool a_mn, bool b_mn, const CUtensorMap& ta, const CUtensorMap& tb, const GemmParams& p,
+                          int splits, const int* live, cudaStream_t stream) {
+  if (!a_mn && !b_mn) return launch_gemm<BLOCK_N, STAGES, false, false, LIVE>(ta, tb, p, splits, live, stream);
+  if (!a_mn && b_mn) return launch_gemm<BLOCK_N, STAGES, false, true, LIVE>(ta, tb, p, splits, live, stream);
+  if (a_mn && b_mn) return launch_gemm<BLOCK_N, STAGES, true, true, LIVE>(ta, tb, p, splits, live, stream);
+  return launch_gemm<BLOCK_N, STAGES, true, false, LIVE>(ta, tb, p, splits, live, stream);
 }
 
 template <int BLOCK_N, int STAGES>
-static int dispatch_major(bool a_mn, bool b_mn, const CUtensorMap& ta, const CUtensorMap& tb, const GemmParams& p,
-                          int splits, cudaStream_t stream) {
-  if (!a_mn && !b_mn) return launch_gemm<BLOCK_N, STAGES, false, false>(ta, tb, p, splits, stream);
-  if (!a_mn && b_mn) return launch_gemm<BLOCK_N, STAGES, false, true>(ta, tb, p, splits, stream);
-  if (a_mn && b_mn) return launch_gemm<BLOCK_N, STAGES, true, true>(ta, tb, p, splits, stream);
-  return launch_gemm<BLOCK_N, STAGES, true, false>(ta, tb, p, splits, stream);
+static int dispatch_live(int live_mode, bool a_mn, bool b_mn, const CUtensorMap& ta, const CUtensorMap& tb,
+                         const GemmParams& p, int splits, const int* live, cudaStream_t stream) {
+  if (live_mode == LIVE_M) {
+    UNIVL_CHECK_ARG(!a_mn, "gemm_live: live M rows need a K-major A");
+    if (b_mn) return launch_gemm<BLOCK_N, STAGES, false, true, LIVE_M>(ta, tb, p, splits, live, stream);
+    return launch_gemm<BLOCK_N, STAGES, false, false, LIVE_M>(ta, tb, p, splits, live, stream);
+  }
+  return dispatch_major<BLOCK_N, STAGES, LIVE_NONE>(a_mn, b_mn, ta, tb, p, splits, nullptr, stream);
 }
 
 enum Fp8Epilogue : int { FP8_EPI_BIAS_BF16 = 0, FP8_EPI_GELU_E4M3 = 1 };
@@ -1007,10 +1033,10 @@
   return 1;
 }
 
-extern "C" int univl_gemm_bf16(const void* A, long long lda, int a_mn_major, const void* B, long long ldb,
-                               int b_mn_major, int M, int N, int Kc, void* out, long long ldo, int epilogue,
-                               const float* bias, const void* aux_in, long long ld_aux_in, void* aux_out,
-                               long long ld_aux_out, float alpha, int block_n, int split_k, void* stream_) {
+static int gemm_bf16(const void* A, long long lda, int a_mn_major, const void* B, long long ldb, int b_mn_major, int M,
+                     int N, int Kc, void* out, long long ldo, int epilogue, const float* bias, const void* aux_in,
+                     long long ld_aux_in, void* aux_out, long long ld_aux_out, float alpha, int block_n, int split_k,
+                     const int* live, int live_mode, void* stream_) {
   cudaStream_t stream = reinterpret_cast<cudaStream_t>(stream_);
   UNIVL_CHECK_ARG(M > 0 && N > 0 && Kc > 0, "gemm: empty problem M=%d N=%d K=%d", M, N, Kc);
   UNIVL_CHECK_ARG(A && B && out, "gemm: null operand");
@@ -1055,11 +1081,30 @@
   }
 
   const bool amn = a_mn_major != 0, bmn = b_mn_major != 0;
-  if (bn == 256) rc = dispatch_major<256, 4>(amn, bmn, ta, tb, p, plan.splits, stream);
-  else if (bn == 128) rc = dispatch_major<128, 6>(amn, bmn, ta, tb, p, plan.splits, stream);
-  else rc = dispatch_major<64, 8>(amn, bmn, ta, tb, p, plan.splits, stream);
+  if (bn == 256) rc = dispatch_live<256, 4>(live_mode, amn, bmn, ta, tb, p, plan.splits, live, stream);
+  else if (bn == 128) rc = dispatch_live<128, 6>(live_mode, amn, bmn, ta, tb, p, plan.splits, live, stream);
+  else rc = dispatch_live<64, 8>(live_mode, amn, bmn, ta, tb, p, plan.splits, live, stream);
   if (p.slots != nullptr) cudaFreeAsync(p.slots, stream);
   return rc;
+}
+
+extern "C" int univl_gemm_bf16(const void* A, long long lda, int a_mn_major, const void* B, long long ldb,
+                               int b_mn_major, int M, int N, int Kc, void* out, long long ldo, int epilogue,
+                               const float* bias, const void* aux_in, long long ld_aux_in, void* aux_out,
+                               long long ld_aux_out, float alpha, int block_n, int split_k, void* stream) {
+  return gemm_bf16(A, lda, a_mn_major, B, ldb, b_mn_major, M, N, Kc, out, ldo, epilogue, bias, aux_in, ld_aux_in,
+                   aux_out, ld_aux_out, alpha, block_n, split_k, nullptr, LIVE_NONE, stream);
+}
+
+extern "C" int univl_gemm_bf16_live(const void* A, long long lda, int a_mn_major, const void* B, long long ldb,
+                                    int b_mn_major, int M, int N, int Kc, void* out, long long ldo, int epilogue,
+                                    const float* bias, const void* aux_in, long long ld_aux_in, void* aux_out,
+                                    long long ld_aux_out, float alpha, int block_n, int split_k, const int* live,
+                                    void* stream) {
+  UNIVL_CHECK_ARG(live != nullptr, "gemm_live: null live row count");
+  UNIVL_CHECK_ARG(epilogue != EPI_ATOMIC_F32, "gemm_live: weight gradients are not bounded by live rows");
+  return gemm_bf16(A, lda, a_mn_major, B, ldb, b_mn_major, M, N, Kc, out, ldo, epilogue, bias, aux_in, ld_aux_in,
+                   aux_out, ld_aux_out, alpha, block_n, split_k, live, LIVE_M, stream);
 }
 
 extern "C" int univl_gemm_fp8(const void* A, long long lda, const float* a_scale, const void* B, long long ldb,
diff --git a/univl_b200/csrc/layernorm.cu b/univl_b200/csrc/layernorm.cu
--- a/univl_b200/csrc/layernorm.cu
+++ b/univl_b200/csrc/layernorm.cu
@@ -73,14 +73,16 @@
   return dropout_keep8(d.seed, d.stream, idx0, d.threshold);
 }
 
-template <typename TIn, int NVEC>
-__global__ void __launch_bounds__(LN_WARPS * 32, NVEC <= 3 ? 3 : 2)
+template <typename TIn, int NVEC, bool LIVE = false>
+__global__ void __launch_bounds__(LN_WARPS * 32, LIVE ? 2 : (NVEC <= 3 ? 3 : 2))
 layernorm_fwd_kernel(const TIn* __restrict__ x, const bf16* __restrict__ res, const float* __restrict__ gamma,
                      const float* __restrict__ beta, bf16* __restrict__ y, float* __restrict__ mean_out,
-                     float* __restrict__ rstd_out, int rows, float eps, DropCfg drop_in) {
+                     float* __restrict__ rstd_out, int rows, float eps, DropCfg drop_in,
+                     const int* __restrict__ live = nullptr, const int* __restrict__ row_map = nullptr) {
   pdl_trigger();
   pdl_wait();
   const DropCfg drop = resolve_drop(drop_in);
+  if constexpr (LIVE) rows = min(rows, *live);
   constexpr int cols = NVEC * 256;
   const int warp = threadIdx.x >> 5, lane = threadIdx.x & 31;
   const float inv_cols = 1.0f / (float)cols;
@@ -104,7 +106,8 @@
       const int c = (i * 32 + lane) * 8;
       raw_unpack(nx[i], z[i]);
       if (drop.mode == 1) {
-        const uint32_t keep = keep8_mask(drop, (uint64_t)row * cols + c);
+        const uint64_t drow = LIVE ? (uint64_t)row_map[row] : (uint64_t)row;
+        const uint32_t keep = keep8_mask(drop, drow * cols + c);
 #pragma unroll
         for (int j = 0; j < 8; ++j) z[i][j] = ((keep >> j) & 1u) ? z[i][j] * drop.scale : 0.f;
       }
@@ -150,7 +153,8 @@
 #pragma unroll
       for (int j = 0; j < 8; ++j) o[j] = g[j] * ((z[i][j] - mean) * rstd) + b[j];
       if (drop.mode == 2) {
-        const uint32_t keep = keep8_mask(drop, (uint64_t)row * cols + c);
+        const uint64_t drow = LIVE ? (uint64_t)row_map[row] : (uint64_t)row;
+        const uint32_t keep = keep8_mask(drop, drow * cols + c);
 #pragma unroll
         for (int j = 0; j < 8; ++j) o[j] = ((keep >> j) & 1u) ? o[j] * drop.scale : 0.f;
       }
@@ -165,21 +169,21 @@
                           DropCfg drop) {
   const dim3 g(grid), b(LN_WARPS * 32);
   switch (cols >> 8) {
-    case 1: launch_kernel(layernorm_fwd_kernel<TIn, 1>, g, b, 0, st, x, res, gamma, beta, y, mean, rstd, rows, eps, drop); break;
-    case 2: launch_kernel(layernorm_fwd_kernel<TIn, 2>, g, b, 0, st, x, res, gamma, beta, y, mean, rstd, rows, eps, drop); break;
-    case 3: launch_kernel(layernorm_fwd_kernel<TIn, 3>, g, b, 0, st, x, res, gamma, beta, y, mean, rstd, rows, eps, drop); break;
-    default: launch_kernel(layernorm_fwd_kernel<TIn, 4>, g, b, 0, st, x, res, gamma, beta, y, mean, rstd, rows, eps, drop); break;
+    case 1: launch_kernel(layernorm_fwd_kernel<TIn, 1>, g, b, 0, st, x, res, gamma, beta, y, mean, rstd, rows, eps, drop, nullptr, nullptr); break;
+    case 2: launch_kernel(layernorm_fwd_kernel<TIn, 2>, g, b, 0, st, x, res, gamma, beta, y, mean, rstd, rows, eps, drop, nullptr, nullptr); break;
+    case 3: launch_kernel(layernorm_fwd_kernel<TIn, 3>, g, b, 0, st, x, res, gamma, beta, y, mean, rstd, rows, eps, drop, nullptr, nullptr); break;
+    default: launch_kernel(layernorm_fwd_kernel<TIn, 4>, g, b, 0, st, x, res, gamma, beta, y, mean, rstd, rows, eps, drop, nullptr, nullptr); break;
   }
 }
 
 
 template <typename TIn>
 __device__ __forceinline__ void ln_bwd_load(const bf16* dy, const bf16* dy2, const TIn* x, const bf16* res,
-                                            long long off, const DropCfg& drop, float (&z)[8], float (&d)[8],
-                                            uint32_t& keep) {
+                                            long long off, long long drop_off, const DropCfg& drop, float (&z)[8],
+                                            float (&d)[8], uint32_t& keep) {
   load8(x + off, z);
   keep = 0xffu;
-  if (drop.mode != 0) keep = keep8_mask(drop, (uint64_t)off);
+  if (drop.mode != 0) keep = keep8_mask(drop, (uint64_t)drop_off);
   if (drop.mode == 1) {
 #pragma unroll
     for (int j = 0; j < 8; ++j) z[j] = ((keep >> j) & 1u) ? z[j] * drop.scale : 0.f;
@@ -211,13 +215,13 @@
   *reinterpret_cast<float4*>(p) = a;
   *reinterpret_cast<float4*>(p + 4) = b;
 }
-template <typename TIn, int NVEC>
-__global__ void __launch_bounds__(LNB_WARPS * 32, NVEC <= 3 ? 5 : 3)
+template <typename TIn, int NVEC, bool LIVE = false>
+__global__ void __launch_bounds__(LNB_WARPS * 32, LIVE ? 4 : (NVEC <= 3 ? 5 : 3))
 layernorm_bwd_kernel(const bf16* __restrict__ dy, const bf16* __restrict__ dy2, const TIn* __restrict__ x,
                      const bf16* __restrict__ res, const float* __restrict__ gamma, const float* __restrict__ mean_in,
                      const float* __restrict__ rstd_in, bf16* __restrict__ dx_res, bf16* __restrict__ dx_dense,
                      float* __restrict__ dgamma, float* __restrict__ dbeta, float* __restrict__ dbias, int rows,
-                     DropCfg drop_in) {
+                     DropCfg drop_in, const int* __restrict__ pos = nullptr) {
   pdl_trigger();
   pdl_wait();
   const DropCfg drop = resolve_drop(drop_in);
@@ -230,7 +234,12 @@
   for (int k = lane * 4; k < 3 * cols; k += 128) *reinterpret_cast<float4*>(my + k) = make_float4(0.f, 0.f, 0.f, 0.f);
   __syncwarp();
 
-  for (long long row = (long long)blockIdx.x * LNB_WARPS + warp; row < rows; row += (long long)gridDim.x * LNB_WARPS) {
+  for (long long q = (long long)blockIdx.x * LNB_WARPS + warp; q < rows; q += (long long)gridDim.x * LNB_WARPS) {
+    long long row = q;
+    if constexpr (LIVE) {
+      row = pos[q];
+      if (row < 0) continue;
+    }
     const float mean = mean_in[row], rstd = rstd_in[row];
     const float nm = -mean * rstd;
     float xh[NVEC][8], g[NVEC][8];
@@ -240,7 +249,7 @@
     for (int i = 0; i < NVEC; ++i) {
       const int c = (i * 32 + lane) * 8;
       float d[8], gm[8], dh[8];
-      ln_bwd_load(dy, dy2, x, res, row * cols + c, drop, xh[i], d, keep[i]);
+      ln_bwd_load(dy, dy2, x, res, row * cols + c, q * cols + c, drop, xh[i], d, keep[i]);
       load8(gamma + c, gm);
 #pragma unroll
       for (int j = 0; j < 8; ++j) {
@@ -289,7 +298,8 @@
 template <typename TIn>
 static int launch_ln_bwd(int grid, cudaStream_t st, const bf16* dy, const bf16* dy2, const TIn* x, const bf16* res,
                          const float* gamma, const float* mean, const float* rstd, bf16* dx_res, bf16* dx_dense,
-                         float* dgamma_out, float* dbeta_out, float* dbias_out, int rows, int cols, DropCfg drop) {
+                         float* dgamma_out, float* dbeta_out, float* dbias_out, int rows, int cols, DropCfg drop,
+                         const int* pos = nullptr) {
   const size_t smem = (size_t)LNB_WARPS * 3 * cols * sizeof(float);
   float* outs[3] = {dgamma_out, dbeta_out, dbias_out};
   float* parts[3] = {nullptr, nullptr, nullptr};
@@ -297,11 +307,17 @@
     if (outs[w] != nullptr)
       if (int rc = scratch_alloc((void**)&parts[w], (size_t)grid * cols * sizeof(float), st)) return rc;
   float *dgamma = parts[0], *dbeta = parts[1], *dbias = parts[2];
-  switch (cols >> 8) {
-    case 1: launch_kernel(layernorm_bwd_kernel<TIn, 1>, dim3(grid), dim3(LNB_WARPS * 32), smem, st, dy, dy2, x, res, gamma, mean, rstd, dx_res, dx_dense, dgamma, dbeta, dbias, rows, drop); break;
-    case 2: launch_kernel(layernorm_bwd_kernel<TIn, 2>, dim3(grid), dim3(LNB_WARPS * 32), smem, st, dy, dy2, x, res, gamma, mean, rstd, dx_res, dx_dense, dgamma, dbeta, dbias, rows, drop); break;
-    case 3: launch_kernel(layernorm_bwd_kernel<TIn, 3>, dim3(grid), dim3(LNB_WARPS * 32), smem, st, dy, dy2, x, res, gamma, mean, rstd, dx_res, dx_dense, dgamma, dbeta, dbias, rows, drop); break;
-    default: launch_kernel(layernorm_bwd_kernel<TIn, 4>, dim3(grid), dim3(LNB_WARPS * 32), smem, st, dy, dy2, x, res, gamma, mean, rstd, dx_res, dx_dense, dgamma, dbeta, dbias, rows, drop); break;
+  const dim3 g(grid), b(LNB_WARPS * 32);
+  if (pos != nullptr) {
+    UNIVL_CHECK_ARG(cols == 768, "layernorm_bwd_rows: cols must be 768 (got %d)", cols);
+    launch_kernel(layernorm_bwd_kernel<TIn, 3, true>, g, b, smem, st, dy, dy2, x, res, gamma, mean, rstd, dx_res, dx_dense, dgamma, dbeta, dbias, rows, drop, pos);
+  } else {
+    switch (cols >> 8) {
+      case 1: launch_kernel(layernorm_bwd_kernel<TIn, 1>, g, b, smem, st, dy, dy2, x, res, gamma, mean, rstd, dx_res, dx_dense, dgamma, dbeta, dbias, rows, drop, nullptr); break;
+      case 2: launch_kernel(layernorm_bwd_kernel<TIn, 2>, g, b, smem, st, dy, dy2, x, res, gamma, mean, rstd, dx_res, dx_dense, dgamma, dbeta, dbias, rows, drop, nullptr); break;
+      case 3: launch_kernel(layernorm_bwd_kernel<TIn, 3>, g, b, smem, st, dy, dy2, x, res, gamma, mean, rstd, dx_res, dx_dense, dgamma, dbeta, dbias, rows, drop, nullptr); break;
+      default: launch_kernel(layernorm_bwd_kernel<TIn, 4>, g, b, smem, st, dy, dy2, x, res, gamma, mean, rstd, dx_res, dx_dense, dgamma, dbeta, dbias, rows, drop, nullptr); break;
+    }
   }
   UNIVL_CHECK_LAUNCH("layernorm_bwd");
   for (int w = 0; w < 3; ++w)
@@ -373,6 +389,39 @@
                              rows, cols, make_drop(drop_mode, p_drop, rng_state, stream_id));
 }
 
+extern "C" int univl_layernorm_fwd_rows(const void* x, const void* res, const float* gamma, const float* beta, void* y,
+                                        float* mean, float* rstd, int rows, int cols, float eps, float p_drop,
+                                        int drop_mode, const unsigned long long* rng_state,
+                                        unsigned long long stream_id, const int* live, const int* row_map,
+                                        void* stream) {
+  if (int rc = check_ln_shape("layernorm_fwd_rows", rows, cols)) return rc;
+  UNIVL_CHECK_ARG(x && gamma && beta && y && live && row_map, "layernorm_fwd_rows: null pointer");
+  UNIVL_CHECK_ARG(cols == 768, "layernorm_fwd_rows: cols must be 768 (got %d)", cols);
+  UNIVL_CHECK_ARG(p_drop == 0.f || rng_state != nullptr, "layernorm_fwd_rows: dropout needs rng_state");
+  UNIVL_CHECK_ARG(p_drop >= 0.f && p_drop < 1.f && drop_mode >= 0 && drop_mode <= 2, "layernorm_fwd_rows: bad dropout");
+  if (rows == 0) return UNIVL_OK;
+  launch_kernel(layernorm_fwd_kernel<bf16, 3, true>, dim3(ln_grid(rows)), dim3(LN_WARPS * 32), 0, (cudaStream_t)stream,
+                (const bf16*)x, (const bf16*)res, gamma, beta, (bf16*)y, mean, rstd, rows, eps,
+                make_drop(drop_mode, p_drop, rng_state, stream_id), live, row_map);
+  UNIVL_CHECK_LAUNCH("layernorm_fwd_rows");
+  return UNIVL_OK;
+}
+
+extern "C" int univl_layernorm_bwd_rows(const void* dy, const void* dy2, const void* x, const void* res,
+                                        const float* gamma, const float* mean, const float* rstd, void* dx_res,
+                                        void* dx_dense, float* dgamma, float* dbeta, float* dbias, int rows, int cols,
+                                        float p_drop, int drop_mode, const unsigned long long* rng_state,
+                                        unsigned long long stream_id, const int* pos, void* stream) {
+  if (int rc = check_ln_shape("layernorm_bwd_rows", rows, cols)) return rc;
+  UNIVL_CHECK_ARG(dy && x && gamma && mean && rstd && pos, "layernorm_bwd_rows: null pointer");
+  UNIVL_CHECK_ARG(p_drop == 0.f || rng_state != nullptr, "layernorm_bwd_rows: dropout needs rng_state");
+  UNIVL_CHECK_ARG(p_drop >= 0.f && p_drop < 1.f && drop_mode >= 0 && drop_mode <= 2, "layernorm_bwd_rows: bad dropout");
+  if (rows == 0) return UNIVL_OK;
+  return launch_ln_bwd<bf16>(lnb_grid(rows), (cudaStream_t)stream, (const bf16*)dy, (const bf16*)dy2, (const bf16*)x,
+                             (const bf16*)res, gamma, mean, rstd, (bf16*)dx_res, (bf16*)dx_dense, dgamma, dbeta, dbias,
+                             rows, cols, make_drop(drop_mode, p_drop, rng_state, stream_id), pos);
+}
+
 extern "C" int univl_layernorm_f32_fwd(const float* x, const float* gamma, const float* beta, void* y, float* mean,
                                        float* rstd, int rows, int cols, float eps, void* stream) {
   if (int rc = check_ln_shape("layernorm_f32_fwd", rows, cols)) return rc;
diff --git a/univl_b200/csrc/misc.cu b/univl_b200/csrc/misc.cu
--- a/univl_b200/csrc/misc.cu
+++ b/univl_b200/csrc/misc.cu
@@ -9,9 +9,10 @@
   return u;
 }
 
+template <bool POS = false>
 __global__ void __launch_bounds__(256)
 colsum_bf16_kernel(const bf16* __restrict__ x, long long ld, float* __restrict__ out, int rows, int cols,
-                   int rows_per_block) {
+                   int rows_per_block, const int* __restrict__ pos = nullptr) {
   pdl_trigger();
   pdl_wait();
   __shared__ float red[8][257];
@@ -31,7 +32,13 @@
       acc[2 * j + 1] += f.y;
     }
   };
-  if (c0 < cols) {
+  if constexpr (POS) {
+    if (c0 + 8 <= cols)
+      for (int r = r_begin + rl; r < r_end; r += 8) {
+        const int pr = pos[r];
+        if (pr >= 0) add8(ld_nc_v4(x + (long long)pr * ld + c0));
+      }
+  } else if (c0 < cols) {
     const bf16* base = x + c0;
     if (c0 + 8 <= cols && (ld & 7) == 0 && (reinterpret_cast<uintptr_t>(base) & 15) == 0) {
       int r = r_begin + rl;
@@ -138,7 +145,7 @@
   return UNIVL_OK;
 }
 
-extern "C" int univl_colsum_bf16(const void* x, long long ld, float* out, int rows, int cols, void* stream) {
+static int colsum_bf16(const void* x, long long ld, float* out, int rows, int cols, const int* pos, void* stream) {
   UNIVL_CHECK_ARG(x && out && rows >= 0 && cols > 0, "colsum: bad arguments");
   if (rows == 0) return UNIVL_OK;
   const int col_blocks = (cols + 255) / 256;
@@ -149,10 +156,94 @@
   row_blocks = (rows + rpb - 1) / rpb;
   float* part;
   if (int rc = scratch_alloc((void**)&part, (size_t)row_blocks * cols * sizeof(float), (cudaStream_t)stream)) return rc;
-  launch_kernel(colsum_bf16_kernel, dim3(col_blocks, row_blocks), dim3(256), 0, (cudaStream_t)stream, (const bf16*)x, ld,
-                part, rows, cols, rpb);
+  if (pos != nullptr)
+    launch_kernel(colsum_bf16_kernel<true>, dim3(col_blocks, row_blocks), dim3(256), 0, (cudaStream_t)stream,
+                  (const bf16*)x, ld, part, rows, cols, rpb, pos);
+  else
+    launch_kernel(colsum_bf16_kernel<false>, dim3(col_blocks, row_blocks), dim3(256), 0, (cudaStream_t)stream,
+                  (const bf16*)x, ld, part, rows, cols, rpb, nullptr);
   UNIVL_CHECK_LAUNCH("colsum_bf16");
   return partials_reduce(part, row_blocks, 1, cols, out, cols, (cudaStream_t)stream);
+}
+
+extern "C" int univl_colsum_bf16(const void* x, long long ld, float* out, int rows, int cols, void* stream) {
+  return colsum_bf16(x, ld, out, rows, cols, nullptr, stream);
+}
+
+extern "C" int univl_colsum_bf16_rows(const void* x, long long ld, float* out, int rows, int cols, const int* pos,
+                                      void* stream) {
+  UNIVL_CHECK_ARG(pos != nullptr && (cols % 8) == 0 && (ld % 8) == 0 && ((uintptr_t)x & 15) == 0,
+                  "colsum_rows: null row map or rows not 16-byte vectors");
+  return colsum_bf16(x, ld, out, rows, cols, pos, stream);
+}
+
+__global__ void __launch_bounds__(256)
+rows_gather_kernel(const bf16* __restrict__ src, long long lds, const int* __restrict__ idx,
+                   const int* __restrict__ live, int rows, int cols, bf16* __restrict__ out, long long ldo) {
+  pdl_trigger();
+  pdl_wait();
+  const int n = min(rows, *live);
+  const int lane = threadIdx.x & 31;
+  for (int r = (blockIdx.x * blockDim.x + threadIdx.x) >> 5; r < n; r += (gridDim.x * blockDim.x) >> 5) {
+    const uint4* s = reinterpret_cast<const uint4*>(src + (long long)idx[r] * lds);
+    uint4* o = reinterpret_cast<uint4*>(out + (long long)r * ldo);
+    for (int c = lane; c < cols / 8; c += 32) o[c] = ld_nc_v4(reinterpret_cast<const bf16*>(s + c));
+  }
+}
+
+__global__ void __launch_bounds__(256)
+rows_expand_kernel(const bf16* __restrict__ src, long long lds, const int* __restrict__ pos, int rows, int cols,
+                   bf16* __restrict__ out, long long ldo) {
+  pdl_trigger();
+  pdl_wait();
+  const int lane = threadIdx.x & 31;
+  for (int q = (blockIdx.x * blockDim.x + threadIdx.x) >> 5; q < rows; q += (gridDim.x * blockDim.x) >> 5) {
+    const int r = pos[q];
+    uint4* o = reinterpret_cast<uint4*>(out + (long long)q * ldo);
+    if (r >= 0) {
+      const uint4* s = reinterpret_cast<const uint4*>(src + (long long)r * lds);
+      for (int c = lane; c < cols / 8; c += 32) o[c] = ld_nc_v4(reinterpret_cast<const bf16*>(s + c));
+    } else {
+      for (int c = lane; c < cols / 8; c += 32) o[c] = make_uint4(0, 0, 0, 0);
+    }
+  }
+}
+
+static int rows_grid(int rows) {
+  const long long blocks = ((long long)rows + 7) / 8;
+  const long long cap = (long long)device_sms() * 16;
+  return (int)(blocks < 1 ? 1 : (blocks > cap ? cap : blocks));
+}
+
+static int check_rows_copy(const char* what, const void* src, long long lds, const void* out, long long ldo, int rows,
+                           int cols) {
+  UNIVL_CHECK_ARG(src && out && rows >= 0 && cols > 0 && (cols % 8) == 0 && (lds % 8) == 0 && (ldo % 8) == 0 &&
+                      ((uintptr_t)src & 15) == 0 && ((uintptr_t)out & 15) == 0,
+                  "%s: bad arguments (rows %d, cols %d; 16-byte aligned rows of a multiple of 8 columns)", what, rows,
+                  cols);
+  return UNIVL_OK;
+}
+
+extern "C" int univl_rows_gather(const void* src, long long lds, const int* idx, const int* live, int rows, int cols,
+                                 void* out, long long ldo, void* stream) {
+  if (int rc = check_rows_copy("rows_gather", src, lds, out, ldo, rows, cols)) return rc;
+  UNIVL_CHECK_ARG(idx && live, "rows_gather: null index");
+  if (rows == 0) return UNIVL_OK;
+  launch_kernel(rows_gather_kernel, dim3(rows_grid(rows)), dim3(256), 0, (cudaStream_t)stream, (const bf16*)src, lds,
+                idx, live, rows, cols, (bf16*)out, ldo);
+  UNIVL_CHECK_LAUNCH("rows_gather");
+  return UNIVL_OK;
+}
+
+extern "C" int univl_rows_expand(const void* src, long long lds, const int* pos, int rows, int cols, void* out,
+                                 long long ldo, void* stream) {
+  if (int rc = check_rows_copy("rows_expand", src, lds, out, ldo, rows, cols)) return rc;
+  UNIVL_CHECK_ARG(pos != nullptr, "rows_expand: null index");
+  if (rows == 0) return UNIVL_OK;
+  launch_kernel(rows_expand_kernel, dim3(rows_grid(rows)), dim3(256), 0, (cudaStream_t)stream, (const bf16*)src, lds,
+                pos, rows, cols, (bf16*)out, ldo);
+  UNIVL_CHECK_LAUNCH("rows_expand");
+  return UNIVL_OK;
 }
 
 extern "C" int univl_cast_f32_to_bf16(const float* src, void* dst, long long n, void* stream) {
diff --git a/univl_b200/modules/module_cross.py b/univl_b200/modules/module_cross.py
--- a/univl_b200/modules/module_cross.py
+++ b/univl_b200/modules/module_cross.py
@@ -1,4 +1,5 @@
 import logging
+import os
 
 import torch
 from torch import nn
@@ -48,6 +49,16 @@
                                     self.dropout.p, self.training)
 
 
+CROSS_LAYOUTS = ("packed", "padded")
+
+
+def cross_layout():
+    value = os.environ.get("UNIVL_CROSS_LAYOUT", "packed")
+    if value not in CROSS_LAYOUTS:
+        raise ValueError("UNIVL_CROSS_LAYOUT must be one of %s, got %r" % ("/".join(CROSS_LAYOUTS), value))
+    return value
+
+
 def _n_seq(Nt, Nv, groups):
     groups = int(groups)
     if groups and (Nt % groups or Nv % groups):
@@ -79,7 +90,18 @@
         n_seq = _n_seq(Nt, Nv, all_pairs)
         x = self.embeddings.run(text2d, video2d, Nt, W, Nv, F, all_pairs)
         mask = ops.MaskSpec(text_mask, video_mask, all_pairs=all_pairs)
-        return self.encoder.run_first_token(x, n_seq, W + F, mask), n_seq
+        if cross_layout() == "padded" or W == 0 or F == 0:
+            return self.encoder.run_first_token(x, n_seq, W + F, mask), n_seq
+        pk = ops.CrossPacking(mask.a, mask.b, all_pairs)
+        x = ops.PackRowsFn.apply(x, pk)
+        layers = self.encoder.layer
+        for layer in layers[:-1]:
+            x = ops.EncoderLayerPackedFn.apply(x, pk, mask, layer.attention.output.dropout.p,
+                                               layer.attention.self.dropout.p, layer.training, *_layer_params(layer))
+        last = layers[-1]
+        return ops.EncoderLayerClsPackedFn.apply(x, pk, mask, last.attention.output.dropout.p,
+                                                 last.attention.self.dropout.p, last.training,
+                                                 *_layer_params(last)), n_seq
 
     def first_layer_source_qkv(self, text2d, video2d, Nt, W, Nv, F):
         return self.first_layer_source_rows(text2d, video2d, Nt, W, Nv, F)[1]
diff --git a/univl_b200/ops.py b/univl_b200/ops.py
--- a/univl_b200/ops.py
+++ b/univl_b200/ops.py
@@ -58,29 +58,37 @@
 
 
 def gemm(a, b, M, N, K, out, epi=EPI_BIAS, bias=None, aux_in=None, aux_out=None, a_mn=False, b_mn=False, alpha=1.0,
-         block_n=0, split_k=0):
+         block_n=0, split_k=0, live=None):
     _check2d(a, "gemm A"); _check2d(b, "gemm B"); _check2d(out, "gemm out")
-    call("univl_gemm_bf16", a.data_ptr(), a.stride(0), int(a_mn), b.data_ptr(), b.stride(0), int(b_mn), M, N, K,
-         out.data_ptr(), out.stride(0), epi, ptr(bias), ptr(aux_in), aux_in.stride(0) if aux_in is not None else 0,
-         ptr(aux_out), aux_out.stride(0) if aux_out is not None else 0, float(alpha), block_n, split_k)
+    args = (a.data_ptr(), a.stride(0), int(a_mn), b.data_ptr(), b.stride(0), int(b_mn), M, N, K, out.data_ptr(),
+            out.stride(0), epi, ptr(bias), ptr(aux_in), aux_in.stride(0) if aux_in is not None else 0, ptr(aux_out),
+            aux_out.stride(0) if aux_out is not None else 0, float(alpha), block_n, split_k)
+    if live is None:
+        call("univl_gemm_bf16", *args)
+    else:
+        call("univl_gemm_bf16_live", *args, live.data_ptr())
     return out
 
 
-def linear_fwd(x, w16, bias, epi=EPI_BIAS, aux_out=None, out_dtype=BF16, ld_out=None):
+def linear_fwd(x, w16, bias, epi=EPI_BIAS, aux_out=None, out_dtype=BF16, ld_out=None, live=None):
     T, K = x.shape
     N = w16.shape[0]
     if ld_out is None:
         out = _empty((T, N), out_dtype, x)
     else:
         out = _empty((T, ld_out), out_dtype, x)[:, :N]
-    return gemm(x, w16, T, N, K, out, epi=epi, bias=bias, aux_out=aux_out)
-
-
-def linear_dgrad(dy, w16, epi=EPI_BIAS, aux_in=None):
+    return gemm(x, w16, T, N, K, out, epi=epi, bias=bias, aux_out=aux_out, **_live_kw(live))
+
+
+def _live_kw(live):
+    return {} if live is None else {"live": live}
+
+
+def linear_dgrad(dy, w16, epi=EPI_BIAS, aux_in=None, live=None):
     T, N = dy.shape
     K = w16.shape[1]
     out = _empty((T, K), BF16, dy)
-    return gemm(dy, w16, T, K, N, out, epi=epi, aux_in=aux_in, b_mn=True)
+    return gemm(dy, w16, T, K, N, out, epi=epi, aux_in=aux_in, b_mn=True, **_live_kw(live))
 
 
 def linear_wgrad(dy, x, dw=None):
@@ -91,26 +99,33 @@
     return gemm(dy, x, N, K, T, dw, epi=EPI_ATOMIC, a_mn=True, b_mn=True)
 
 
-def colsum(x, out=None):
+def colsum(x, out=None, pos=None):
     rows, cols = x.shape
     if out is None:
         out = _zeros((cols,), F32, x)
-    call("univl_colsum_bf16", x.data_ptr(), x.stride(0), out.data_ptr(), rows, cols)
+    if pos is None:
+        call("univl_colsum_bf16", x.data_ptr(), x.stride(0), out.data_ptr(), rows, cols)
+    else:
+        call("univl_colsum_bf16_rows", x.data_ptr(), x.stride(0), out.data_ptr(), rows, cols, pos.data_ptr())
     return out
 
 
-def layernorm_fwd(x, res, gamma, beta, p=0.0, mode=0, seed=0, stream=0):
+def layernorm_fwd(x, res, gamma, beta, p=0.0, mode=0, seed=0, stream=0, pk=None):
     rows, cols = x.shape
     y = _empty((rows, cols), BF16, x)
     mean = _empty((rows,), F32, x)
     rstd = _empty((rows,), F32, x)
-    call("univl_layernorm_fwd", x.data_ptr(), ptr(res), gamma.data_ptr(), beta.data_ptr(), y.data_ptr(),
-         mean.data_ptr(), rstd.data_ptr(), rows, cols, LN_EPS, float(p), mode, seed, stream)
+    args = (x.data_ptr(), ptr(res), gamma.data_ptr(), beta.data_ptr(), y.data_ptr(), mean.data_ptr(), rstd.data_ptr(),
+            rows, cols, LN_EPS, float(p), mode, seed, stream)
+    if pk is None:
+        call("univl_layernorm_fwd", *args)
+    else:
+        call("univl_layernorm_fwd_rows", *args, pk.live.data_ptr(), pk.row_map.data_ptr())
     return y, mean, rstd
 
 
 def layernorm_bwd(dy, dy2, x, res, gamma, mean, rstd, p=0.0, mode=0, seed=0, stream=0, want_dbias=True,
-                  want_dx=True, dgamma=None, dbeta=None, dbias=None):
+                  want_dx=True, dgamma=None, dbeta=None, dbias=None, pk=None):
     rows, cols = x.shape
     dx_res = _empty((rows, cols), BF16, x) if want_dx else None
     dx_dense = _empty((rows, cols), BF16, x) if (want_dx and p > 0.0 and mode == 1) else dx_res
@@ -118,9 +133,13 @@
     dbeta = _zeros((cols,), F32, x) if dbeta is None else dbeta
     if dbias is None and want_dbias:
         dbias = _zeros((cols,), F32, x)
-    call("univl_layernorm_bwd", dy.data_ptr(), ptr(dy2), x.data_ptr(), ptr(res), gamma.data_ptr(), mean.data_ptr(),
-         rstd.data_ptr(), ptr(dx_res), ptr(dx_dense), dgamma.data_ptr(), dbeta.data_ptr(), ptr(dbias), rows, cols,
-         float(p), mode, seed, stream)
+    args = (dy.data_ptr(), ptr(dy2), x.data_ptr(), ptr(res), gamma.data_ptr(), mean.data_ptr(), rstd.data_ptr(),
+            ptr(dx_res), ptr(dx_dense), dgamma.data_ptr(), dbeta.data_ptr(), ptr(dbias), rows, cols, float(p), mode,
+            seed, stream)
+    if pk is None:
+        call("univl_layernorm_bwd", *args)
+    else:
+        call("univl_layernorm_bwd_rows", *args, pk.pos.data_ptr())
     return dx_res, dx_dense, dgamma, dbeta, dbias
 
 
@@ -394,6 +413,68 @@
         cu = _exclusive_cumsum(len_a.long() + len_b.long()).to(I32)
         return VarlenSeqs(cu, self.tokens(t0, t1, v0, v1), self.max_sk, self.idx_t, self.idx_v,
                           self.start_t[t0:t1].repeat_interleave(nv), self.start_v[v0:v1].repeat(nt), len_a)
+
+
+PACK_ALIGN = 128
+
+
+class CrossPacking:
+
+    def __init__(self, text_mask, video_mask, groups):
+        Nt, W = text_mask.shape
+        Nv, F = video_mask.shape
+        dev = text_mask.device
+        G = int(groups)
+        if G:
+            Bt, Bv = Nt // G, Nv // G
+            p = torch.arange(Nt * Nv // G, device=dev)
+            g, r = p // (Bt * Bv), p % (Bt * Bv)
+            i, j = g * Bt + r // Bv, g * Bv + r % Bv
+        else:
+            i = j = torch.arange(Nt, device=dev)
+        tm = text_mask.index_select(0, i) != 0
+        keep = torch.cat([tm, video_mask.index_select(0, j) != 0], 1)
+        keep |= ~tm[:, :1]
+        self.n_seq, self.S = keep.shape
+        cap = self.n_seq * self.S
+        self.capacity = cap
+        flat = keep.reshape(-1)
+        n = flat.sum()
+        target = torch.clamp((n + PACK_ALIGN - 1) // PACK_ALIGN * PACK_ALIGN, max=cap)
+        pad = ~flat
+        flat = flat | (pad & (torch.cumsum(pad, 0) <= target - n))
+        rank = torch.cumsum(flat, 0) - 1
+        self.pos = torch.where(flat, rank, -1).to(I32)
+        row_map = torch.empty(cap + 1, dtype=I32, device=dev)
+        row_map.scatter_(0, torch.where(flat, rank, cap), torch.arange(cap, dtype=I32, device=dev))
+        self.row_map = row_map[:cap]
+        self.live = target.to(I32).view(1)
+        self.cu = _exclusive_cumsum(flat.view(self.n_seq, self.S).sum(1)).to(I32)
+        self.first = self.cu[:-1].long()
+
+    def gather(self, src):
+        out = _empty((self.capacity, src.shape[1]), BF16, src)
+        call("univl_rows_gather", src.data_ptr(), src.stride(0), self.row_map.data_ptr(), self.live.data_ptr(),
+             self.capacity, src.shape[1], out.data_ptr(), out.stride(0))
+        return out
+
+    def expand(self, src):
+        out = _empty((self.capacity, src.shape[1]), BF16, src)
+        call("univl_rows_expand", src.data_ptr(), src.stride(0), self.pos.data_ptr(), self.capacity, src.shape[1],
+             out.data_ptr(), out.stride(0))
+        return out
+
+
+class PackRowsFn(torch.autograd.Function):
+
+    @staticmethod
+    def forward(ctx, x, pk):
+        ctx.pk = pk
+        return pk.gather(x)
+
+    @staticmethod
+    def backward(ctx, dy):
+        return ctx.pk.expand(dy.contiguous()), None
 
 
 def attention_varlen_fwd(q, k, v, seqs, q_first, qb=None, kb=None, vb=None):
@@ -493,14 +574,29 @@
         return self.arena.next_stream()
 
 
-def attn_block_fwd(xq, xkv, n_seq, Sq, Sk, mask, w, drop, need_bwd=True):
+def attn_block_fwd(xq, xkv, n_seq, Sq, Sk, mask, w, drop, need_bwd=True, pk=None):
     arena = rt.current()
     H = xq.shape[1]
     self_attn = xkv is xq
-    sv = {"self": self_attn, "fused": False}
+    sv = {"self": self_attn, "fused": False, "pk": pk}
     wqkv = arena.bf16_qkv(w["q"], w["k"], w["v"])
+    live = pk.live if pk is not None else None
     ctx = None
-    if self_attn and fused_attention_supported(n_seq, Sq, H):
+    if self_attn and pk is not None:
+        x_pad = pk.expand(xq)
+        bias = rt.packed_bias(w["bq"], w["bk"], w["bv"])
+        sa, sd = drop.stream(), drop.stream()
+        if fused_attention_supported(n_seq, Sq, H):
+            ctx_pad, lse, qkv = fused_qkv_attention_fwd(x_pad, wqkv, bias, n_seq, Sq, mask, drop.pa, drop.seed, sa,
+                                                        save_qkv=need_bwd)
+            sv["fused"] = True
+        else:
+            qkv = linear_fwd(x_pad, wqkv, bias)
+            ctx_pad, lse = attention_fwd(*_split_qkv(qkv), n_seq, Sq, Sk, mask, drop.pa, drop.seed, sa)
+        del x_pad
+        sv["qkv"], sv["ctx_pad"] = qkv, ctx_pad
+        ctx = pk.gather(ctx_pad)
+    elif self_attn and fused_attention_supported(n_seq, Sq, H):
         sa, sd = drop.stream(), drop.stream()
         ctx, lse, qkv = fused_qkv_attention_fwd(xq, wqkv, rt.packed_bias(w["bq"], w["bk"], w["bv"]), n_seq, Sq, mask,
                                                 drop.pa, drop.seed, sa, save_qkv=need_bwd)
@@ -512,14 +608,17 @@
         sv["qkv"] = qkv
     else:
         q = linear_fwd(xq, wqkv[:H], w["bq"])
-        kv = linear_fwd(xkv, wqkv[H:], rt.packed_bias(w["bk"], w["bv"]))
+        kv = linear_fwd(xkv, wqkv[H:], rt.packed_bias(w["bk"], w["bv"]), live=live)
+        if pk is not None:
+            kv = pk.expand(kv)
         k, v = kv[:, :H], kv[:, H:]
         sv["q"], sv["kv"] = q, kv
     if ctx is None:
         sa, sd = drop.stream(), drop.stream()
         ctx, lse = attention_fwd(q, k, v, n_seq, Sq, Sk, mask, drop.pa, drop.seed, sa)
-    ao = linear_fwd(ctx, arena.bf16(w["o"]), w["bo"])
-    y, mean, rstd = layernorm_fwd(ao, xq, w["gamma"], w["beta"], drop.ph, 1, drop.seed, sd)
+    q_pk = pk if self_attn else None
+    ao = linear_fwd(ctx, arena.bf16(w["o"]), w["bo"], live=q_pk.live if q_pk is not None else None)
+    y, mean, rstd = layernorm_fwd(ao, xq, w["gamma"], w["beta"], drop.ph, 1, drop.seed, sd, pk=q_pk)
     sv.update(xq=xq, xkv=xkv, ctx=ctx, lse=lse, ao=ao, mean=mean, rstd=rstd, sa=sa, sd=sd, n_seq=n_seq, Sq=Sq, Sk=Sk,
               mask=mask, pa=drop.pa, ph=drop.ph, seed=drop.seed, wqkv=wqkv, wo=arena.bf16(w["o"]),
               gamma=w["gamma"], w=w, sink=GradSink(), arena=arena, epoch=drop.epoch)
@@ -533,55 +632,74 @@
     dgamma, r_gamma = sink.one(w["gamma"])
     dbeta, r_beta = sink.one(w["beta"])
     dbo, r_bo = sink.one(w["bo"])
+    pk = sv["pk"]
+    live = pk.live if pk is not None else None
+    q_pk = pk if sv["self"] else None
+    q_live = q_pk.live if q_pk is not None else None
     g, gd, _, _, _ = layernorm_bwd(dy, dy2, sv["ao"], sv["xq"], sv["gamma"], sv["mean"], sv["rstd"], sv["ph"], 1,
-                                   sv["seed"], sv["sd"], dgamma=dgamma, dbeta=dbeta, dbias=dbo)
+                                   sv["seed"], sv["sd"], dgamma=dgamma, dbeta=dbeta, dbias=dbo, pk=q_pk)
     dwo, r_o = sink.one(w["o"])
-    linear_wgrad(gd, sv["ctx"], dwo)
-    dctx = linear_dgrad(gd, sv["wo"])
+    if q_pk is not None:
+        linear_wgrad(q_pk.expand(gd), sv["ctx_pad"], dwo)
+    else:
+        linear_wgrad(gd, sv["ctx"], dwo)
+    dctx = linear_dgrad(gd, sv["wo"], live=q_live)
     T, Tk = sv["xq"].shape[0], sv["xkv"].shape[0]
     dwqkv, r_w = sink.packed((w["q"], w["k"], w["v"]))
     dbqkv, r_b = sink.packed((w["bq"], w["bk"], w["bv"]))
     if sv["self"]:
         qkv = sv["qkv"]
-        dqkv = _empty((T, 3 * H), BF16, dy)
+        ctx = sv["ctx"]
+        if pk is not None:
+            dctx, ctx = pk.expand(dctx), sv["ctx_pad"]
+        dqkv = _empty((qkv.shape[0], 3 * H), BF16, dy)
         if sv["fused"] and os.environ.get("UNIVL_FUSED_ATTN_BWD", "1") != "0":
-            fused_attention_bwd(qkv, sv["ctx"], sv["lse"], dctx, dqkv, sv["n_seq"], sv["Sq"], sv["mask"], sv["pa"],
+            fused_attention_bwd(qkv, ctx, sv["lse"], dctx, dqkv, sv["n_seq"], sv["Sq"], sv["mask"], sv["pa"],
                                 sv["seed"], sv["sa"], dbias=dbqkv)
         else:
-            attention_bwd(qkv[:, :H], qkv[:, H:2 * H], qkv[:, 2 * H:], sv["ctx"], sv["lse"], dctx, dqkv[:, :H],
+            attention_bwd(qkv[:, :H], qkv[:, H:2 * H], qkv[:, 2 * H:], ctx, sv["lse"], dctx, dqkv[:, :H],
                           dqkv[:, H:2 * H], dqkv[:, 2 * H:], sv["n_seq"], sv["Sq"], sv["Sk"], sv["mask"], sv["pa"],
                           sv["seed"], sv["sa"], dbias=(dbqkv[:H], dbqkv[H:2 * H], dbqkv[2 * H:]),
                           rng_layout=1 if sv["fused"] else 0)
-        linear_wgrad(dqkv, sv["xq"], dwqkv)
-        dxq = linear_dgrad(dqkv, sv["wqkv"], epi=EPI_ADD, aux_in=g)
+        if pk is not None:
+            linear_wgrad(dqkv, pk.expand(sv["xq"]), dwqkv)
+            dqkv = pk.gather(dqkv)
+        else:
+            linear_wgrad(dqkv, sv["xq"], dwqkv)
+        dxq = linear_dgrad(dqkv, sv["wqkv"], epi=EPI_ADD, aux_in=g, live=live)
         dxkv = None
     else:
         q, kv = sv["q"], sv["kv"]
         dq = _empty((T, H), BF16, dy)
-        dkv = _empty((Tk, 2 * H), BF16, dy)
+        dkv = _empty((kv.shape[0], 2 * H), BF16, dy)
         attention_bwd(q, kv[:, :H], kv[:, H:], sv["ctx"], sv["lse"], dctx, dq, dkv[:, :H], dkv[:, H:], sv["n_seq"],
                       sv["Sq"], sv["Sk"], sv["mask"], sv["pa"], sv["seed"], sv["sa"],
                       dbias=(dbqkv[:H], dbqkv[H:2 * H], dbqkv[2 * H:]))
         linear_wgrad(dq, sv["xq"], dwqkv[:H])
-        linear_wgrad(dkv, sv["xkv"], dwqkv[H:])
+        if pk is not None:
+            linear_wgrad(dkv, pk.expand(sv["xkv"]), dwqkv[H:])
+            dkv = pk.gather(dkv)
+        else:
+            linear_wgrad(dkv, sv["xkv"], dwqkv[H:])
         dxq = linear_dgrad(dq, sv["wqkv"][:H], epi=EPI_ADD, aux_in=g)
-        dxkv = linear_dgrad(dkv, sv["wqkv"][H:]) if need_dxkv else None
+        dxkv = linear_dgrad(dkv, sv["wqkv"][H:], live=live) if need_dxkv else None
     rets = {"q": r_w[0], "k": r_w[1], "v": r_w[2], "bq": r_b[0], "bk": r_b[1], "bv": r_b[2], "o": r_o, "bo": r_bo,
             "gamma": r_gamma, "beta": r_beta}
     return dxq, dxkv, rets
 
 
-def ffn_block_fwd(x, w, drop):
+def ffn_block_fwd(x, w, drop, pk=None):
     arena = rt.current()
     w1, w2 = arena.bf16(w["w1"]), arena.bf16(w["w2"])
     T = x.shape[0]
+    live = pk.live if pk is not None else None
     pre = _empty((T, w1.shape[0]), BF16, x)
-    h = linear_fwd(x, w1, w["b1"], epi=EPI_GELU, aux_out=pre)
-    fo = linear_fwd(h, w2, w["b2"])
+    h = linear_fwd(x, w1, w["b1"], epi=EPI_GELU, aux_out=pre, live=live)
+    fo = linear_fwd(h, w2, w["b2"], live=live)
     sd = drop.stream()
-    y, mean, rstd = layernorm_fwd(fo, x, w["gamma"], w["beta"], drop.ph, 1, drop.seed, sd)
+    y, mean, rstd = layernorm_fwd(fo, x, w["gamma"], w["beta"], drop.ph, 1, drop.seed, sd, pk=pk)
     sv = dict(x=x, pre=pre, h=h, fo=fo, mean=mean, rstd=rstd, sd=sd, ph=drop.ph, seed=drop.seed, w1=w1, w2=w2,
-              gamma=w["gamma"], w=w, sink=GradSink(), arena=arena, epoch=drop.epoch)
+              gamma=w["gamma"], w=w, sink=GradSink(), arena=arena, epoch=drop.epoch, pk=pk)
     return y, sv
 
 
@@ -591,16 +709,19 @@
     dgamma, r_gamma = sink.one(w["gamma"])
     dbeta, r_beta = sink.one(w["beta"])
     db2, r_b2 = sink.one(w["b2"])
+    pk = sv["pk"]
+    live = pk.live if pk is not None else None
     g, gd, _, _, _ = layernorm_bwd(dy, None, sv["fo"], sv["x"], sv["gamma"], sv["mean"], sv["rstd"], sv["ph"], 1,
-                                   sv["seed"], sv["sd"], dgamma=dgamma, dbeta=dbeta, dbias=db2)
+                                   sv["seed"], sv["sd"], dgamma=dgamma, dbeta=dbeta, dbias=db2, pk=pk)
+    pad = pk.expand if pk is not None else (lambda t: t)
     dw2, r_w2 = sink.one(w["w2"])
-    linear_wgrad(gd, sv["h"], dw2)
-    dpre = linear_dgrad(gd, sv["w2"], epi=EPI_GELU_BWD, aux_in=sv["pre"])
+    linear_wgrad(pad(gd), pad(sv["h"]), dw2)
+    dpre = linear_dgrad(gd, sv["w2"], epi=EPI_GELU_BWD, aux_in=sv["pre"], live=live)
     db1, r_b1 = sink.one(w["b1"])
-    colsum(dpre, db1)
+    colsum(dpre, db1, pos=pk.pos if pk is not None else None)
     dw1, r_w1 = sink.one(w["w1"])
-    linear_wgrad(dpre, sv["x"], dw1)
-    dx = linear_dgrad(dpre, sv["w1"])
+    linear_wgrad(pad(dpre), pad(sv["x"]), dw1)
+    dx = linear_dgrad(dpre, sv["w1"], live=live)
     return g, dx, {"w1": r_w1, "b1": r_b1, "w2": r_w2, "b2": r_b2, "gamma": r_gamma, "beta": r_beta}
 
 
@@ -654,6 +775,54 @@
         dxkv.view(n_seq, S, H)[:, 0].add_(dxq)
         ctx.sva = ctx.svf = None
         return (dxkv, None, None, None, None, None, None) + tuple(ga[k] for k in ATT_KEYS) + \
+            tuple(gf[k] for k in FFN_KEYS)
+
+
+class EncoderLayerPackedFn(torch.autograd.Function):
+
+    @staticmethod
+    def forward(ctx, x, pk, mask, p_hidden, p_attn, training, *params):
+        wa = dict(zip(ATT_KEYS, params[:10]))
+        wf = dict(zip(FFN_KEYS, params[10:16]))
+        drop = _Drop(p_hidden, p_attn, training)
+        y1, sva = attn_block_fwd(x, x, pk.n_seq, pk.S, pk.S, mask, wa, drop, need_bwd=any(ctx.needs_input_grad),
+                                 pk=pk)
+        y2, svf = ffn_block_fwd(y1, wf, drop, pk=pk)
+        ctx.sva, ctx.svf = sva, svf
+        return y2
+
+    @staticmethod
+    def backward(ctx, dy):
+        dy = dy.contiguous()
+        g2, dy1, gf = ffn_block_bwd(dy, ctx.svf)
+        dx, _, ga = attn_block_bwd(dy1, g2, ctx.sva)
+        ctx.sva = ctx.svf = None
+        return (dx, None, None, None, None, None) + tuple(ga[k] for k in ATT_KEYS) + tuple(gf[k] for k in FFN_KEYS)
+
+
+class EncoderLayerClsPackedFn(torch.autograd.Function):
+
+    @staticmethod
+    def forward(ctx, x, pk, mask, p_hidden, p_attn, training, *params):
+        wa = dict(zip(ATT_KEYS, params[:10]))
+        wf = dict(zip(FFN_KEYS, params[10:16]))
+        drop = _Drop(p_hidden, p_attn, training)
+        xq = x.index_select(0, pk.first)
+        y1, sva = attn_block_fwd(xq, x, pk.n_seq, 1, pk.S, mask, wa, drop, pk=pk)
+        y2, svf = ffn_block_fwd(y1, wf, drop)
+        ctx.sva, ctx.svf = sva, svf
+        ctx.pk = pk
+        return y2
+
+    @staticmethod
+    def backward(ctx, dy):
+        dy = dy.contiguous()
+        g2, dy1, gf = ffn_block_bwd(dy, ctx.svf)
+        dxq, dxkv, ga = attn_block_bwd(dy1, g2, ctx.sva)
+        first = ctx.pk.first
+        dxkv.index_copy_(0, first, dxkv.index_select(0, first) + dxq)
+        ctx.sva = ctx.svf = ctx.pk = None
+        return (dxkv, None, None, None, None, None) + tuple(ga[k] for k in ATT_KEYS) + \
             tuple(gf[k] for k in FFN_KEYS)
 
 
```

Measured after the change: 1498, median of 6. +3.7%, better.
